# transferia/transferia

Measured on NVIDIA H100. Metric: ChangeItems/sec on ClickBench-shaped 99-col batches (filter_rows + cast + ClickHouse native block + LZ4 frames), higher is better.
Workload: dtype u8

## Files before the change

### transferia_b200/csrc/device_types.cuh

```cuda
#pragma once
#include <cstdint>
#include "../../include/tfgpu.h"

namespace tfk {

enum OutKind : int32_t {
    OK_COPY = 0,
    OK_BOOL = 1,
    OK_DATE = 2,
    OK_DATETIME = 3,
    OK_TS64 = 4,
    OK_STR = 5,
    OK_MASK = 6,
    OK_TODT = 8,
    OK_TOSTR = 7
};

struct DCol {
    int32_t type;
    int32_t out_kind;
    int32_t in_w;
    int32_t out_w;
    int32_t nullable;
    int32_t str_slot;
    int32_t mask_slot;
    int32_t pad;
    const uint8_t* values;
    const uint8_t* validity;
    const uint32_t* offsets;
    const uint8_t* heap;
    const uint8_t* aux;
    uint64_t hdr_off;
    uint64_t null_off;
    uint64_t out_off;
    uint64_t aux_off;
    uint64_t offs_off;
};

struct DTerm {
    int32_t col, op, vtype, nlist;
    int64_t i; double f;
    uint32_t s_off, s_len;
    uint32_t list_off, pad;
};

struct DFilterStep { int32_t expr_begin, nexpr, step_index, flags; };

struct DState {
    uint64_t n_kept;
    uint64_t n_errors;
    uint64_t raw_total;
    uint64_t n_frames;
    uint64_t wire_total;
    uint32_t frame_ticket;
    uint32_t pad;
};

__host__ __device__ inline int varint_len(uint64_t v) { int n = 1; while (v >= 0x80) { v >>= 7; n++; } return n; }

}
```

### transferia_b200/csrc/kernels_deflate.cuh

```cuda
#pragma once
#include "device_types.cuh"
#include "kernels_encode.cuh"
#include "deflate_sum.hpp"

namespace tfk {

#define DF_CHUNK 16384
#define DF_THREADS 512
#define DF_PPT (DF_CHUNK / DF_THREADS)
#define DF_HASH_BITS 12
#define DF_CHUNK_OVERHEAD 10
#define DF_FLAG_AGG (1ull << 62)
#define DF_FLAG_INCL (2ull << 62)
#define DF_VAL_MASK ((1ull << 62) - 1)

struct DfSmem { uint32_t data, dist, lenb, work, path, hist, lens, codes, sort, crct, total; };
__host__ __device__ inline DfSmem df_smem() {
    DfSmem s; uint32_t o = 0;
    s.data = o; o += 16 + DF_CHUNK + 32;
    s.dist = o; o += 2 * DF_CHUNK;
    s.lenb = o; o += DF_CHUNK;
    s.work = o; o += 2 * DF_CHUNK + 64;
    s.path = o; o += (DF_CHUNK / 32 + 4) * 4;
    s.hist = o; o += (288 + 32 + 20) * 4;
    s.lens = o; o += 288 + 32 + 32;
    s.codes = o; o += (288 + 32 + 32) * 2;
    s.sort = o; o += 320 * 4 * 2 + 320 * 2 + 320 * 2;
    s.crct = o; o += 256 * 4;
    s.total = o; return s;
}

struct DeflateArgs {
    const uint8_t* text; uint64_t total;
    uint8_t* out;
    unsigned long long* pfx;
    uint32_t* sums;
    uint32_t* ticket;
    uint32_t nchunks;
    int zlib;
    DState* st;
};

__device__ __forceinline__ uint32_t df_ld32(const uint32_t* w, uint32_t p) {
    const uint32_t i = p >> 2, s = (p & 3) * 8;
    return __funnelshift_r(w[i], w[i + 1], s);
}
__device__ __forceinline__ uint32_t df_match_len(const uint32_t* dw, uint32_t c, uint32_t p, uint32_t maxl) {
    uint32_t n = 0;
    while (n < maxl) {
        const uint32_t x = df_ld32(dw, c + n) ^ df_ld32(dw, p + n);
        if (x) { n += (uint32_t)(__ffs((int)x) - 1) >> 3; break; }
        n += 4;
    }
    return n < maxl ? n : maxl;
}
__device__ __forceinline__ void df_len_sym(uint32_t len, uint32_t& sym, uint32_t& eb, uint32_t& ev) {
    const uint32_t l = len - 3;
    if (l < 8) { sym = 257 + l; eb = 0; ev = 0; }
    else if (l == 255) { sym = 285; eb = 0; ev = 0; }
    else { const uint32_t nb = 31 - __clz(l); eb = nb - 2; sym = 257 + 4 * (nb - 1) + ((l >> eb) & 3); ev = l & ((1u << eb) - 1); }
}
__device__ __forceinline__ void df_dist_sym(uint32_t d, uint32_t& sym, uint32_t& eb, uint32_t& ev) {
    const uint32_t v = d - 1;
    if (v < 4) { sym = v; eb = 0; ev = 0; }
    else { const uint32_t nb = 31 - __clz(v); eb = nb - 1; sym = 2 * nb + ((v >> eb) & 1); ev = v & ((1u << eb) - 1); }
}
__device__ __forceinline__ uint32_t df_fixed_len(uint32_t s) { return s < 144 ? 8 : s < 256 ? 9 : s < 280 ? 7 : 8; }
__device__ __forceinline__ void df_put(uint32_t* img, uint32_t at, uint32_t v, uint32_t n) {
    if (!n) return;
    const uint32_t w = at >> 5, s = at & 31;
    atomicOr(&img[w], v << s);
    if (s + n > 32) atomicOr(&img[w + 1], v >> (32 - s));
}

#ifdef TF_KERNELS_DEFLATE
__device__ void df_huff_lengths(uint32_t* w, const uint16_t* sym, int n, uint32_t maxbits, uint8_t* lens) {
    w[0] += w[1];
    int root = 0, leaf = 2;
    for (int next = 1; next < n - 1; next++) {
        if (leaf >= n || w[root] < w[leaf]) { w[next] = w[root]; w[root++] = (uint32_t)next; }
        else w[next] = w[leaf++];
        if (leaf >= n || (root < next && w[root] < w[leaf])) { w[next] += w[root]; w[root++] = (uint32_t)next; }
        else w[next] += w[leaf++];
    }
    w[n - 2] = 0;
    for (int next = n - 3; next >= 0; next--) w[next] = w[w[next]] + 1;
    {
        int avail = 1, used = 0, depth = 0, r = n - 2, next = n - 1;
        while (avail > 0) {
            while (r >= 0 && (int)w[r] == depth) { used++; r--; }
            while (avail > used) { w[next--] = (uint32_t)depth; avail--; }
            avail = 2 * used; depth++; used = 0;
        }
    }
    uint32_t cnt[16];
    for (uint32_t l = 0; l <= 15; l++) cnt[l] = 0;
    for (int i = 0; i < n; i++) cnt[w[i] < maxbits ? w[i] : maxbits]++;
    uint32_t kraft = 0;
    for (uint32_t l = 1; l <= maxbits; l++) kraft += cnt[l] << (maxbits - l);
    while (kraft > (1u << maxbits)) {
        cnt[maxbits]--;
        for (uint32_t l = maxbits - 1; l > 0; l--) if (cnt[l]) { cnt[l]--; cnt[l + 1] += 2; break; }
        kraft--;
    }
    int i = n - 1;
    for (uint32_t l = 1; l <= maxbits; l++) for (uint32_t k = 0; k < cnt[l]; k++) lens[sym[i--]] = (uint8_t)l;
}
__device__ void df_codes(const uint8_t* lens, int n, uint16_t* codes) {
    uint32_t cnt[16], next[16];
    for (int l = 0; l < 16; l++) cnt[l] = 0;
    for (int s = 0; s < n; s++) cnt[lens[s]]++;
    cnt[0] = 0; uint32_t c = 0;
    for (int l = 1; l < 16; l++) { c = (c + cnt[l - 1]) << 1; next[l] = c; }
    for (int s = 0; s < n; s++) { const uint32_t l = lens[s]; codes[s] = l ? (uint16_t)(__brev(next[l]++) >> (32 - l)) : 0; }
}

__device__ __forceinline__ unsigned long long df_lookback(const DeflateArgs& a, uint32_t f, uint32_t lane) {
    unsigned long long excl = 0;
    int64_t base = (int64_t)f;
    for (uint32_t spins = 0; base > 0;) {
        const int64_t j = base - 1 - (int64_t)lane;
        const unsigned long long v = j >= 0 ? *(volatile unsigned long long*)&a.pfx[j] : DF_FLAG_INCL;
        const uint32_t fl = (uint32_t)(v >> 62);
        const uint32_t incl = __ballot_sync(0xffffffffu, fl == 2), none = __ballot_sync(0xffffffffu, fl == 0);
        const uint32_t upto = incl ? (uint32_t)__ffs((int)incl) - 1 : 31u;
        const uint32_t need = upto == 31 ? 0xffffffffu : ((2u << upto) - 1);
        if (none & need) {
            if (++spins > (1u << 20)) { if (lane == 0) a.st->pad = 1; break; }
            __nanosleep(100); continue;
        }
        unsigned long long part = lane <= upto ? (v & DF_VAL_MASK) : 0ull;
#pragma unroll
        for (int d = 16; d; d >>= 1) part += __shfl_xor_sync(0xffffffffu, part, d);
        excl += part; base -= 32;
        if (incl) break;
    }
    return excl;
}

__device__ __forceinline__ uint32_t df_block_xor(uint32_t v, uint32_t* red) {
#pragma unroll
    for (int d = 16; d; d >>= 1) v ^= __shfl_xor_sync(0xffffffffu, v, d);
    if ((threadIdx.x & 31) == 0) red[threadIdx.x >> 5] = v;
    __syncthreads();
    uint32_t r = 0;
    for (uint32_t w = 0; w < (blockDim.x + 31) / 32; w++) r ^= red[w];
    __syncthreads();
    return r;
}
__device__ __forceinline__ uint64_t df_block_sum64(uint64_t v, unsigned long long* red) {
#pragma unroll
    for (int d = 16; d; d >>= 1) v += __shfl_xor_sync(0xffffffffu, v, d);
    if ((threadIdx.x & 31) == 0) red[threadIdx.x >> 5] = v;
    __syncthreads();
    uint64_t r = 0;
    for (uint32_t w = 0; w < (blockDim.x + 31) / 32; w++) r += red[w];
    __syncthreads();
    return r;
}

__global__ void __launch_bounds__(DF_THREADS, 2) k_deflate_chunks(DeflateArgs a) {
    extern __shared__ __align__(16) uint8_t smem[];
    const DfSmem S = df_smem();
    uint8_t* db = smem + S.data + 16;
    const uint32_t* dw = (const uint32_t*)db;
    uint16_t* dist = (uint16_t*)(smem + S.dist);
    uint8_t* lenb = smem + S.lenb;
    uint16_t* J = (uint16_t*)(smem + S.work);
    uint32_t* img = (uint32_t*)(smem + S.work);
    uint32_t* path = (uint32_t*)(smem + S.path);
    uint32_t* hl = (uint32_t*)(smem + S.hist); uint32_t* hd = hl + 288; uint32_t* hc = hd + 32;
    uint8_t* ll_len = smem + S.lens; uint8_t* d_len = ll_len + 288; uint8_t* c_len = d_len + 32;
    uint16_t* ll_code = (uint16_t*)(smem + S.codes); uint16_t* d_code = ll_code + 288; uint16_t* c_code = d_code + 32;
    uint32_t* bw = (uint32_t*)(smem + S.sort);
    uint32_t* sw = bw + 320;
    uint16_t* ssym = (uint16_t*)(sw + 320);
    uint16_t* rle = ssym + 320;
    uint32_t* crct = (uint32_t*)(smem + S.crct);
    __shared__ uint32_t s_f, s_btype, s_hdr_bits, s_nbytes, s_nrle, s_hlit, s_hdist, s_hclen;
    __shared__ uint32_t red[33];
    __shared__ unsigned long long red64[32], s_off;
    const uint32_t tid = threadIdx.x, lane = tid & 31, warp = tid >> 5;

    for (uint32_t i = tid; i < 256; i += DF_THREADS) {
        uint32_t c = i;
        for (int k = 0; k < 8; k++) c = (c & 1) ? (c >> 1) ^ tfdf::CRC_POLY : c >> 1;
        crct[i] = c;
    }
    for (;;) {
        __syncthreads();
        if (tid == 0) s_f = atomicAdd(a.ticket, 1u);
        __syncthreads();
        const uint32_t f = s_f;
        if (f >= a.nchunks) break;
        const uint64_t pos0 = (uint64_t)f * DF_CHUNK;
        const uint32_t L = (uint32_t)((a.total - pos0 < DF_CHUNK) ? a.total - pos0 : DF_CHUNK);

        {
            const int4* g = (const int4*)(a.text + pos0);
            const uint32_t nv = (L + 15) >> 4;
            int4* d4 = (int4*)db;
            for (uint32_t i = tid; i < DF_CHUNK / 16 + 2; i += DF_THREADS) d4[i] = i < nv ? __ldg(g + i) : make_int4(0, 0, 0, 0);
            if (tid < 4) ((uint32_t*)(smem + S.data))[tid] = 0;
            int4* t4 = (int4*)J;
            for (uint32_t i = tid; i < (2u << DF_HASH_BITS) / 16; i += DF_THREADS) t4[i] = make_int4(0, 0, 0, 0);
            for (uint32_t i = tid; i < DF_CHUNK / 32 + 4; i += DF_THREADS) path[i] = 0;
            for (uint32_t i = tid; i < 288 + 32 + 20; i += DF_THREADS) hl[i] = 0;
        }
        __syncthreads();
        if (tid < 16 && L + tid < ((L + 15) & ~15u)) db[L + tid] = 0;
        {
            const uint32_t b0 = tid * DF_PPT, b1 = b0 + DF_PPT < L ? b0 + DF_PPT : L, nb = b1 > b0 ? b1 - b0 : 0;
            if (a.zlib) {
                uint64_t s1 = 0, s2 = 0;
                for (uint32_t i = 0; i < nb; i++) { const uint32_t v = db[b0 + i]; s1 += v; s2 += (uint64_t)(L - b0 - i) * v; }
                s1 = df_block_sum64(s1, red64) % tfdf::ADLER_MOD; s2 = df_block_sum64(s2, red64) % tfdf::ADLER_MOD;
                if (tid == 0) { a.sums[2 * f] = (uint32_t)s1; a.sums[2 * f + 1] = (uint32_t)s2; }
            } else {
                uint32_t c = 0;
                if (nb) {
                    c = 0xffffffffu;
                    for (uint32_t i = 0; i < nb; i++) c = crct[(c ^ db[b0 + i]) & 0xff] ^ (c >> 8);
                    c = tfdf::crc_mulmod(tfdf::crc_xpow8(L - b1), ~c);
                }
                c = df_block_xor(c, red);
                if (tid == 0) a.sums[2 * f] = c;
            }
        }

        const uint32_t nrounds = (L + DF_THREADS - 1) / DF_THREADS;
        for (uint32_t r = 0; r < nrounds; r++) {
            const uint32_t p = r * DF_THREADS + tid;
            const bool valid = p + 4 <= L;
            const uint32_t w = valid ? df_ld32(dw, p) : 0, h = (w * 2654435761u) >> (32 - DF_HASH_BITS);
            const uint32_t t1 = valid ? J[h] : 0;
            __syncthreads();
            if (valid) J[h] = (uint16_t)(p + 1);
            __syncthreads();
            const uint32_t t2 = valid ? J[h] : 0;
            uint32_t best = 0, bd = 0;
            if (valid) {
                const uint32_t maxl = L - p < 258 ? L - p : 258;
                uint32_t c = 0xffffffffu;
                if (p >= 1 && df_ld32(dw, p - 1) == w) c = p - 1;
                else if (p >= 2 && df_ld32(dw, p - 2) == w) c = p - 2;
                else if (p >= 4 && df_ld32(dw, p - 4) == w) c = p - 4;
                if (c != 0xffffffffu) { best = df_match_len(dw, c, p, maxl); bd = p - c; }
                const uint32_t ct = (t2 && t2 - 1 < p) ? t2 - 1 : (t1 ? t1 - 1 : 0xffffffffu);
                if (ct != 0xffffffffu && ct != c && best < maxl) {
                    const uint32_t m = df_match_len(dw, ct, p, maxl);
                    if (m > best) { best = m; bd = p - ct; }
                }
            }
            if (p < L) { lenb[p] = (uint8_t)(best >= 4 ? best - 3 : 0); dist[p] = (uint16_t)bd; }
        }
        __syncthreads();

        for (uint32_t k = 0; k < DF_PPT; k++) { const uint32_t p = tid * DF_PPT + k; if (p < L) J[p] = (uint16_t)(p + (lenb[p] ? lenb[p] + 3u : 1u)); }
        if (tid == 0) { J[L] = (uint16_t)L; path[0] = 1; }
        __syncthreads();
        for (;;) {
            uint32_t bits = path[tid];
            while (bits) {
                const uint32_t k = (uint32_t)__ffs((int)bits) - 1; bits &= bits - 1;
                const uint32_t p = tid * DF_PPT + k;
                if (p < L) { const uint32_t q = J[p]; if (q < L) atomicOr(&path[q >> 5], 1u << (q & 31)); }
            }
            __syncthreads();
            uint32_t nx[DF_PPT / 2];
#pragma unroll
            for (uint32_t k = 0; k < DF_PPT; k += 2) {
                const uint32_t p = tid * DF_PPT + k;
                const uint32_t lo = p < L ? J[J[p]] : 0, hi = p + 1 < L ? J[J[p + 1]] : 0;
                nx[k / 2] = lo | (hi << 16);
            }
            __syncthreads();
#pragma unroll
            for (uint32_t k = 0; k < DF_PPT; k += 2) {
                const uint32_t p = tid * DF_PPT + k;
                if (p < L) J[p] = (uint16_t)nx[k / 2];
                if (p + 1 < L) J[p + 1] = (uint16_t)(nx[k / 2] >> 16);
            }
            __syncthreads();
            if (J[0] == L) break;
            __syncthreads();
        }
        const uint32_t mine = path[tid] & (tid * DF_PPT + DF_PPT <= L ? 0xffffffffu : (tid * DF_PPT < L ? (1u << (L - tid * DF_PPT)) - 1 : 0u));

        uint32_t ext = 0;
        for (uint32_t bits = mine; bits;) {
            const uint32_t k = (uint32_t)__ffs((int)bits) - 1; bits &= bits - 1;
            const uint32_t p = tid * DF_PPT + k, l = lenb[p];
            if (!l) { atomicAdd(&hl[db[p]], 1u); continue; }
            uint32_t s, eb, ev, ds, deb, dev;
            df_len_sym(l + 3, s, eb, ev); df_dist_sym(dist[p], ds, deb, dev);
            atomicAdd(&hl[s], 1u); atomicAdd(&hd[ds], 1u); ext += eb + deb;
        }
        if (tid == 0) atomicAdd(&hl[256], 1u);
        uint32_t ext_total; block_excl_scan(ext, &ext_total, red);

        const int nzd = __syncthreads_count(tid < 30 && hd[tid] > 0);
        if (tid < 288) { bw[tid] = tid < 286 ? hl[tid] : 0; ll_len[tid] = 0; }
        else if (tid < 320) {
            const uint32_t i = tid - 288; uint32_t v = i < 30 ? hd[i] : 0;
            if (i < 30 && !v && ((nzd == 0 && i < 2) || (nzd == 1 && i == (hd[0] ? 1u : 0u)))) v = 1;
            bw[tid] = v; d_len[i] = 0;
        }
        __syncthreads();
        {
            const bool ll = tid < 286, dd = tid >= 288 && tid < 318;
            if (ll || dd) {
                const uint32_t base = ll ? 0 : 288, n = ll ? 286 : 30, i = tid - base, v = bw[tid];
                if (v) {
                    uint32_t rank = 0;
                    for (uint32_t j = 0; j < n; j++) { const uint32_t u = bw[base + j]; rank += (u && (u < v || (u == v && j < i))) ? 1u : 0u; }
                    sw[base + rank] = v; ssym[base + rank] = (uint16_t)i;
                }
            }
        }
        const int nzl = __syncthreads_count(tid < 286 && hl[tid] > 0);
        if (tid == 0) df_huff_lengths(sw, ssym, nzl, 15, ll_len);
        if (tid == 32) df_huff_lengths(sw + 288, ssym + 288, nzd < 2 ? 2 : nzd, 15, d_len);
        __syncthreads();
        if (tid == 0) {
            uint32_t hlit = 286; while (hlit > 257 && !ll_len[hlit - 1]) hlit--;
            uint32_t hdist = 30; while (hdist > 1 && !d_len[hdist - 1]) hdist--;
            const uint32_t N = hlit + hdist;
            auto lv = [&](uint32_t i) -> uint32_t { return i < hlit ? ll_len[i] : d_len[i - hlit]; };
            uint32_t nr = 0;
            for (uint32_t i = 0; i < N;) {
                const uint32_t v = lv(i); uint32_t run = 1;
                while (i + run < N && lv(i + run) == v) run++;
                i += run;
                if (v == 0) {
                    while (run >= 11) { const uint32_t r = run < 138 ? run : 138; rle[nr++] = (uint16_t)(18 | ((r - 11) << 8)); run -= r; }
                    if (run >= 3) { rle[nr++] = (uint16_t)(17 | ((run - 3) << 8)); run = 0; }
                } else {
                    rle[nr++] = (uint16_t)v; run--;
                    while (run >= 3) { const uint32_t r = run < 6 ? run : 6; rle[nr++] = (uint16_t)(16 | ((r - 3) << 8)); run -= r; }
                }
                while (run) { rle[nr++] = (uint16_t)v; run--; }
            }
            for (uint32_t k = 0; k < nr; k++) hc[rle[k] & 0xff]++;
            uint32_t n = 0;
            for (uint32_t s = 0; s < 19; s++) { c_len[s] = 0; if (hc[s]) { sw[n] = hc[s]; ssym[n] = (uint16_t)s; n++; } }
            for (uint32_t s = 0; n < 2; s++) if (!hc[s]) { sw[n] = 1; ssym[n] = (uint16_t)s; n++; }
            for (uint32_t i = 1; i < n; i++) {
                const uint32_t v = sw[i]; const uint16_t y = ssym[i]; int j = (int)i - 1;
                while (j >= 0 && (sw[j] > v || (sw[j] == v && ssym[j] > y))) { sw[j + 1] = sw[j]; ssym[j + 1] = ssym[j]; j--; }
                sw[j + 1] = v; ssym[j + 1] = y;
            }
            df_huff_lengths(sw, ssym, (int)n, 7, c_len);
            const uint8_t order[19] = {16, 17, 18, 0, 8, 7, 9, 6, 10, 5, 11, 4, 12, 3, 13, 2, 14, 1, 15};
            uint32_t hclen = 19; while (hclen > 4 && !c_len[order[hclen - 1]]) hclen--;
            uint64_t hdr = 14 + 3 * hclen;
            for (uint32_t s = 0; s < 19; s++) hdr += (uint64_t)hc[s] * (c_len[s] + (s == 16 ? 2 : s == 17 ? 3 : s == 18 ? 7 : 0));
            uint64_t dyn = 3 + hdr + ext_total, fix = 3 + ext_total;
            for (uint32_t s = 0; s < 286; s++) { dyn += (uint64_t)hl[s] * ll_len[s]; fix += (uint64_t)hl[s] * df_fixed_len(s); }
            for (uint32_t s = 0; s < 30; s++) { dyn += (uint64_t)hd[s] * d_len[s]; fix += (uint64_t)hd[s] * 5; }
            const uint64_t by_dyn = (dyn + 3 + 7) / 8 + 4, by_fix = (fix + 3 + 7) / 8 + 4, by_sto = (uint64_t)L + DF_CHUNK_OVERHEAD;
            uint32_t bt = 2; uint64_t by = by_dyn;
            if (by_fix <= by) { bt = 1; by = by_fix; }
            if (by_sto <= by) { bt = 0; by = by_sto; }
            s_btype = bt; s_nbytes = (uint32_t)by; s_hdr_bits = bt == 2 ? (uint32_t)hdr : 0;
            s_nrle = nr; s_hlit = hlit; s_hdist = hdist; s_hclen = hclen;
            if (bt == 1) { for (uint32_t s = 0; s < 288; s++) ll_len[s] = (uint8_t)df_fixed_len(s); for (uint32_t s = 0; s < 30; s++) d_len[s] = 5; }
            if (bt != 0) { df_codes(ll_len, 288, ll_code); df_codes(d_len, 30, d_code); df_codes(c_len, 19, c_code); }
        }
        __syncthreads();
        const uint32_t btype = s_btype, nbytes = s_nbytes;
        for (uint32_t i = tid; i < (nbytes + 11) / 4; i += DF_THREADS) img[i] = 0;
        __syncthreads();

        if (btype == 0) {
            uint8_t* ib = (uint8_t*)img;
            if (tid == 0) { ib[1] = (uint8_t)L; ib[2] = (uint8_t)(L >> 8); ib[3] = (uint8_t)~L; ib[4] = (uint8_t)(~L >> 8); ib[L + 8] = 0xff; ib[L + 9] = 0xff; }
            for (uint32_t i = tid; i < L; i += DF_THREADS) ib[5 + i] = db[i];
        } else {
            if (tid == 0) {
                df_put(img, 0, (uint32_t)btype << 1, 3);
                if (btype == 2) {
                    uint32_t at = 3;
                    df_put(img, at, s_hlit - 257, 5); df_put(img, at + 5, s_hdist - 1, 5); df_put(img, at + 10, s_hclen - 4, 4); at += 14;
                    const uint8_t order[19] = {16, 17, 18, 0, 8, 7, 9, 6, 10, 5, 11, 4, 12, 3, 13, 2, 14, 1, 15};
                    for (uint32_t k = 0; k < s_hclen; k++) { df_put(img, at, c_len[order[k]], 3); at += 3; }
                    for (uint32_t k = 0; k < s_nrle; k++) {
                        const uint32_t s = rle[k] & 0xff, x = rle[k] >> 8;
                        df_put(img, at, c_code[s], c_len[s]); at += c_len[s];
                        const uint32_t xb = s == 16 ? 2 : s == 17 ? 3 : s == 18 ? 7 : 0;
                        df_put(img, at, x, xb); at += xb;
                    }
                }
            }
            uint32_t my = 0;
            for (uint32_t bits = mine; bits;) {
                const uint32_t k = (uint32_t)__ffs((int)bits) - 1; bits &= bits - 1;
                const uint32_t p = tid * DF_PPT + k, l = lenb[p];
                if (!l) { my += ll_len[db[p]]; continue; }
                uint32_t s, eb, ev, ds, deb, dev;
                df_len_sym(l + 3, s, eb, ev); df_dist_sym(dist[p], ds, deb, dev);
                my += ll_len[s] + eb + d_len[ds] + deb;
            }
            uint32_t tok_total; uint32_t at = 3 + s_hdr_bits + block_excl_scan(my, &tok_total, red);
            for (uint32_t bits = mine; bits;) {
                const uint32_t k = (uint32_t)__ffs((int)bits) - 1; bits &= bits - 1;
                const uint32_t p = tid * DF_PPT + k, l = lenb[p];
                if (!l) { const uint32_t c = db[p]; df_put(img, at, ll_code[c], ll_len[c]); at += ll_len[c]; continue; }
                uint32_t s, eb, ev, ds, deb, dev;
                df_len_sym(l + 3, s, eb, ev); df_dist_sym(dist[p], ds, deb, dev);
                df_put(img, at, ll_code[s] | (ev << ll_len[s]), ll_len[s] + eb); at += ll_len[s] + eb;
                df_put(img, at, d_code[ds] | (dev << d_len[ds]), d_len[ds] + deb); at += d_len[ds] + deb;
            }
            if (tid == 0) {
                const uint32_t e = 3 + s_hdr_bits + tok_total;
                df_put(img, e, ll_code[256], ll_len[256]);
                uint8_t* ib = (uint8_t*)img; ib[nbytes - 2] = 0xff; ib[nbytes - 1] = 0xff;
            }
        }
        if (tid == 0) *(volatile unsigned long long*)&a.pfx[f] = DF_FLAG_AGG | nbytes;
        __syncthreads();

        if (warp == 0) {
            const unsigned long long excl = df_lookback(a, f, lane);
            if (lane == 0) { *(volatile unsigned long long*)&a.pfx[f] = DF_FLAG_INCL | (excl + nbytes); s_off = excl; }
        }
        __syncthreads();
        uint8_t* G = a.out + (a.zlib ? sizeof(tfdf::ZLIB_HDR) : sizeof(tfdf::GZIP_HDR)) + s_off;
        const uint8_t* ib = (const uint8_t*)img;
        for (uint32_t i = tid; i < nbytes; i += DF_THREADS) G[i] = ib[i];
    }
}

__global__ void __launch_bounds__(1024) k_deflate_finish(DeflateArgs a) {
    __shared__ uint32_t red[33];
    __shared__ unsigned long long red64[32];
    const uint32_t tid = threadIdx.x, n = a.nchunks;
    const uint64_t T = a.total;
    const uint32_t per = (n + blockDim.x - 1) / blockDim.x, f0 = tid * per < n ? tid * per : n, f1 = f0 + per < n ? f0 + per : n;
    uint32_t sum;
    if (a.zlib) {
        uint64_t s1 = 0, s2 = 0;
        for (uint32_t f = f0; f < f1; f++) {
            const uint64_t end = (uint64_t)f * DF_CHUNK + DF_CHUNK < T ? (uint64_t)f * DF_CHUNK + DF_CHUNK : T;
            s1 += a.sums[2 * f]; s2 = (s2 + a.sums[2 * f + 1] + ((T - end) % tfdf::ADLER_MOD) * a.sums[2 * f]) % tfdf::ADLER_MOD;
        }
        s1 = df_block_sum64(s1 % tfdf::ADLER_MOD, red64) % tfdf::ADLER_MOD;
        s2 = df_block_sum64(s2, red64) % tfdf::ADLER_MOD;
        sum = (uint32_t)((((T % tfdf::ADLER_MOD) + s2) % tfdf::ADLER_MOD) << 16 | ((1 + s1) % tfdf::ADLER_MOD));
    } else {
        uint32_t acc = 0; uint64_t end = (uint64_t)f0 * DF_CHUNK;
        const uint32_t xc = tfdf::crc_xpow8(DF_CHUNK);
        for (uint32_t f = f0; f < f1; f++) {
            const uint64_t len = T - end < DF_CHUNK ? T - end : DF_CHUNK;
            acc = tfdf::crc_mulmod(len == DF_CHUNK ? xc : tfdf::crc_xpow8(len), acc) ^ a.sums[2 * f];
            end += len;
        }
        if (f1 > f0) acc = tfdf::crc_mulmod(tfdf::crc_xpow8(T - end), acc);
        sum = df_block_xor(acc, red);
    }
    if (tid == 0) {
        const uint32_t hdr = a.zlib ? sizeof(tfdf::ZLIB_HDR) : sizeof(tfdf::GZIP_HDR);
        const uint64_t body = n ? (a.pfx[n - 1] & DF_VAL_MASK) : 0;
        uint8_t* o = a.out;
        if (a.zlib) { o[0] = 0x78; o[1] = 0x9c; }
        else { o[0] = 0x1f; o[1] = 0x8b; o[2] = 0x08; for (int i = 3; i < 9; i++) o[i] = 0; o[9] = 0xff; }
        o += hdr + body;
        *o++ = 0x03; *o++ = 0x00;
        if (a.zlib) { for (int i = 0; i < 4; i++) *o++ = (uint8_t)(sum >> (24 - 8 * i)); }
        else { for (int i = 0; i < 4; i++) *o++ = (uint8_t)(sum >> (8 * i)); for (int i = 0; i < 4; i++) *o++ = (uint8_t)(T >> (8 * i)); }
        a.st->wire_total = hdr + body + 2 + (a.zlib ? tfdf::ZLIB_TRAILER : tfdf::GZIP_TRAILER);
    }
}
#endif

}
```

### transferia_b200/csrc/kernels_encode.cuh

```cuda
#pragma once
#include "device_types.cuh"

namespace tfk {

__device__ __forceinline__ uint32_t warp_incl_scan(uint32_t v) {
    const unsigned lane = threadIdx.x & 31;
#pragma unroll
    for (int d = 1; d < 32; d <<= 1) { uint32_t t = __shfl_up_sync(0xffffffffu, v, d); if (lane >= (unsigned)d) v += t; }
    return v;
}
__device__ __forceinline__ uint32_t block_excl_scan(uint32_t v, uint32_t* total, uint32_t* smem33) {
    const unsigned lane = threadIdx.x & 31, warp = threadIdx.x >> 5, nw = (blockDim.x + 31) >> 5;
    uint32_t inc = warp_incl_scan(v);
    if (lane == 31) smem33[warp] = inc;
    __syncthreads();
    if (warp == 0) {
        uint32_t w = lane < nw ? smem33[lane] : 0;
        uint32_t wi = warp_incl_scan(w);
        smem33[lane] = wi - w;
        if (lane == 31) smem33[32] = wi;
    }
    __syncthreads();
    uint32_t res = inc - v + smem33[warp];
    *total = smem33[32];
// ... 119 lines not shown
    const bool is_float1 = v.cls == 2 || v.cls == 3 || v.cls == 0;
    const double float1 = v.cls == 2 ? v.f : (v.cls == 3 ? v.f : 0.0);
    const int64_t* il = (const int64_t*)(blob + t.list_off);
    const double* fl = (const double*)(blob + t.list_off);
    switch (base) {
    case 1:
        if (is_int1) {
            if (is_set) { bool c = false; for (int k = 0; k < t.nlist; k++) c |= (il[k] == v.i); matched = (op == 6) ? c : !c; return 0; }
            matched = ordered<int64_t>(v.i, t.i, op); return 0;
        }
        if (is_float1) {
            if (is_set) {
                if (trunc(float1) == float1) { int64_t x = go_f2i64(float1); bool c = false; for (int k = 0; k < t.nlist; k++) c |= (il[k] == x); matched = (op == 6) ? c : !c; }
                else matched = false;
                return 0;
            }
            matched = ordered<double>(float1, (double)t.i, op); return 0;
        }
        break;
    case 2:
        if (is_int1 || is_float1) {
            const double x = is_int1 ? (double)v.i : float1;
            if (is_set) { bool c = false; for (int k = 0; k < t.nlist; k++) c |= (fl[k] == x); matched = (op == 6) ? c : !c; return 0; }
            matched = ordered<double>(x, t.f, op); return 0;
        }
        break;
    case 3:
        if (!is_list && v.cls == 3) { matched = ordered<int>(v.i ? 1 : 0, t.i ? 1 : 0, op); return 0; }
        break;
    case 4:
        if (v.cls == 4 || v.cls == 5) {
            const uint8_t* lit = blob + t.s_off;
            if (!is_list) {
                if (op == 8) { matched = contains_bytes(v.s, v.slen, lit, t.s_len); return 0; }
                if (op == 9) { matched = !contains_bytes(v.s, v.slen, lit, t.s_len); return 0; }
                if (is_set) return TF_ROWERR_FILTER_TYPEPAIR;
                const int c = cmp_bytes(v.s, v.slen, lit, t.s_len);
                matched = ordered<int>(c, 0, op); return 0;
            }
            if (!is_set) return TF_ROWERR_FILTER_TYPEPAIR;
            const uint32_t* so = (const uint32_t*)(blob + t.list_off);
            const uint8_t* sh = (const uint8_t*)(so + t.nlist + 1);
            bool c = false;
            for (int k = 0; k < t.nlist && !c; k++) { uint32_t a = so[k], b = so[k + 1]; c = (b - a == v.slen) && cmp_bytes(sh + a, b - a, v.s, v.slen) == 0; }
            matched = (op == 6) ? c : !c; return 0;
        }
        break;
    case 5:
        if (v.cls == 6) {
            const int64_t um = v.i * 1000000LL + (int64_t)(v.nsec / 1000u);
            if (is_set) { bool c = false; for (int k = 0; k < t.nlist; k++) c |= (il[k] == um); matched = (op == 6) ? c : !c; return 0; }
            matched = ordered<int64_t>(um, t.i, op); return 0;
        }
        break;
    case 6:
        if (op == 0) { matched = v.cls == 0; return 0; }
        if (op == 1) { matched = v.cls != 0; return 0; }
        break;
    }
    return TF_ROWERR_FILTER_TYPEPAIR;
}

struct FilterArgs {
    const DCol* cols; const uint8_t* kinds; uint64_t nrows;
    const DFilterStep* steps; int nsteps;
    const uint32_t* expr_off;
    const DTerm* terms; const uint8_t* blob;
    uint8_t* keep; uint8_t* errcode; uint16_t* errstep; uint32_t* blockcnt; DState* st;
    const uint8_t* pre_err;
    const uint16_t* pre_term;
    int sink_guard;
};

#ifdef TF_KERNELS_ENCODE
__global__ void __launch_bounds__(256) k_filter(FilterArgs a) {
    __shared__ uint32_t s_cnt, s_err;
    if (threadIdx.x == 0) { s_cnt = 0; s_err = 0; }
    __syncthreads();
    const uint64_t r = (uint64_t)blockIdx.x * blockDim.x + threadIdx.x;
    bool keep = false, is_err = false;
    if (r < a.nrows) {
        keep = true; int err = 0, estep = 0;
        const int kind = a.kinds ? a.kinds[r] : TF_KIND_INSERT;
        if (a.pre_err && a.pre_err[r]) { err = a.pre_err[r]; estep = a.pre_term ? a.pre_term[r] : 0xff; keep = false; }
        for (int s = 0; s < a.nsteps && keep; s++) {
            const DFilterStep st = a.steps[s];
            if (st.flags & 1) { if ((st.expr_begin >> kind) & 1) keep = false; continue; }
            if (kind == TF_KIND_UPDATE || kind == TF_KIND_DELETE) { err = TF_ROWERR_FILTER_KIND; estep = st.step_index; keep = false; break; }
            if (st.flags & 2) continue;
            bool any = false;
            for (int e = 0; e < st.nexpr && !any && !err; e++) {
                bool all = true;
                const uint32_t kb = a.expr_off[st.expr_begin + e], ke = a.expr_off[st.expr_begin + e + 1];
                for (uint32_t k = kb; k < ke; k++) {
                    const DTerm t = a.terms[k];
                    const RowVal v = load_val(a.cols[t.col], r);
                    bool m = false; const int rc = eval_term(v, t, a.blob, m);
                    if (rc) { err = rc; break; }
                    if (!m) { all = false; break; }
                }
                if (!err && all) any = true;
            }
            if (err) { estep = st.step_index; keep = false; break; }
            if (!any) keep = false;
        }
        if (keep && a.sink_guard && (kind == TF_KIND_UPDATE || kind == TF_KIND_DELETE)) { err = TF_ROWERR_SINK_KIND_HOST; estep = 0xff; keep = false; }
        a.keep[r] = keep ? 1 : 0;
        a.errcode[r] = (uint8_t)err; a.errstep[r] = (uint16_t)estep; is_err = err != 0;
    }
    const unsigned b = __ballot_sync(0xffffffffu, keep);
    const unsigned be = __ballot_sync(0xffffffffu, is_err);
    if ((threadIdx.x & 31) == 0) { if (b) atomicAdd(&s_cnt, __popc(b)); if (be) atomicAdd(&s_err, __popc(be)); }
    __syncthreads();
    if (threadIdx.x == 0) { a.blockcnt[blockIdx.x] = s_cnt; if (s_err) atomicAdd((unsigned long long*)&a.st->n_errors, (unsigned long long)s_err); }
}
#endif

struct DevRowErr { uint32_t row; uint16_t code, term; };
#ifdef TF_KERNELS_ENCODE
__global__ void __launch_bounds__(256) k_collect_errors(const uint8_t* errcode, const uint16_t* errstep, uint64_t nrows, DevRowErr* out, unsigned long long* counter, unsigned long long cap) {
    const uint64_t r = (uint64_t)blockIdx.x * blockDim.x + threadIdx.x;
    const uint8_t c = r < nrows ? errcode[r] : 0;
    if (!c) return;
    const unsigned long long at = atomicAdd(counter, 1ull);
    if (at < cap) out[at] = DevRowErr{(uint32_t)r, c, errstep[r]};
}
#endif

#ifdef TF_KERNELS_ENCODE
__global__ void __launch_bounds__(1024) k_scan_blockcnt(const uint32_t* blockcnt, uint32_t* blockoff, uint32_t nblocks, DState* st) {
    __shared__ uint32_t sm[33];
    uint32_t carry = 0;
    for (uint32_t base = 0; base < nblocks; base += blockDim.x) {
        const uint32_t i = base + threadIdx.x;
        const uint32_t v = i < nblocks ? blockcnt[i] : 0;
        uint32_t tot; const uint32_t ex = block_excl_scan(v, &tot, sm);
        if (i < nblocks) blockoff[i] = carry + ex;
        carry += tot;
    }
    if (threadIdx.x == 0) st->n_kept = carry;
}
#endif

#ifdef TF_KERNELS_ENCODE
__global__ void __launch_bounds__(256) k_compact_sel(const uint8_t* keep, const uint32_t* blockoff, uint64_t nrows, uint32_t* sel) {
    __shared__ uint32_t sm[33];
    const uint64_t r = (uint64_t)blockIdx.x * blockDim.x + threadIdx.x;
    const uint32_t k = (r < nrows && keep[r]) ? 1u : 0u;
    uint32_t tot; const uint32_t ex = block_excl_scan(k, &tot, sm);
    if (k) sel[blockoff[blockIdx.x] + ex] = (uint32_t)r;
}
#endif

struct LayoutArgs {
    DCol* cols; int ncols;
    const int32_t* out_cols;
    const int32_t* str_cols; int nstr;
    const uint32_t* tile_sum;
    uint64_t* tile_base;
    uint32_t ntiles_cap;
    const uint8_t* col_headers; const uint32_t* col_header_off;
    uint8_t* raw; DState* st;
    uint64_t nrows_in; int has_sel; uint32_t frame_bytes;
    uint64_t* col_bytes;
};

#define TF_STR_TILE 256
#define TF_STR_THREADS 256
#define TF_STR_STAGE 16384

#ifdef TF_KERNELS_ENCODE
__global__ void __launch_bounds__(1024) k_layout_scan(LayoutArgs a) {
    __shared__ uint32_t sm[33];
    const int s = blockIdx.x;
    const uint64_t n = a.st->n_kept;
    const uint32_t ntiles = (uint32_t)((n + TF_STR_TILE - 1) / TF_STR_TILE);
    uint64_t carry = 0;
    for (uint32_t base = 0; base < ntiles; base += blockDim.x) {
        const uint32_t i = base + threadIdx.x;
        const uint32_t v = i < ntiles ? a.tile_sum[(size_t)s * a.ntiles_cap + i] : 0;
        uint32_t tot; const uint32_t ex = block_excl_scan(v, &tot, sm);
        if (i < ntiles) a.tile_base[(size_t)s * a.ntiles_cap + i] = carry + ex;
        carry += tot;
    }
    if (threadIdx.x == 0) a.col_bytes[s] = carry;
}
#endif

#ifdef TF_KERNELS_ENCODE
__global__ void __launch_bounds__(256) k_layout_finish(LayoutArgs a) {
    __shared__ uint64_t s_size[3][256];
    __shared__ uint64_t s_pos[256];
    __shared__ uint64_t s_run;
    const uint64_t n = a.st->n_kept;
    if (threadIdx.x == 0) {
        uint8_t* o = a.raw; uint64_t p = 0;
        o[p++] = 1; o[p++] = 0; o[p++] = 2; o[p++] = 0xff; o[p++] = 0xff; o[p++] = 0xff; o[p++] = 0xff; o[p++] = 0;
        uint64_t v = (uint64_t)a.ncols; while (v >= 0x80) { o[p++] = (uint8_t)(v | 0x80); v >>= 7; } o[p++] = (uint8_t)v;
        v = n; while (v >= 0x80) { o[p++] = (uint8_t)(v | 0x80); v >>= 7; } o[p++] = (uint8_t)v;
        s_run = p;
    }
    for (int base = 0; base < a.ncols; base += 256) {
        const int c = base + threadIdx.x;
        __syncthreads();
        if (c < a.ncols) {
            const DCol& d = a.cols[a.out_cols[c]];
            s_size[0][threadIdx.x] = a.col_header_off[c + 1] - a.col_header_off[c];
            s_size[1][threadIdx.x] = (d.nullable && n) ? n : 0;
            s_size[2][threadIdx.x] = n ? ((d.out_kind == OK_STR || d.out_kind == OK_TOSTR) ? a.col_bytes[d.str_slot] : (uint64_t)d.out_w * n) : 0;
        }
        __syncthreads();
        if (threadIdx.x == 0) {
            uint64_t p = s_run; const int m = a.ncols - base < 256 ? a.ncols - base : 256;
            for (int k = 0; k < m; k++) { s_pos[k] = p; p += s_size[0][k] + s_size[1][k] + s_size[2][k]; }
            s_run = p;
        }
        __syncthreads();
        if (c < a.ncols) {
            DCol& d = a.cols[a.out_cols[c]];
            const uint64_t p = s_pos[threadIdx.x];
            d.hdr_off = p; d.null_off = p + s_size[0][threadIdx.x]; d.out_off = d.null_off + s_size[1][threadIdx.x];
            const uint32_t hb = a.col_header_off[c], hn = (uint32_t)s_size[0][threadIdx.x];
            for (uint32_t k = 0; k < hn; k++) a.raw[p + k] = a.col_headers[hb + k];
        }
    }
    __syncthreads();
    if (threadIdx.x == 0) {
        const uint64_t p = s_run;
        a.st->raw_total = p;
        a.st->n_frames = p ? (p + a.frame_bytes - 1) / a.frame_bytes : 1;
        a.st->frame_ticket = 0;
    }
}
#endif

struct ColRegions { uint64_t values, validity, aux, offsets, heap, heap_len; };

#ifdef TF_KERNELS_ENCODE
__global__ void __launch_bounds__(256) k_layout_columnar(LayoutArgs a, ColRegions* regions) {
    __shared__ uint64_t s_sz[5][256];
    __shared__ uint64_t s_pos[256];
    __shared__ uint64_t s_run;
    const uint64_t n = a.st->n_kept;
    if (threadIdx.x == 0) s_run = 0;
    for (int base = 0; base < a.ncols; base += 256) {
        const int k = base + threadIdx.x;
        __syncthreads();
        if (k < a.ncols) {
            const DCol& d = a.cols[a.out_cols[k]];
            const bool var = d.out_kind == OK_STR || d.out_kind == OK_MASK || d.out_kind == OK_TOSTR;
            const bool fresh = d.out_kind == OK_MASK || d.out_kind == OK_TOSTR || d.out_kind == OK_TODT;
            const uint64_t heap = (d.out_kind == OK_STR || d.out_kind == OK_TOSTR) ? a.col_bytes[d.str_slot] : (d.out_kind == OK_MASK ? 64 * n : 0);
            s_sz[0][threadIdx.x] = var ? 0 : (uint64_t)d.out_w * n;
            s_sz[1][threadIdx.x] = (d.validity && !fresh) ? (n + 7) / 8 : 0;
            s_sz[2][threadIdx.x] = (d.aux && !fresh) ? (d.type == TF_ANY ? n : 4 * n) : 0;
            s_sz[3][threadIdx.x] = var ? 4 * (n + 1) : 0;
            s_sz[4][threadIdx.x] = heap;
        }
        __syncthreads();
        if (threadIdx.x == 0) {
            uint64_t p = s_run; const int m = a.ncols - base < 256 ? a.ncols - base : 256;
            for (int q = 0; q < m; q++) { s_pos[q] = p; for (int z = 0; z < 5; z++) p += (s_sz[z][q] + 15) & ~15ull; }
            s_run = p;
        }
        __syncthreads();
        if (k < a.ncols) {
            DCol& d = a.cols[a.out_cols[k]];
            uint64_t p = s_pos[threadIdx.x]; ColRegions r;
            auto take = [&](int z) { const uint64_t at = p; p += (s_sz[z][threadIdx.x] + 15) & ~15ull; return at; };
            const uint64_t v = take(0), val = take(1), ax = take(2), of = take(3), hp = take(4);
            const bool var = d.out_kind == OK_STR || d.out_kind == OK_MASK || d.out_kind == OK_TOSTR;
            d.out_off = var ? hp : v; d.null_off = val; d.aux_off = ax; d.offs_off = of;
            r.values = var ? ~0ull : v; r.validity = s_sz[1][threadIdx.x] ? val : ~0ull; r.aux = s_sz[2][threadIdx.x] ? ax : ~0ull;
            r.offsets = var ? of : ~0ull; r.heap = var ? hp : ~0ull; r.heap_len = s_sz[4][threadIdx.x];
            regions[k] = r;
            if (var) ((uint32_t*)(a.raw + of))[n] = (uint32_t)s_sz[4][threadIdx.x];
        }
    }
    __syncthreads();
    if (threadIdx.x == 0) { a.st->raw_total = s_run; a.st->n_frames = 0; a.st->frame_ticket = 0; }
}
#endif

struct EncodeArgs {
    const DCol* cols;
    const int32_t* slots;
    const uint32_t* sel; const DState* st; uint8_t* raw;
    uint32_t* tile_sum; const uint64_t* tile_base; uint32_t ntiles_cap;
    int columnar;
};

#define TF_SLOT_NULLMAP (1 << 30)
#define TF_SLOT_AUX (1 << 29)
#define TF_SLOT_ZEROMAP (1 << 28)
#define TF_FIX_TILE_WORDS 2048
#define CH_MAX_DATE_SEC 4291747200LL

enum StreamKind { SK_COPY = 0, SK_BOOL, SK_DATE, SK_DATETIME, SK_TS64, SK_NULLMAP, SK_AUX32, SK_AUX8, SK_ZERO, SK_TODT_CH, SK_TODT_SEC };

template <int K, int INW> __device__ __forceinline__ uint64_t elem_t(const DCol& c, const uint32_t* sel, uint64_t j, uint64_t n) {
    if (j >= n) return 0;
    const uint64_t r = sel ? sel[j] : j;
    if (K == SK_ZERO) return 0;
    if (K == SK_TODT_CH || K == SK_TODT_SEC) {
        int64_t s = 0;
        if (row_valid(c, r)) s = c.type == TF_INT32 ? (int64_t)((const int32_t*)c.values)[r] : (int64_t)((const uint32_t*)c.values)[r];
        if (K == SK_TODT_SEC) return (uint64_t)s;
        if (s > CH_MAX_DATE_SEC) s = CH_MAX_DATE_SEC;
        if (s < 0) s = 0;
        return (uint64_t)s;
    }
    if (K == SK_AUX8) return (uint64_t)c.aux[r];
    if (K == SK_AUX32) return (uint64_t)((const uint32_t*)c.aux)[r];
    const bool valid = row_valid(c, r);
    if (K == SK_NULLMAP) return valid ? 0 : 1;
    if (!valid) return 0;
    if (K == SK_COPY) {
        if (INW == 1) return c.values[r];
        if (INW == 2) return ((const uint16_t*)c.values)[r];
        if (INW == 4) return ((const uint32_t*)c.values)[r];
        return ((const uint64_t*)c.values)[r];
    }
    if (K == SK_BOOL) return c.values[r] != 0;
    if (K == SK_DATE || K == SK_DATETIME) {
        int64_t s = ((const int64_t*)c.values)[r];
        const uint32_t ns = c.aux ? ((const uint32_t*)c.aux)[r] : 0;
        if (s > CH_MAX_DATE_SEC || (s == CH_MAX_DATE_SEC && ns > 0)) s = CH_MAX_DATE_SEC;
        if (s < 0) s = 0;
        return K == SK_DATE ? (uint64_t)(s / 86400) : (uint64_t)s;
    }
    const int64_t s = ((const int64_t*)c.values)[r];
    const uint32_t ns = c.aux ? ((const uint32_t*)c.aux)[r] : 0;
    return (uint64_t)(s * 1000000LL + (int64_t)(ns / 1000u));
}

template <int K, int INW, int W> __device__ __forceinline__ uint32_t stream_word_t(const DCol& c, const uint32_t* sel, uint64_t q, uint64_t n) {
    if (W == 1) return (uint32_t)elem_t<K, INW>(c, sel, 4 * q, n) | ((uint32_t)elem_t<K, INW>(c, sel, 4 * q + 1, n) << 8) |
                       ((uint32_t)elem_t<K, INW>(c, sel, 4 * q + 2, n) << 16) | ((uint32_t)elem_t<K, INW>(c, sel, 4 * q + 3, n) << 24);
    if (W == 2) return (uint32_t)(elem_t<K, INW>(c, sel, 2 * q, n) & 0xffff) | ((uint32_t)(elem_t<K, INW>(c, sel, 2 * q + 1, n) & 0xffff) << 16);
    if (W == 4) return (uint32_t)elem_t<K, INW>(c, sel, q, n);
    const uint64_t v = elem_t<K, INW>(c, sel, q >> 1, n); return (uint32_t)(v >> ((q & 1) * 32));
}

template <int K, int INW, int W> __device__ __forceinline__ void encode_stream(const DCol& c, const EncodeArgs& a, uint64_t base, uint64_t n) {
    const uint32_t m = (uint32_t)(base & 3);
    const uint64_t total = n * (uint64_t)W;
    const uint64_t T = (m + total + 3) >> 2;
    uint8_t* dst0 = a.raw + (base - m);
    const unsigned lane = threadIdx.x & 31;
    for (uint64_t t0 = (uint64_t)blockIdx.x * TF_FIX_TILE_WORDS; t0 < T; t0 += (uint64_t)gridDim.x * TF_FIX_TILE_WORDS)
#pragma unroll 2
    for (uint32_t it = 0; it < TF_FIX_TILE_WORDS / 256; it++) {
        const uint64_t t = t0 + it * 256 + threadIdx.x;
        const uint32_t wcur = (t < T) ? stream_word_t<K, INW, W>(c, a.sel, t, n) : 0;
        uint32_t wprev = __shfl_up_sync(0xffffffffu, wcur, 1);
        if (lane == 0) wprev = (m && t > 0 && t <= T) ? stream_word_t<K, INW, W>(c, a.sel, t - 1, n) : 0;
        if (t >= T) continue;
        const uint32_t val = m ? __funnelshift_r(wprev, wcur, 8 * (4 - m)) : wcur;
        const int64_t sb = (int64_t)(4 * t) - (int64_t)m;
        uint8_t* dst = dst0 + 4 * t;
        if (sb >= 0 && (uint64_t)sb + 4 <= total) *(uint32_t*)dst = val;
        else {
#pragma unroll
            for (int b = 0; b < 4; b++) { const int64_t x = sb + b; if (x >= 0 && (uint64_t)x < total) dst[b] = (uint8_t)(val >> (8 * b)); }
        }
    }
}

#ifdef TF_KERNELS_ENCODE
__global__ void __launch_bounds__(256) k_encode_fixed(EncodeArgs a) {
    const int32_t slot = a.slots[blockIdx.y];
    const DCol c = a.cols[slot & ~(TF_SLOT_NULLMAP | TF_SLOT_AUX | TF_SLOT_ZEROMAP)];
    const uint64_t n = a.st->n_kept;
    if (n == 0) return;
// ... 70 lines not shown
```

### transferia_b200/csrc/kernels_lz4.cuh

```cuda
#pragma once
#include "device_types.cuh"
#include "kernels_encode.cuh"

namespace tfk {

#ifndef LZ_THREADS
#define LZ_THREADS 256
#endif
#define LZ_CTAS_PER_SM (LZ_THREADS <= 256 ? 4 : 2)
#define LZ_ROUND (4 * LZ_THREADS)
#define LZ_SEG 60
#ifndef LZ_HASH_BITS
#define LZ_HASH_BITS 11
#endif
#define LZ_MAX_FRAME (LZ_THREADS * LZ_SEG)
#define LZ_HDR 25
#define LZ_NONE 0xffffffffu
#define LZ_FLAG_AGG (1ull << 62)
#define LZ_FLAG_INCL (2ull << 62)
#define LZ_VAL_MASK ((1ull << 62) - 1)

__host__ __device__ inline uint32_t lz4_bound(uint32_t n) { return n + n / 255 + 16; }

struct LzSmem { uint32_t data, cand, bitmap, table, stg, total; };
__host__ __device__ inline LzSmem lz_smem(uint32_t F) {
    LzSmem s; uint32_t o = 0;
    const uint32_t F16 = (F + 15) & ~15u;
    s.data = o + 16; o += 16 + F16 + 16;
    s.cand = o; o += F16;
    s.bitmap = o; o += ((F + LZ_ROUND - 1) / LZ_ROUND) * (LZ_THREADS / 4) + 16;
    s.table = o; o += 4u << LZ_HASH_BITS;
    s.stg = o + 16; o += 16 + ((9 + lz4_bound(F) + 15) & ~15u) + 32;
    s.total = o; return s;
}

struct Lz4Args {
    const uint8_t* raw; DState* st; uint8_t* wire; uint32_t* comp_size; uint64_t* wire_off;
    unsigned long long* pfx;
    uint64_t* tail;
    uint32_t frame_bytes;
    unsigned long long* phases;
};
#define LZ_PHASE(k) do { if (a.phases && tid == 0) { const long long t_ = clock64(); atomicAdd(&a.phases[k], (unsigned long long)(t_ - t_ph)); t_ph = t_; } } while (0)

__device__ __forceinline__ uint32_t ld32u(const uint32_t* w, uint32_t p) {
    const uint32_t i = p >> 2, s = (p & 3) * 8;
    return __funnelshift_r(w[i], w[i + 1], s);
}
__device__ __forceinline__ uint32_t ext_bytes(uint32_t x) { return x < 15 ? 0u : 1u + (x - 15u) / 255u; }
__device__ __forceinline__ uint8_t* put_ext(uint8_t* o, uint32_t x) {
    x -= 15; while (x >= 255) { *o++ = 255; x -= 255; } *o++ = (uint8_t)x; return o;
}
__device__ __forceinline__ void put_bytes3(uint8_t* dst, uint32_t x, uint32_t n) {
#pragma unroll
    for (uint32_t k = 0; k < 3; k++) if (k < n) dst[k] = (uint8_t)(x >> (8 * k));
}
__device__ __forceinline__ void copy_lit(uint8_t* dst, const uint32_t* dw, uint32_t src, uint32_t n) {
    const uint32_t h = min(n, (0u - (uint32_t)(uintptr_t)dst) & 3u);
    if (h) { put_bytes3(dst, ld32u(dw, src), h); dst += h; src += h; n -= h; }
    for (; n >= 8; n -= 8, dst += 8, src += 8) {
        const uint32_t x = ld32u(dw, src), y = ld32u(dw, src + 4);
        *(uint32_t*)dst = x; *(uint32_t*)(dst + 4) = y;
    }
    if (n >= 4) { *(uint32_t*)dst = ld32u(dw, src); n -= 4; dst += 4; src += 4; }
    if (n) put_bytes3(dst, ld32u(dw, src), n);
}
__device__ __forceinline__ uint32_t lz_match_len(const uint32_t* dw, uint32_t c, uint32_t p, uint32_t maxl) {
    uint32_t ic = c >> 2, ip = p >> 2; const uint32_t sc = (c & 3) * 8, sp = (p & 3) * 8;
    uint32_t wc0 = dw[ic], wp0 = dw[ip], ml = 0;
    for (;;) {
        const uint32_t wc1 = dw[ic + 1], wp1 = dw[ip + 1], wc2 = dw[ic + 2], wp2 = dw[ip + 2];
        const uint32_t x0 = __funnelshift_r(wc0, wc1, sc) ^ __funnelshift_r(wp0, wp1, sp);
        const uint32_t x1 = __funnelshift_r(wc1, wc2, sc) ^ __funnelshift_r(wp1, wp2, sp);
        if (x0 | x1) { ml += x0 ? (uint32_t)(__ffs((int)x0) - 1) >> 3 : 4u + ((uint32_t)(__ffs((int)x1) - 1) >> 3); break; }
        ml += 8; if (ml >= maxl) break;
        ic += 2; ip += 2; wc0 = wc2; wp0 = wp2;
    }
    return ml < maxl ? ml : maxl;
}
__device__ __forceinline__ uint32_t lz_back_len(const uint32_t* dw, uint32_t c, uint32_t p, uint32_t maxb) {
    uint32_t n = 0;
    while (n < maxb) {
        const int32_t qc = (int32_t)(c - n) - 4, qp = (int32_t)(p - n) - 4;
        const uint32_t x = __funnelshift_r(dw[qc >> 2], dw[(qc >> 2) + 1], (qc & 3) * 8) ^ __funnelshift_r(dw[qp >> 2], dw[(qp >> 2) + 1], (qp & 3) * 8);
        if (x) { n += (uint32_t)__clz((int)x) >> 3; break; }
        n += 4;
    }
    return n < maxb ? n : maxb;
}

__device__ __forceinline__ unsigned long long lz_lookback(const Lz4Args& a, uint32_t f, uint32_t lane) {
    unsigned long long excl = 0;
    if (!f) return 0;
    int64_t base = (int64_t)f;
    for (uint32_t spins = 0;;) {
        unsigned long long v[4];
#pragma unroll
        for (int k = 0; k < 4; k++) { const int64_t j = base - 1 - 32 * k - (int64_t)lane; v[k] = j >= 0 ? *(volatile unsigned long long*)&a.pfx[j] : LZ_FLAG_INCL; }
        bool done = false, stale = false;
#pragma unroll
        for (int k = 0; k < 4; k++) {
            if (done || stale) continue;
            const uint32_t fl = (uint32_t)(v[k] >> 62);
            const uint32_t incl = __ballot_sync(0xffffffffu, fl == 2), none = __ballot_sync(0xffffffffu, fl == 0);
            const uint32_t upto = incl ? (uint32_t)__ffs((int)incl) - 1 : 31u;
            const uint32_t need = upto == 31 ? 0xffffffffu : ((2u << upto) - 1);
            if (none & need) { stale = true; continue; }
            unsigned long long part = lane <= upto ? (v[k] & LZ_VAL_MASK) : 0ull;
#pragma unroll
            for (int d = 16; d; d >>= 1) part += __shfl_xor_sync(0xffffffffu, part, d);
            excl += part; base -= 32;
            if (incl) done = true;
        }
        if (done) break;
        if (stale) { if (++spins > (1u << 20)) { if (lane == 0) a.st->pad = 1; break; } __nanosleep(100); }
    }
    return excl;
}

#ifdef TF_KERNELS_LZ4
template <bool FULL>
__device__ __forceinline__ void lz_match_round(const uint32_t* dw, uint32_t* table, uint32_t* cand_w, uint32_t* bm, uint32_t wi, uint32_t lane, uint32_t len) {
    const uint32_t p0 = wi * 4;
    const bool active = FULL || p0 < len;
    uint32_t i0 = 0, i1 = 0, i2 = 0, i3 = 0, e0 = 0, e1 = 0, e2 = 0, e3 = 0, c0 = LZ_NONE, c2 = LZ_NONE, t0 = 0, t2 = 0;
    if (active) {
        const uint32_t wm2 = dw[(int)wi - 2], wm1 = dw[(int)wi - 1], w0 = dw[wi], w1 = dw[wi + 1];
        const uint32_t s1 = __funnelshift_r(w0, w1, 8), s2 = __funnelshift_r(w0, w1, 16), s3 = __funnelshift_r(w0, w1, 24);
        const uint32_t h0 = w0 * 2654435761u, h1 = s1 * 2654435761u, h2 = s2 * 2654435761u, h3 = s3 * 2654435761u;
        i0 = h0 >> (32 - LZ_HASH_BITS); i1 = h1 >> (32 - LZ_HASH_BITS); i2 = h2 >> (32 - LZ_HASH_BITS); i3 = h3 >> (32 - LZ_HASH_BITS);
        e0 = ((h0 << LZ_HASH_BITS) & 0xffff0000u) | p0; e1 = ((h1 << LZ_HASH_BITS) & 0xffff0000u) | (p0 + 1);
        e2 = ((h2 << LZ_HASH_BITS) & 0xffff0000u) | (p0 + 2); e3 = ((h3 << LZ_HASH_BITS) & 0xffff0000u) | (p0 + 3);
        const uint32_t a2 = __funnelshift_r(wm1, w0, 16), b2 = __funnelshift_r(wm2, wm1, 16);
        c0 = w0 == wm1 ? p0 - 4 : (w0 == wm2 ? p0 - 8 : LZ_NONE);
        c2 = s2 == a2 ? p0 - 2 : (s2 == b2 ? p0 - 6 : LZ_NONE);
        if (p0 < 8) c0 = c2 = LZ_NONE;
        t0 = table[i0]; t2 = table[i2];
    }
    __syncthreads();
    if (active) {
        table[i3] = e3; table[i2] = e2; table[i1] = e1; table[i0] = e0;
        if (c0 == LZ_NONE && ((t0 ^ e0) >> 16) == 0) c0 = t0 & 0xffffu;
        if (c2 == LZ_NONE && ((t2 ^ e2) >> 16) == 0) c2 = t2 & 0xffffu;
    }
    __syncthreads();
    if (active) {
        if (c0 == LZ_NONE) { const uint32_t t = table[i0]; if (((t ^ e0) >> 16) == 0 && (t & 0xffffu) < p0) c0 = t & 0xffffu; }
        if (c2 == LZ_NONE) { const uint32_t t = table[i2]; if (((t ^ e2) >> 16) == 0 && (t & 0xffffu) < p0 + 2) c2 = t & 0xffffu; }
        cand_w[wi] = (c0 & 0xffffu) | (c2 << 16);
    }
    const uint32_t b0 = __ballot_sync(0xffffffffu, c0 != LZ_NONE), b2 = __ballot_sync(0xffffffffu, c2 != LZ_NONE);
    if (lane == 0) { bm[2 * (wi >> 5)] = b0; bm[2 * (wi >> 5) + 1] = b2; }
}
__device__ __forceinline__ uint32_t lz_spread(uint32_t x) {
    x = (x | (x << 8)) & 0x00ff00ffu; x = (x | (x << 4)) & 0x0f0f0f0fu; x = (x | (x << 2)) & 0x33333333u; return (x | (x << 1)) & 0x55555555u;
}

__global__ void __launch_bounds__(LZ_THREADS, LZ_CTAS_PER_SM) k_lz4_frames(Lz4Args a) {
    extern __shared__ __align__(16) uint8_t smem[];
    const uint32_t F = a.frame_bytes;
    const LzSmem L = lz_smem(F);
    uint32_t* dw = (uint32_t*)(smem + L.data);
    uint16_t* cand = (uint16_t*)(smem + L.cand);
    uint32_t* cand_w = (uint32_t*)(smem + L.cand);
    uint32_t* bm = (uint32_t*)(smem + L.bitmap);
    uint32_t* table = (uint32_t*)(smem + L.table);
    uint8_t* stg = smem + L.stg;
    __shared__ uint32_t s_frame;
    __shared__ uint32_t scratch[80];
    __shared__ unsigned long long s_woff;
    int32_t* delta0 = (int32_t*)table;
    uint32_t* scanv = (uint32_t*)(delta0 + LZ_THREADS);
    uint16_t* carry_incl = (uint16_t*)(scanv + LZ_THREADS);
    uint16_t* ext16 = carry_incl + LZ_THREADS;
    uint8_t* clt8 = (uint8_t*)(ext16 + LZ_THREADS + 4);
    uint8_t* flg8 = clt8 + LZ_THREADS;
    const uint32_t tid = threadIdx.x, lane = tid & 31, warp = tid >> 5;
    const uint64_t raw_total = a.st->raw_total, n_frames = a.st->n_frames;

    uint32_t pend_f = 0xffffffffu, pend_cs = 0;
    auto resolve_flush = [&](uint32_t pf, uint32_t pcs) {
        if (warp == 0) {
            const unsigned long long excl = lz_lookback(a, pf, lane);
            if (lane == 0) {
                *(volatile unsigned long long*)&a.pfx[pf] = LZ_FLAG_INCL | (excl + pcs + LZ_HDR);
                s_woff = excl;
                a.comp_size[pf] = pcs; a.wire_off[pf] = excl;
                if (pf + 1 == n_frames) { a.st->wire_total = excl + pcs + LZ_HDR; a.tail[0] = n_frames; }
            }
        }
        __syncthreads();
        uint8_t* G = a.wire + s_woff + 16;
        const uint32_t m = (uint32_t)((uintptr_t)G & 15), total = 9 + pcs;
        const uint32_t nchunks = (m + total + 15) >> 4;
        int4* g4 = (int4*)(G - m);
        const uint32_t* sw = (const uint32_t*)(stg - 16);
        const uint32_t o0 = 16 - m, sh = (o0 & 3) * 8;
        for (uint32_t j = tid; j < nchunks; j += LZ_THREADS) {
            const uint32_t wi0 = (o0 + 16 * j) >> 2;
            const uint32_t q0 = sw[wi0], q1 = sw[wi0 + 1], q2 = sw[wi0 + 2], q3 = sw[wi0 + 3], q4 = sw[wi0 + 4];
            int4 v;
            v.x = (int)__funnelshift_r(q0, q1, sh); v.y = (int)__funnelshift_r(q1, q2, sh);
            v.z = (int)__funnelshift_r(q2, q3, sh); v.w = (int)__funnelshift_r(q3, q4, sh);
            g4[j] = v;
        }
        __syncthreads();
    };
    for (;;) {
        __syncthreads();
        if (tid == 0) s_frame = atomicAdd(&a.st->frame_ticket, 1u);
        __syncthreads();
        const uint32_t f = s_frame;
        if (f >= n_frames) break;
        long long t_ph = a.phases ? clock64() : 0;
        const uint64_t pos0 = (uint64_t)f * F;
        const uint32_t len = (uint32_t)((raw_total - pos0 < F) ? raw_total - pos0 : F);

        {
            const int4* g = (const int4*)(a.raw + pos0);
            const uint32_t nv = (len + 15) >> 4;
            int4* d4 = (int4*)(smem + L.data);
            constexpr uint32_t NLD = (LZ_MAX_FRAME / 16 + LZ_THREADS) / LZ_THREADS;
            int4 v[NLD];
#pragma unroll
            for (uint32_t k = 0; k < NLD; k++) { const uint32_t i = tid + k * LZ_THREADS; v[k] = i < nv ? __ldg(g + i) : make_int4(0, 0, 0, 0); }
#pragma unroll
            for (uint32_t k = 0; k < NLD; k++) { const uint32_t i = tid + k * LZ_THREADS; if (i < nv + 1) d4[i] = v[k]; }
            int4* t4 = (int4*)table;
            for (uint32_t i = tid; i < (1u << LZ_HASH_BITS) / 4; i += LZ_THREADS) t4[i] = make_int4(0, 0, 0, 0);
            if (tid < 4) ((uint32_t*)smem)[tid] = 0;
        }
        __syncthreads();

        LZ_PHASE(0);
        const uint32_t nrounds = (len + LZ_ROUND - 1) / LZ_ROUND;
        const uint32_t nfull = len / LZ_ROUND;
        for (uint32_t rd = 0; rd < nfull; rd++) lz_match_round<true>(dw, table, cand_w, bm, rd * LZ_THREADS + tid, lane, len);
        if (nfull < nrounds) lz_match_round<false>(dw, table, cand_w, bm, nfull * LZ_THREADS + tid, lane, len);
        if (tid == 0) { bm[((nrounds * LZ_THREADS) >> 4)] = 0; bm[((nrounds * LZ_THREADS) >> 4) + 1] = 0; }
        __syncthreads();
        if (tid == 0) bm[0] &= ~1u;

        LZ_PHASE(1);
        const uint32_t nseg = (len + LZ_SEG - 1) / LZ_SEG;
        const uint32_t lim5 = len >= 5 ? len - 5 : 0;
        const int32_t pmax = (int32_t)len - 12;
        const uint32_t sa = tid * LZ_SEG;
        uint32_t sb = 0, slimit = 0, nseq = 0, d_last = 0;
        bool reach = false, pure = false;
        uint32_t* desc = cand_w + tid * (LZ_SEG / 4);
        if (tid < nseg) {
            sb = sa + LZ_SEG < len ? sa + LZ_SEG : len;
            slimit = sb < lim5 ? sb : lim5;
            const uint32_t k = tid * (LZ_SEG / 4), bw = 2 * (k >> 5);
            const uint32_t m0 = __funnelshift_r(bm[bw], bm[bw + 2], k & 31) & 0x7fffu, m2 = __funnelshift_r(bm[bw + 1], bm[bw + 3], k & 31) & 0x7fffu;
            const uint32_t m = lz_spread(m0) | (lz_spread(m2) << 1);
            uint32_t cur = 0, anchor = sa;
            for (;;) {
                const uint32_t cb = (cur + 1) >> 1;
                if (cb >= LZ_SEG / 2) break;
                const uint32_t mm = m >> cb;
                if (!mm) break;
                const uint32_t r = cb + (uint32_t)__ffs((int)mm) - 1;
                uint32_t p = sa + 2 * r;
                if (p + 4 > slimit || (int32_t)p > pmax) break;
                uint32_t c = cand[p >> 1];
                uint32_t ml = lz_match_len(dw, c, p, slimit - p);
                if (ml < 4) { cur = 2 * r + 1; continue; }
                const uint32_t nb = lz_back_len(dw, c, p, min(p - anchor, c));
                p -= nb; c -= nb; ml += nb;
                desc[nseq++] = ((p - c) << 16) | (ml << 8) | (p - sa);
                d_last = p - c;
                anchor = p + ml; cur = anchor - sa;
            }
            reach = nseq && anchor == sa + LZ_SEG;
            pure = nseq == 1 && reach && (desc[0] & 0xffu) == 0;
        }
        __syncthreads();

        uint32_t k0 = 0, cl = 0, D = 0; bool merged = false, head = false;
        {
            uint32_t sv = tid < nseg ? (pure ? 0u : (reach ? (d_last << 2) | 2u : 1u)) : 1u;
#pragma unroll
            for (int d = 1; d < 32; d <<= 1) { const uint32_t o = __shfl_up_sync(0xffffffffu, sv, d); if (lane >= (uint32_t)d && sv == 0) sv = o; }
            if (lane == 31) scratch[warp] = sv;
            __syncthreads();
            if (sv == 0) { for (int w = (int)warp - 1; w >= 0; w--) { const uint32_t o = scratch[w]; if (o) { sv = o; break; } } if (sv == 0) sv = 1; }
            scanv[tid] = sv;
            __syncthreads();
            const uint32_t prev = tid ? scanv[tid - 1] : 1u;
            const bool dvalid = tid < nseg && prev >= 2;
            D = prev >> 2;
            uint32_t n = 0;
            if (dvalid && slimit > sa) {
                const uint32_t maxn = slimit - sa;
                const uint32_t q = sa - D; uint32_t iq = q >> 2; const uint32_t sq = (q & 3) * 8;
                uint32_t wq0 = dw[iq]; const uint32_t* pw = dw + tid * (LZ_SEG / 4);
                for (;;) {
                    const uint32_t wq1 = dw[iq + 1], wq2 = dw[iq + 2];
                    const uint32_t x0 = __funnelshift_r(wq0, wq1, sq) ^ pw[n >> 2], x1 = __funnelshift_r(wq1, wq2, sq) ^ pw[(n >> 2) + 1];
                    if (x0 | x1) { n += x0 ? (uint32_t)(__ffs((int)x0) - 1) >> 3 : 4u + ((uint32_t)(__ffs((int)x1) - 1) >> 3); break; }
                    n += 8; if (n >= maxn) break;
                    iq += 2; wq0 = wq2;
                }
                if (n > maxn) n = maxn;
            }
            clt8[tid] = (uint8_t)n; flg8[tid] = (uint8_t)((pure ? 1 : 0) | (reach ? 2 : 0) | (dvalid ? 4 : 0));
            __syncthreads();
            if (dvalid) {
                const uint32_t pf = flg8[tid - 1];
                const bool alive = (pf & 1) ? (clt8[tid - 1] == LZ_SEG && (pf & 4)) : (pf & 2) != 0;
                if (pure) {
                    if (!(alive && n > 0) && n != LZ_SEG) n = 0;
                    if (n && n < LZ_SEG && LZ_SEG - n < 4) n = LZ_SEG - 4;
                } else {
                    if (!alive) n = 0;
                    if (reach && n > LZ_SEG - 4) n = LZ_SEG - 4;
                }
                if (n && !alive && (int32_t)sa > pmax) n = 0;
                cl = n;
                if (n) {
                    merged = alive; head = !alive;
                    while (k0 < nseq) {
                        const uint32_t dsc = desc[k0], pr = dsc & 0xffu, ml = (dsc >> 8) & 0xffu;
                        if (pr + ml <= n) { k0++; continue; }
                        if (pr >= n) break;
                        const uint32_t nml = pr + ml - n;
                        if (nml >= 4 && (int32_t)(sa + n) <= pmax) desc[k0] = (dsc & 0xffff0000u) | (nml << 8) | n; else k0++;
                        break;
                    }
                }
            }
            uint32_t es = merged ? cl : 0u, ec = (merged && cl == LZ_SEG) ? 1u : 0u;
#pragma unroll
            for (int d = 1; d < 32; d <<= 1) {
                const uint32_t os = __shfl_down_sync(0xffffffffu, es, d), oc = __shfl_down_sync(0xffffffffu, ec, d);
                if (lane + d < 32 && ec) { es += os; ec = oc; }
            }
            if (lane == 0) { scratch[32 + warp] = es; scratch[48 + warp] = ec; }
            __syncthreads();
            if (ec) for (uint32_t w = warp + 1; w < LZ_THREADS / 32; w++) { es += scratch[32 + w]; if (!scratch[48 + w]) break; }
            ext16[tid] = (uint16_t)es;
            if (tid == 0) ext16[LZ_THREADS] = 0;
        }
        __syncthreads();
        const uint32_t ext_next = ext16[tid + 1];

        LZ_PHASE(2);
        const bool emits = tid < nseg && (head || k0 < nseq);
        uint32_t my_trail = 0;
        if (tid < nseg) {
            uint32_t last_end = sa + cl;
            if (k0 < nseq) { const uint32_t dsc = desc[nseq - 1]; last_end = sa + (dsc & 0xffu) + ((dsc >> 8) & 0xffu); }
            my_trail = sb - last_end;
        }
        {
            uint32_t has = emits ? 1u : 0u, tr = my_trail;
#pragma unroll
            for (int d = 1; d < 32; d <<= 1) {
                const uint32_t h2 = __shfl_up_sync(0xffffffffu, has, d), t2 = __shfl_up_sync(0xffffffffu, tr, d);
                if (lane >= (uint32_t)d && !has) { tr += t2; has = h2; }
            }
            if (lane == 31) { scratch[warp] = has; scratch[16 + warp] = tr; }
            __syncthreads();
            if (warp == 0) {
                uint32_t wh = lane < LZ_THREADS / 32 ? scratch[lane] : 0, wt = lane < LZ_THREADS / 32 ? scratch[16 + lane] : 0;
#pragma unroll
                for (int d = 1; d < 16; d <<= 1) {
                    const uint32_t h2 = __shfl_up_sync(0xffffffffu, wh, d), t2 = __shfl_up_sync(0xffffffffu, wt, d);
                    if (lane >= (uint32_t)d && !wh) { wt += t2; wh = h2; }
                }
                const uint32_t eh = __shfl_up_sync(0xffffffffu, wh, 1), et = __shfl_up_sync(0xffffffffu, wt, 1);
                if (lane < LZ_THREADS / 32) { scratch[lane] = lane ? eh : 0; scratch[16 + lane] = lane ? et : 0; }
            }
            __syncthreads();
            if (!has) { tr += scratch[16 + warp]; }
            carry_incl[tid] = (uint16_t)tr;
        }
        __syncthreads();
        const uint32_t carry_in = (tid > 0 && tid < nseg) ? carry_incl[tid - 1] : 0;

        uint32_t my_bytes = 0, p_first = 0, ll_first = 0;
        if (emits) {
            uint32_t prev_end = sa + (merged ? cl : 0u); bool first = true;
            if (head) {
                const uint32_t ml = LZ_SEG + ext_next;
                my_bytes += 1 + ext_bytes(carry_in) + carry_in + 2 + ext_bytes(ml - 4);
                p_first = sa; ll_first = carry_in; prev_end = sa + LZ_SEG; first = false;
            }
            for (uint32_t k = k0; k < nseq; k++) {
                const uint32_t dsc = desc[k], pr = dsc & 0xffu; uint32_t ml = (dsc >> 8) & 0xffu;
                const uint32_t p = sa + pr, ll = (first ? carry_in : 0u) + (p - prev_end);
                prev_end = p + ml;
                if (k + 1 == nseq && pr + ml == LZ_SEG) ml += ext_next;
                my_bytes += 1 + ext_bytes(ll) + ll + 2 + ext_bytes(ml - 4);
                if (first) { p_first = p; ll_first = ll; first = false; }
            }
        }
        uint32_t total_seq_bytes;
        const uint32_t my_off = block_excl_scan(my_bytes, &total_seq_bytes, scratch);
        if (emits) delta0[tid] = (int32_t)(my_off + 1 + ext_bytes(ll_first)) - (int32_t)(p_first - ll_first);
        uint32_t my_next_has = 0xffff;
        {
            const uint32_t hm = __ballot_sync(0xffffffffu, emits);
            if (lane == 0) scratch[40 + warp] = hm;
            __syncthreads();
            const uint32_t above = lane == 31 ? 0u : (hm >> (lane + 1));
            if (above) my_next_has = tid + (uint32_t)__ffs((int)above);
            else for (uint32_t w = warp + 1; w < LZ_THREADS / 32; w++) { const uint32_t m = scratch[40 + w]; if (m) { my_next_has = w * 32 + (uint32_t)__ffs((int)m) - 1; break; } }
        }
        const uint32_t ll_final = nseg ? carry_incl[nseg - 1] : 0;
        const int32_t delta_final = (int32_t)(total_seq_bytes + 1 + ext_bytes(ll_final)) - (int32_t)(len - ll_final);
        const uint32_t cs = total_seq_bytes + 1 + ext_bytes(ll_final) + ll_final;
        if (tid == 0) { *(volatile unsigned long long*)&a.pfx[f] = LZ_FLAG_AGG | (unsigned long long)(cs + LZ_HDR); }
        LZ_PHASE(3);
        if (pend_f != 0xffffffffu) resolve_flush(pend_f, pend_cs);
        LZ_PHASE(5);
        uint8_t* out = stg + 9;
        if (tid < nseg) {
            uint32_t prev_end = sa + (merged ? cl : 0u);
            if (emits) {
                uint8_t* o = out + my_off; bool first = true;
                if (head) {
                    const uint32_t mt = LZ_SEG + ext_next - 4, ll = carry_in;
                    *o++ = (uint8_t)(((ll < 15 ? ll : 15) << 4) | 15);
                    if (ll >= 15) o = put_ext(o, ll);
                    o += ll;
                    *o++ = (uint8_t)D; *o++ = (uint8_t)(D >> 8);
                    o = put_ext(o, mt);
                    prev_end = sa + LZ_SEG; first = false;
                }
                for (uint32_t k = k0; k < nseq; k++) {
                    const uint32_t dsc = desc[k], pr = dsc & 0xffu, off = dsc >> 16; uint32_t ml = (dsc >> 8) & 0xffu;
                    const uint32_t p = sa + pr, cin = first ? carry_in : 0u, ll = cin + (p - prev_end);
                    const uint32_t lit0 = prev_end, nlit = p - prev_end;
                    prev_end = p + ml;
                    if (k + 1 == nseq && pr + ml == LZ_SEG) ml += ext_next;
                    const uint32_t mt = ml - 4;
                    *o++ = (uint8_t)(((ll < 15 ? ll : 15) << 4) | (mt < 15 ? mt : 15));
                    if (ll >= 15) o = put_ext(o, ll);
                    copy_lit(o + cin, dw, lit0, nlit);
                    o += ll;
                    *o++ = (uint8_t)off; *o++ = (uint8_t)(off >> 8);
                    if (mt >= 15) o = put_ext(o, mt);
                    first = false;
                }
            }
            if (sb > prev_end) {
                const uint32_t nh = my_next_has;
                const int32_t dl = (nh != 0xffff && nh < nseg) ? delta0[nh] : delta_final;
                copy_lit(out + ((int32_t)prev_end + dl), dw, prev_end, sb - prev_end);
            }
        }
        if (tid == 0) {
            uint8_t* o = out + total_seq_bytes;
            *o++ = (uint8_t)((ll_final < 15 ? ll_final : 15) << 4);
            if (ll_final >= 15) o = put_ext(o, ll_final);
            const uint32_t c9 = cs + 9;
            stg[0] = 0x82; stg[1] = (uint8_t)c9; stg[2] = (uint8_t)(c9 >> 8); stg[3] = (uint8_t)(c9 >> 16); stg[4] = (uint8_t)(c9 >> 24);
            stg[5] = (uint8_t)len; stg[6] = (uint8_t)(len >> 8); stg[7] = (uint8_t)(len >> 16); stg[8] = (uint8_t)(len >> 24);
        }
        LZ_PHASE(4);
        pend_f = f; pend_cs = cs;
    }
    if (pend_f != 0xffffffffu) { __syncthreads(); resolve_flush(pend_f, pend_cs); }
}
#endif

namespace cityd {
#define CK0 0xc3a5c85c97cb3127ULL
#define CK1 0xb492b66fbe98f273ULL
#define CK2 0x9ae16a3b2f90404fULL
#define CK3 0xc949d7c7509e6557ULL
__device__ __forceinline__ uint64_t f64(const uint8_t* p) {
    const uintptr_t a = (uintptr_t)p; const uint64_t* q = (const uint64_t*)(a & ~(uintptr_t)7); const uint32_t s = (uint32_t)(a & 7) * 8;
    if (s == 0) return q[0];
    return (q[0] >> s) | (q[1] << (64 - s));
}
__device__ __forceinline__ uint32_t f32(const uint8_t* p) { return (uint32_t)p[0] | ((uint32_t)p[1] << 8) | ((uint32_t)p[2] << 16) | ((uint32_t)p[3] << 24); }
__device__ __forceinline__ uint64_t rot(uint64_t v, int s) { return s == 0 ? v : ((v >> s) | (v << (64 - s))); }
__device__ __forceinline__ uint64_t smix(uint64_t v) { return v ^ (v >> 47); }
__device__ __forceinline__ uint64_t hl16(uint64_t u, uint64_t v) {
    const uint64_t kMul = 0x9ddfea08eb382d69ULL;
    uint64_t a = (u ^ v) * kMul; a ^= (a >> 47);
    uint64_t b = (v ^ a) * kMul; b ^= (b >> 47); b *= kMul; return b;
}
static __device__ uint64_t hl0to16(const uint8_t* s, size_t len) {
    if (len > 8) { uint64_t a = f64(s), b = f64(s + len - 8); return hl16(a, rot(b + len, (int)len)) ^ b; }
    if (len >= 4) { uint64_t a = f32(s); return hl16(len + (a << 3), f32(s + len - 4)); }
    if (len > 0) { uint8_t a = s[0], b = s[len >> 1], c = s[len - 1]; uint32_t y = (uint32_t)a + ((uint32_t)b << 8); uint32_t z = (uint32_t)len + ((uint32_t)c << 2); return smix(y * CK2 ^ z * CK3) * CK2; }
    return CK2;
}
struct P { uint64_t first, second; };
__device__ __forceinline__ P weak32(uint64_t w, uint64_t x, uint64_t y, uint64_t z, uint64_t a, uint64_t b) {
    a += w; b = rot(b + a + z, 21); const uint64_t c = a; a += x; a += y; b += rot(a, 44); P r; r.first = a + z; r.second = b + c; return r;
}
__device__ __forceinline__ P weak32p(const uint8_t* s, uint64_t a, uint64_t b) { return weak32(f64(s), f64(s + 8), f64(s + 16), f64(s + 24), a, b); }
static __device__ P murmur(const uint8_t* s, size_t len, P seed) {
    uint64_t a = seed.first, b = seed.second, c = 0, d = 0; long l = (long)len - 16;
    if (l <= 0) { a = smix(a * CK1) * CK1; c = b * CK1 + hl0to16(s, len); d = smix(a + (len >= 8 ? f64(s) : c)); }
    else {
        c = hl16(f64(s + len - 8) + CK1, a); d = hl16(b + len, c + f64(s + len - 16)); a += d;
        do { a ^= smix(f64(s) * CK1) * CK1; a *= CK1; b ^= a; c ^= smix(f64(s + 8) * CK1) * CK1; c *= CK1; d ^= c; s += 16; l -= 16; } while (l > 0);
    }
    a = hl16(a, c); b = hl16(d, b);
    P r; r.first = a ^ b; r.second = hl16(b, a); return r;
}
static __device__ P hash128_seed(const uint8_t* s, size_t len, P seed) {
    if (len < 128) return murmur(s, len, seed);
    P v, w; uint64_t x = seed.first, y = seed.second, z = len * CK1;
    v.first = rot(y ^ CK1, 49) * CK1 + f64(s);
    v.second = rot(v.first, 42) * CK1 + f64(s + 8);
    w.first = rot(y + z, 35) * CK1 + x;
    w.second = rot(x + f64(s + 88), 53) * CK1;
    do {
#pragma unroll
        for (int rep = 0; rep < 2; rep++) {
            x = rot(x + y + v.first + f64(s + 16), 37) * CK1;
            y = rot(y + v.second + f64(s + 48), 42) * CK1;
            x ^= w.second; y ^= v.first; z = rot(z ^ w.first, 33);
            v = weak32p(s, v.second * CK1, x + w.first);
            w = weak32p(s + 32, z + w.second, y);
            const uint64_t t = z; z = x; x = t; s += 64;
        }
        len -= 128;
    } while (len >= 128);
    y += rot(w.first, 37) * CK0 + z;
    x += rot(v.first + z, 49) * CK0;
    for (size_t tail = 0; tail < len;) {
        tail += 32;
        y = rot(y - x, 42) * CK0 + v.second;
        w.first += f64(s + len - tail + 16);
        x = rot(x, 49) * CK0 + w.first;
        w.first += v.first;
        v = weak32p(s + len - tail, v.first, v.second);
    }
    x = hl16(x, v.first); y = hl16(y, w.first);
    P r; r.first = hl16(x + v.second, w.second) + y; r.second = hl16(x + w.second, y + v.second); return r;
}
static __device__ P hash128(const uint8_t* s, size_t len) {
    P seed;
    if (len >= 16) { seed.first = f64(s) ^ CK3; seed.second = f64(s + 8); return hash128_seed(s + 16, len - 16, seed); }
    if (len >= 8) { seed.first = f64(s) ^ (len * CK0); seed.second = f64(s + len - 8) ^ CK1; return hash128_seed(nullptr, 0, seed); }
    seed.first = CK0; seed.second = CK1; return hash128_seed(s, len, seed);
}
}

struct FrameArgs { const uint32_t* comp_size; const uint64_t* wire_off; uint8_t* wire; const uint64_t* tail; };

#define SEAL_STEP 512
#define SEAL_STRIDE 544
#define SEAL_TAIL 320
#define SEAL_STAGES 2
#define SEAL_SMEM ((size_t)SEAL_STAGES * 32 * SEAL_STRIDE + 32 * SEAL_TAIL)
__device__ __forceinline__ uint64_t sm64u(const uint8_t* base, uint32_t off) {
    const uint32_t al = off & ~7u, s = (off & 7u) * 8;
    const uint64_t lo = *(const uint64_t*)(base + al), hi = *(const uint64_t*)(base + al + 8);
    return (lo >> s) | ((hi << 1) << (63 - s));
}
__device__ __forceinline__ void cp_async16(void* smem_dst, const void* gsrc) {
    const uint32_t d = (uint32_t)__cvta_generic_to_shared(smem_dst);
    asm volatile("cp.async.cg.shared.global [%0], [%1], 16;\n" ::"r"(d), "l"(gsrc) : "memory");
}
__device__ __forceinline__ void cp_async_commit() { asm volatile("cp.async.commit_group;\n" ::: "memory"); }
template <int N> __device__ __forceinline__ void cp_async_wait() { asm volatile("cp.async.wait_group %0;\n" ::"n"(N) : "memory"); }

#ifdef TF_KERNELS_LZ4
// ... 97 lines not shown
```

### transferia_b200/csrc/kernels_str.cuh

```cuda
#pragma once
#include "device_types.cuh"
#include "kernels_encode.cuh"
#include "kernels_fmt.cuh"

namespace tfk {

__device__ __forceinline__ uint32_t str_len(const DCol& c, const uint32_t* sel, uint64_t j, uint64_t n, uint64_t& r) {
    if (j >= n) { r = 0; return 0xffffffffu; }
    r = sel ? sel[j] : j;
    if (c.out_kind == OK_TOSTR) { CountSink cs; cs.n = 0; fmt_value(cs, c, r); return cs.n; }
    if (!row_valid(c, r)) return 0;
    return c.offsets[r + 1] - c.offsets[r];
}

#define TF_STR_GROUP 4
#ifdef TF_KERNELS_STR
__global__ void __launch_bounds__(TF_STR_THREADS) k_str_sizes(EncodeArgs a) {
    __shared__ uint32_t sm[33];
    const DCol c = a.cols[a.slots[blockIdx.y]];
    const uint64_t n = a.st->n_kept;
    const uint64_t jg = (uint64_t)blockIdx.x * TF_STR_TILE * TF_STR_GROUP;
    if (jg >= n) return;
    uint32_t Ls[TF_STR_GROUP];
#pragma unroll
    for (int g = 0; g < TF_STR_GROUP; g++) { uint64_t r; Ls[g] = str_len(c, a.sel, jg + (uint64_t)g * TF_STR_TILE + threadIdx.x, n, r); }
#pragma unroll
    for (int g = 0; g < TF_STR_GROUP; g++) {
        uint32_t tot; block_excl_scan(Ls[g] != 0xffffffffu ? Ls[g] + (a.columnar ? 0 : varint_len(Ls[g])) : 0u, &tot, sm);
        if (threadIdx.x == 0 && jg + (uint64_t)g * TF_STR_TILE < n) a.tile_sum[(size_t)c.str_slot * a.ntiles_cap + blockIdx.x * TF_STR_GROUP + g] = tot;
        __syncthreads();
    }
}
#endif

__device__ __forceinline__ uint32_t str_find_row(const uint32_t* ex, uint32_t x) {
    uint32_t lo = 0, hi = TF_STR_TILE;
#pragma unroll
    for (int it = 0; it < 8; it++) { const uint32_t mid = (lo + hi) >> 1; if (ex[mid] <= x) lo = mid; else hi = mid; }
    return lo;
}
#ifdef TF_KERNELS_STR
__global__ void __launch_bounds__(TF_STR_THREADS) k_encode_str_plain(EncodeArgs a) {
    __shared__ uint32_t sm[33];
    __shared__ uint32_t s_ex[TF_STR_GROUP][TF_STR_TILE + 1];
    __shared__ uint32_t s_src[TF_STR_GROUP][TF_STR_TILE];
    __shared__ uint64_t s_tb[TF_STR_GROUP];
    const DCol c = a.cols[a.slots[blockIdx.y]];
    if (c.out_kind == OK_TOSTR) return;
    const uint64_t n = a.st->n_kept;
    const uint64_t jg = (uint64_t)blockIdx.x * TF_STR_TILE * TF_STR_GROUP;
    if (jg >= n) return;
    const uint32_t vlb = a.columnar ? 0u : 1u;
    uint32_t Ls[TF_STR_GROUP]; uint64_t Rs[TF_STR_GROUP]; uint32_t src[TF_STR_GROUP];
#pragma unroll
    for (int g = 0; g < TF_STR_GROUP; g++) Ls[g] = str_len(c, a.sel, jg + (uint64_t)g * TF_STR_TILE + threadIdx.x, n, Rs[g]);
#pragma unroll
    for (int g = 0; g < TF_STR_GROUP; g++) src[g] = (Ls[g] != 0xffffffffu && Ls[g]) ? c.offsets[Rs[g]] : 0u;
#pragma unroll
    for (int g = 0; g < TF_STR_GROUP; g++) {
        const bool have = Ls[g] != 0xffffffffu;
        uint32_t tot; const uint32_t ex = block_excl_scan(have ? Ls[g] + (vlb ? varint_len(Ls[g]) : 0) : 0u, &tot, sm);
        const uint64_t j0 = jg + (uint64_t)g * TF_STR_TILE;
        const uint64_t tb = j0 < n ? a.tile_base[(size_t)c.str_slot * a.ntiles_cap + blockIdx.x * TF_STR_GROUP + g] : 0;
        if (a.columnar && have) ((uint32_t*)(a.raw + c.offs_off))[j0 + threadIdx.x] = (uint32_t)(tb + ex);
        s_ex[g][threadIdx.x] = ex; s_src[g][threadIdx.x] = src[g];
        if (threadIdx.x == 0) { s_ex[g][TF_STR_TILE] = tot; s_tb[g] = tb; }
        __syncthreads();
    }
    const uint32_t hsh = ((uint32_t)(uintptr_t)c.heap & 3);
    const uint32_t* hw = (const uint32_t*)(c.heap - hsh);
#pragma unroll 1
    for (int g = 0; g < TF_STR_GROUP; g++) {
        const uint32_t* ex_ = s_ex[g]; const uint32_t* src_ = s_src[g];
        const uint32_t tot = ex_[TF_STR_TILE];
        if (!tot) continue;
        uint8_t* gdst = a.raw + c.out_off + s_tb[g];
        const uint32_t m = (uint32_t)((uintptr_t)gdst & 3);
        const uint32_t T = (m + tot + 3) >> 2;
        uint8_t* dst0 = gdst - m;
        for (uint32_t t = threadIdx.x; t < T; t += TF_STR_THREADS) {
            const int32_t sb = (int32_t)(4 * t) - (int32_t)m;
            const uint32_t x0 = sb < 0 ? 0u : (uint32_t)sb;
            uint32_t r = str_find_row(ex_, x0);
            uint32_t pe = ex_[r + 1], pl = pe - ex_[r];
            uint32_t plen = pl, vl = 0;
            if (vlb) { vl = pl < 129 ? 1 : (pl < 16386 ? 2 : (pl < 2097155 ? 3 : (pl < 268435460 ? 4 : 5))); plen = pl - vl; }
            const uint32_t k0 = x0 - ex_[r];
            if (sb >= 0 && (uint32_t)sb + 4 <= pe && k0 >= vl) {
                const uint32_t so = src_[r] + (k0 - vl) + hsh; const uint32_t sh = (so & 3) * 8;
                const uint32_t w0 = __ldg(hw + (so >> 2)); uint32_t val = w0;
                if (sh) val = __funnelshift_r(w0, __ldg(hw + (so >> 2) + 1), sh);
                *(uint32_t*)(dst0 + 4 * (size_t)t) = val;
                continue;
            }
            uint32_t val = 0, mask = 0;
#pragma unroll
            for (int b = 0; b < 4; b++) {
                const int32_t xs = sb + b;
                if (xs < 0 || (uint32_t)xs >= tot) continue;
                const uint32_t x = (uint32_t)xs;
                while (x >= pe) { r++; pe = ex_[r + 1]; pl = pe - ex_[r]; if (vlb) { vl = pl < 129 ? 1 : (pl < 16386 ? 2 : (pl < 2097155 ? 3 : (pl < 268435460 ? 4 : 5))); plen = pl - vl; } else plen = pl; }
                const uint32_t k = x - ex_[r];
                uint32_t byte;
                if (k < vl) { const uint32_t v = plen >> (7 * k); byte = (v & 0x7f) | ((v >> 7) ? 0x80u : 0u); }
                else byte = c.heap[src_[r] + (k - vl)];
                val |= byte << (8 * b); mask |= 1u << b;
            }
            uint8_t* dst = dst0 + 4 * (size_t)t;
            if (mask == 15) *(uint32_t*)dst = val;
            else { for (int b = 0; b < 4; b++) if ((mask >> b) & 1) dst[b] = (uint8_t)(val >> (8 * b)); }
        }
    }
}
#endif

#ifdef TF_KERNELS_STR
__global__ void __launch_bounds__(TF_STR_THREADS) k_encode_str(EncodeArgs a) {
    __shared__ uint32_t sm[33];
    __shared__ __align__(16) uint8_t stage[TF_STR_STAGE + 8];
    const DCol c = a.cols[a.slots[blockIdx.y]];
    if (c.out_kind != OK_TOSTR) return;
    const uint64_t n = a.st->n_kept;
    const uint64_t j0 = (uint64_t)blockIdx.x * TF_STR_TILE;
    if (j0 >= n) return;
    uint64_t R; const uint32_t L = str_len(c, a.sel, j0 + threadIdx.x, n, R);
    const bool tostr = c.out_kind == OK_TOSTR;
    const uint8_t* s = (L != 0xffffffffu && L && !tostr) ? c.heap + c.offsets[R] : nullptr;
    if (tostr && c.nullable && !a.columnar && L != 0xffffffffu) a.raw[c.null_off + j0 + threadIdx.x] = 0;
    uint32_t tot; const uint32_t ex = block_excl_scan(L != 0xffffffffu ? L + (a.columnar ? 0 : varint_len(L)) : 0u, &tot, sm);
    const uint64_t tb = a.tile_base[(size_t)c.str_slot * a.ntiles_cap + blockIdx.x];
    uint8_t* gdst = a.raw + c.out_off + tb;
    if (a.columnar && L != 0xffffffffu) ((uint32_t*)(a.raw + c.offs_off))[j0 + threadIdx.x] = (uint32_t)(tb + ex);
    const bool staged = tot <= TF_STR_STAGE;
    uint8_t* o = staged ? stage + ex : gdst + ex;
    if (L != 0xffffffffu) {
        if (!a.columnar) {
            uint32_t v = L;
            while (v >= 0x80) { *o++ = (uint8_t)(v | 0x80); v >>= 7; }
            *o++ = (uint8_t)v;
        }
        if (tostr) { MemSink ms; ms.p = o; fmt_value(ms, c, R); o = ms.p; }
        uint32_t nb = tostr ? 0 : L;
        const uint32_t sh = ((uint32_t)(uintptr_t)s & 3) * 8;
        const uint32_t* sw = (const uint32_t*)((uintptr_t)s & ~(uintptr_t)3);
        while (nb) {
            const uint32_t take = nb < 16 ? nb : 16;
            const uint32_t need = (take + (sh >> 3) + 3) >> 2;
            uint32_t w0 = __ldg(sw), w1 = need > 1 ? __ldg(sw + 1) : 0, w2 = need > 2 ? __ldg(sw + 2) : 0, w3 = need > 3 ? __ldg(sw + 3) : 0, w4 = need > 4 ? __ldg(sw + 4) : 0;
            if (sh) { w0 = __funnelshift_r(w0, w1, sh); w1 = __funnelshift_r(w1, w2, sh); w2 = __funnelshift_r(w2, w3, sh); w3 = __funnelshift_r(w3, w4, sh); }
            const uint32_t ww[4] = {w0, w1, w2, w3};
#pragma unroll
            for (int q = 0; q < 4; q++) {
#pragma unroll
                for (int b = 0; b < 4; b++) if ((uint32_t)(4 * q + b) < take) o[4 * q + b] = (uint8_t)(ww[q] >> (8 * b));
            }
            o += take; sw += 4; nb -= take;
        }
    }
    if (!staged) return;
    __syncthreads();
    const uint32_t m = (uint32_t)((uintptr_t)gdst & 3);
    const uint32_t T = (m + tot + 3) >> 2;
    uint8_t* dst0 = gdst - m;
    const uint32_t* sw = (const uint32_t*)stage;
    for (uint32_t t = threadIdx.x; t < T; t += TF_STR_THREADS) {
        const uint32_t wcur = sw[t], wprev = t ? sw[t - 1] : 0;
        const uint32_t val = m ? __funnelshift_r(wprev, wcur, 8 * (4 - m)) : wcur;
        const int32_t sb = (int32_t)(4 * t) - (int32_t)m;
        uint8_t* dst = dst0 + 4 * (size_t)t;
        if (sb >= 0 && (uint32_t)sb + 4 <= tot) *(uint32_t*)dst = val;
        else {
#pragma unroll
            for (int b = 0; b < 4; b++) { const int32_t x = sb + b; if (x >= 0 && (uint32_t)x < tot) dst[b] = (uint8_t)(val >> (8 * b)); }
        }
    }
}
#endif


}
```

### transferia_b200/csrc/launch.hpp

```cpp
#pragma once
#include <cuda_runtime.h>
#include "kernels_encode.cuh"
#include "kernels_str.cuh"
#include "kernels_mask.cuh"
#include "kernels_lz4.cuh"
#include "kernels_csv.cuh"
#include "kernels_json_in.cuh"
#include "kernels_n2f.cuh"
#include "kernels_dbz.cuh"
#include "kernels_json_out.cuh"
#include "kernels_deflate.cuh"
namespace tfk {
void launch_k_strictify(dim3 grid, dim3 block, size_t smem, cudaStream_t s, StrictArgs a);
void launch_k_filter(dim3 grid, dim3 block, size_t smem, cudaStream_t s, FilterArgs a);
void launch_k_scan_blockcnt(dim3 grid, dim3 block, size_t smem, cudaStream_t s, const uint32_t* blockcnt, uint32_t* blockoff, uint32_t nblocks, DState* st);
void launch_k_collect_errors(dim3 grid, dim3 block, size_t smem, cudaStream_t s, const uint8_t* errcode, const uint16_t* errstep, uint64_t nrows, DevRowErr* out, unsigned long long* counter, unsigned long long cap);
void launch_k_compact_sel(dim3 grid, dim3 block, size_t smem, cudaStream_t s, const uint8_t* keep, const uint32_t* blockoff, uint64_t nrows, uint32_t* sel);
void launch_k_layout_scan(dim3 grid, dim3 block, size_t smem, cudaStream_t s, LayoutArgs a);
void launch_k_layout_finish(dim3 grid, dim3 block, size_t smem, cudaStream_t s, LayoutArgs a);
void launch_k_layout_columnar(dim3 grid, dim3 block, size_t smem, cudaStream_t s, LayoutArgs a, ColRegions* regions);
void launch_k_encode_fixed(dim3 grid, dim3 block, size_t smem, cudaStream_t s, EncodeArgs a);
void launch_k_pack_validity(dim3 grid, dim3 block, size_t smem, cudaStream_t s, EncodeArgs a);
void launch_k_measure(dim3 grid, dim3 block, size_t smem, cudaStream_t s, MeasureArgs a);
void launch_k_str_sizes(dim3 grid, dim3 block, size_t smem, cudaStream_t s, EncodeArgs a);
void launch_k_encode_str_plain(dim3 grid, dim3 block, size_t smem, cudaStream_t s, EncodeArgs a);
void launch_k_encode_str(dim3 grid, dim3 block, size_t smem, cudaStream_t s, EncodeArgs a);
void launch_k_mask_encode(dim3 grid, dim3 block, size_t smem, cudaStream_t s, MaskArgs a);
void launch_k_shard_ids(dim3 grid, dim3 block, size_t smem, cudaStream_t s, ShardArgs a);
void launch_k_lz4_frames(dim3 grid, dim3 block, size_t smem, cudaStream_t s, Lz4Args a);
void launch_k_frame_seal(dim3 grid, dim3 block, size_t smem, cudaStream_t s, FrameArgs a);
void launch_k_csv_count_nl(dim3 grid, dim3 block, size_t smem, cudaStream_t s, const uint8_t* text, uint64_t len, uint32_t* blk_cnt, const uint32_t* endbits);
void launch_k_csv_line_index(dim3 grid, dim3 block, size_t smem, cudaStream_t s, const uint8_t* text, uint64_t len, const uint32_t* blk_off, uint32_t* line_end, const uint32_t* endbits);
void launch_k_widen_lens(dim3 grid, dim3 block, size_t smem, cudaStream_t s, const LensSrc* src, uint64_t nrows, uint32_t* out);
void launch_k_csv_pass1(dim3 grid, dim3 block, size_t smem, cudaStream_t s, CsvArgs a);
void launch_k_csv_offsets(dim3 grid, dim3 block, size_t smem, cudaStream_t s, const uint32_t* span_len, uint64_t nrows, uint32_t* offsets , uint64_t* col_total);
void launch_k_offsets_sum(dim3 grid, dim3 block, size_t smem, cudaStream_t s, const uint32_t* span_len, uint64_t nrows, uint32_t nchunks, uint64_t* chunk_sum);
void launch_k_offsets_chunks(dim3 grid, dim3 block, size_t smem, cudaStream_t s, uint64_t* chunk_sum, uint32_t nchunks, uint64_t* col_total);
void launch_k_offsets_write(dim3 grid, dim3 block, size_t smem, cudaStream_t s, const uint32_t* span_len, uint64_t nrows, uint32_t nchunks, const uint64_t* chunk_base, const uint64_t* col_total, uint32_t* offsets);
void launch_k_csv_pass2(dim3 grid, dim3 block, size_t smem, cudaStream_t s, CsvCopyArgs a);
void launch_k_json_mark_msgs(dim3 grid, dim3 block, size_t smem, cudaStream_t s, const uint64_t* msg_end, uint32_t nmsgs, uint32_t* bits);
void launch_k_json_count_nonempty(dim3 grid, dim3 block, size_t smem, cudaStream_t s, const uint8_t* text, const uint32_t* line_end, uint64_t nlines, uint32_t* blk_cnt);
void launch_k_json_rank(dim3 grid, dim3 block, size_t smem, cudaStream_t s, const uint8_t* text, const uint32_t* line_end, uint64_t nlines, const uint32_t* blk_off, uint32_t* rank);
void launch_k_json_msg_first(dim3 grid, dim3 block, size_t smem, cudaStream_t s, const uint64_t* msg_end, uint32_t nmsgs, const uint32_t* line_end, uint64_t nlines, const uint32_t* rank, uint32_t* msg_rank0);
void launch_k_json_pass1(dim3 grid, dim3 block, size_t smem, cudaStream_t s, JsnArgs a);
void launch_k_json_pass2(dim3 grid, dim3 block, size_t smem, cudaStream_t s, JsnWriteArgs w);
void launch_k_n2f_sizes(dim3 grid, dim3 block, size_t smem, cudaStream_t s, N2fArgs a);
void launch_k_n2f_write(dim3 grid, dim3 block, size_t smem, cudaStream_t s, N2fArgs a);
void launch_k_dbz_pass1(dim3 grid, dim3 block, size_t smem, cudaStream_t s, DbzArgs a);
void launch_k_dbz_pass2(dim3 grid, dim3 block, size_t smem, cudaStream_t s, DbzWriteArgs w);
void launch_k_json_sizes(dim3 grid, dim3 block, size_t smem, cudaStream_t s, JsonArgs a);
void launch_k_json_write(dim3 grid, dim3 block, size_t smem, cudaStream_t s, JsonArgs a);
cudaError_t dbz_kernels_init();
void launch_k_deflate_chunks(dim3 grid, dim3 block, size_t smem, cudaStream_t s, DeflateArgs a);
void launch_k_deflate_finish(dim3 grid, dim3 block, size_t smem, cudaStream_t s, DeflateArgs a);
cudaError_t deflate_kernels_init();
cudaError_t lz4_kernels_init();
}
```

### transferia_b200/csrc/tfgpu.cu

```cuda
#include <cuda_runtime.h>
#include <algorithm>
#include <chrono>
#include <cstdio>
#include <cstdlib>
#include <cstring>
#include <memory>
#include <string>
#include <vector>

#include "../../include/tfgpu.h"
#include "../../include/tfgpu_sink.h"
#include "plan.hpp"
#include "device_types.cuh"
#include "launch.hpp"
#include "host_internal.hpp"

using namespace tfk;

namespace {

struct CudaError { cudaError_t e; const char* what; };
#define CK(x) do { cudaError_t _e = (x); if (_e != cudaSuccess) throw CudaError{_e, #x}; } while (0)

inline size_t align_up(size_t v, size_t a) { return (v + a - 1) / a * a; }

struct DevBuf {
    uint8_t* p = nullptr; size_t cap = 0;
    DevBuf() = default;
    DevBuf(const DevBuf&) = delete;
    DevBuf& operator=(const DevBuf&) = delete;
    ~DevBuf() { if (p) cudaFree(p); }
    void ensure(size_t n) {
        if (n <= cap) return;
        if (p) { CK(cudaDeviceSynchronize()); CK(cudaFree(p)); p = nullptr; cap = 0; }
        size_t want = align_up(n + n / 8 + 4096, 1 << 20);
        CK(cudaMalloc(&p, want)); cap = want;
    }
};

struct Layout {
    size_t slack, end = 0;
    explicit Layout(size_t slack_ = 0) : slack(slack_) {}
    size_t take(size_t bytes) { const size_t at = end; end += align_up(std::max<size_t>(bytes + slack, 1), 256); return at; }
    size_t total() const { return end; }
};

struct PlanDev {
    tfplan::Plan plan;
    DevBuf consts;
    DTerm* d_terms = nullptr; uint32_t* d_expr_off = nullptr; DFilterStep* d_fsteps = nullptr; uint8_t* d_blob = nullptr;
    uint8_t* d_col_headers = nullptr; uint32_t* d_col_header_off = nullptr;
    JsonCol* d_jcols = nullptr; uint8_t* d_jnames = nullptr; size_t jnames_len = 0;
    JsonCol* d_sjcols = nullptr; JsonCol* d_scsvcols = nullptr; uint8_t* d_snames = nullptr;
    int32_t* d_fixed_slots = nullptr; int32_t* d_str_slots = nullptr; int32_t* d_mask_slots = nullptr; int32_t* d_out_cols = nullptr;
    MaskKey* d_mask_keys = nullptr;
    int n_fsteps = 0, n_fixed_slots = 0, n_str = 0, n_mask_cols = 0, n_tostr = 0;
    std::vector<int32_t> fixed_slots, str_slots, mask_slot_cols, mask_slot_key;
    std::vector<int> col_out_kind, col_out_w, col_str_slot, col_mask_slot, col_nullable;
    ShardCol* d_shard_cols = nullptr;
    std::vector<JsonCol> h_sjcols;
    DevBuf dbz_consts; std::string dbz_opts_key; DbzEmitArgs dbz{};
};

}

struct tfgpu_engine {
    int device = 0;
    cudaStream_t own_stream = nullptr, stream = nullptr;
    cudaStream_t side_stream = nullptr; cudaEvent_t ev_fork = nullptr, ev_tail = nullptr;
    bool tail_pending = false; uint64_t tail_nrows = 0, tail_nframes_max = 0; const void* tail_plan = nullptr;
    uint64_t* d_tail = nullptr;
    std::string last_error;
    uint64_t launches = 0;
    uint32_t frame_bytes = LZ_MAX_FRAME;
    int sm_count = 132;
    std::vector<std::unique_ptr<PlanDev>> plans;
    DevBuf in_arena, work, raw, wire, strict_stage, lens_arena, lens_arena2, csv_text, csv_stage, json_msgs, n2f_stage, n2f_heap, off_scratch;
    DState* d_state = nullptr; DCol* d_cols = nullptr; size_t d_cols_cap = 0;
    int32_t* d_call_slots = nullptr; ColRegions* d_regions = nullptr; size_t d_call_cap = 0;
    uint8_t *keep = nullptr, *errcode = nullptr; uint16_t* errstep = nullptr; uint32_t *blockcnt = nullptr, *blockoff = nullptr, *sel = nullptr;
    uint32_t* tile_sum = nullptr; uint64_t* tile_base = nullptr; uint64_t* col_bytes = nullptr; uint32_t* comp_size = nullptr; uint64_t* wire_off = nullptr; unsigned long long* frame_pfx = nullptr;
    uint64_t last_nrows = 0; bool last_has_filter = false, last_has_sharder = false; int last_wire_fmt = 0;
    uint8_t* pinned = nullptr; size_t pinned_cap = 0;
    DevBuf err_list;
    DevBuf sel_stage; uint8_t* sel_host = nullptr; size_t sel_host_cap = 0; tfgpu_columnar* gather_pool = nullptr;
    uint64_t h2d_bytes = 0;
    DevBuf json_sizes, dbz_keysz, dbz_meta, dbz_old, dbz_msgsz, old_arena, part_ids;
    DevBuf defl_meta;
    DbzEmitArgs dbz{};
    unsigned long long* lz_phases = nullptr;
    void* work_json_sizes(uint64_t n) { json_sizes.ensure(n * 4 + 256); return json_sizes.p; }
    bool prof_on = false; std::vector<cudaEvent_t> prof_ev; std::vector<const char*> prof_names; int prof_n = 0;
    std::string prof_json;
    void prof_begin(const char* name, cudaStream_t s) {
        launches++;
        if (!prof_on) return;
        while ((int)prof_ev.size() < 2 * (prof_n + 1)) { cudaEvent_t ev; cudaEventCreate(&ev); prof_ev.push_back(ev); }
        if ((int)prof_names.size() <= prof_n) prof_names.resize(prof_n + 1);
        prof_names[prof_n] = name; cudaEventRecord(prof_ev[2 * prof_n], s);
    }
    void prof_end(cudaStream_t s) { if (!prof_on) return; cudaEventRecord(prof_ev[2 * prof_n + 1], s); prof_n++; }
};

struct tfgpu_result {
    uint64_t rows_in = 0, rows_out = 0, raw_len = 0, n_frames = 0, consumed = 0;
    std::vector<tf_rowerr> errs;
    uint8_t* bytes = nullptr; uint64_t bytes_len = 0; bool bytes_pinned = false;
    std::vector<uint32_t> selection;
    std::vector<uint8_t> meta_kinds; std::vector<uint32_t> meta_tx; std::vector<uint64_t> meta_lsn, meta_ct;
    std::vector<uint32_t> row_sizes;
    std::vector<uint32_t> key_sizes;
    std::vector<uint32_t> msg_sizes;
    std::vector<uint32_t> part_ids;
    tf_batch batch{}; std::vector<tf_col> cols; std::vector<uint8_t*> owned;
};

namespace {

void join_tail(tfgpu_engine* e) {
    if (!e->tail_pending) return;
    CK(cudaStreamWaitEvent(e->stream, e->ev_tail, 0));
    e->tail_pending = false;
}
int fail(tfgpu_engine* e, int code, const std::string& msg) { if (e) e->last_error = msg; return code; }
int cuda_fail(tfgpu_engine* e, const CudaError& c) {
    std::string m = std::string("CUDA error: ") + cudaGetErrorString(c.e) + " in " + c.what;
    cudaGetLastError();
    return fail(e, c.e == cudaErrorMemoryAllocation ? TF_E_RETRY_OOM : TF_E_RETRY_LAUNCH, m);
}

template <typename F> int on_device(tfgpu_engine* e, F&& body) {
    try {
        CK(cudaSetDevice(e->device));
        return body();
    } catch (const tfplan::FatalError& f) { return fail(e, f.code, f.what()); }
    catch (const CudaError& c) { return cuda_fail(e, c); }
    catch (const std::bad_alloc&) { return fail(e, TF_E_RETRY_OOM, "host allocation failed"); }
    catch (const std::exception& x) { return fail(e, TF_E_FATAL_CONFIG, x.what()); }
}

tfj::ValuePtr parse_opts_json(const char* js) {
    try { return tfj::parse(js); }
    catch (const std::runtime_error& x) { throw tfplan::FatalError(TF_E_FATAL_CONFIG, std::string("opts_json: ") + x.what()); }
}

int in_width(int tf) {
    switch (tf) {
    case TF_INT8: case TF_UINT8: case TF_BOOLEAN: return 1;
    case TF_INT16: case TF_UINT16: return 2;
    case TF_INT32: case TF_UINT32: case TF_FLOAT: return 4;
    case TF_INT64: case TF_UINT64: case TF_DOUBLE: case TF_INTERVAL: case TF_DATE: case TF_DATETIME: case TF_TIMESTAMP: return 8;
    }
    return 0;
}

struct ConstImage {
    Layout L; std::vector<uint8_t> bytes;
    size_t add(const void* src, size_t n) { const size_t at = L.take(n); bytes.resize(L.total()); if (n) std::memcpy(bytes.data() + at, src, n); return at; }
    uint8_t* upload(DevBuf& dst) { dst.ensure(bytes.size()); CK(cudaMemcpy(dst.p, bytes.data(), bytes.size(), cudaMemcpyHostToDevice)); return dst.p; }
};

void upload_plan(PlanDev& pd) {
    const tfplan::Plan& pl = pd.plan;
    const size_t nc = pl.in_schema.size();
    pd.col_mask_slot.assign(nc, -1);
    std::vector<MaskKey> keys;
    for (size_t m = 0; m < pl.masks.size(); m++) {
        keys.push_back(make_mask_key((const uint8_t*)pl.masks[m].salt.data(), pl.masks[m].salt.size()));
        for (int c : pl.masks[m].cols) {
            if (pd.col_mask_slot[c] >= 0) throw tfplan::FatalError(TF_E_FATAL_UNSUPPORTED, "column masked twice in one chain");
            pd.col_mask_slot[c] = (int)m;
        }
    }
    pd.col_out_kind.assign(nc, 0); pd.col_out_w.assign(nc, 0); pd.col_str_slot.assign(nc, -1);
    pd.col_nullable.assign(nc, 0);
    for (size_t k = 0; k < pl.out_cols.size(); k++) {
        const size_t c = (size_t)pl.out_cols[k];
        const int tf = pl.in_schema[c].tf;
        int kind, w;
        if (pd.col_mask_slot[c] >= 0) {
            kind = OK_MASK; w = 65;
        } else if (pl.tostr_col.size() > c && pl.tostr_col[c]) { kind = OK_TOSTR; w = 0; }
        else if (pl.todt_col.size() > c && pl.todt_col[c]) { kind = OK_TODT; w = 4; }
        else switch (tf) {
            case TF_BOOLEAN: kind = OK_BOOL; w = 1; break;
            case TF_DATE: kind = OK_DATE; w = 2; break;
            case TF_DATETIME: kind = OK_DATETIME; w = 4; break;
            case TF_TIMESTAMP: kind = OK_TS64; w = 8; break;
            case TF_BYTES: case TF_UTF8: case TF_ANY: kind = OK_STR; w = 0; break;
            default: kind = OK_COPY; w = in_width(tf);
        }
        pd.col_out_kind[c] = kind; pd.col_out_w[c] = w;
        const bool nullable = !pl.out_schema[k].required; pd.col_nullable[c] = nullable ? 1 : 0;
        if (kind == OK_STR || kind == OK_TOSTR) { pd.col_str_slot[c] = (int)pd.str_slots.size(); pd.str_slots.push_back((int32_t)c); }
        else if (kind == OK_MASK) { pd.mask_slot_cols.push_back((int32_t)c); }
        else pd.fixed_slots.push_back((int32_t)c);
        if (nullable && kind == OK_TODT) pd.fixed_slots.push_back((int32_t)c | TF_SLOT_ZEROMAP);
        else if (nullable && kind != OK_MASK && kind != OK_TOSTR) pd.fixed_slots.push_back((int32_t)c | TF_SLOT_NULLMAP);
    }
    if (pd.str_slots.size() > 65535) throw tfplan::FatalError(TF_E_FATAL_UNSUPPORTED, "more than 65535 String columns (one grid row per column)");
    std::vector<JsonCol> jcols; std::vector<uint8_t> jnames;
    for (size_t k = 0; k < pl.out_cols.size(); k++) {
        JsonCol jc; std::memset(&jc, 0, sizeof jc); jc.col = pl.out_cols[k]; jc.name_off = (int32_t)jnames.size(); jc.name_len = (int32_t)pl.out_schema[k].name.size();
        jnames.insert(jnames.end(), pl.out_schema[k].name.begin(), pl.out_schema[k].name.end());
        const int rt = pl.out_schema[k].tf; jc.result_tf = rt;
        jc.ch_class = (rt == TF_ANY || rt == TF_BYTES || rt == TF_UTF8) ? JC_STRING : rt == TF_DATE ? JC_DATE : rt == TF_DATETIME ? JC_DATETIME : rt == TF_TIMESTAMP ? JC_DT64 : JC_OTHER;
        jc.prec = 6;
        jcols.push_back(jc);
    }
    pd.jnames_len = jnames.size();
    std::vector<JsonCol> sjcols, scsvcols; std::vector<uint8_t> snames;
    {
        std::vector<size_t> order(pl.out_cols.size()); for (size_t k = 0; k < order.size(); k++) order[k] = k;
        std::stable_sort(order.begin(), order.end(), [&](size_t a, size_t b) { return pl.out_schema[a].name < pl.out_schema[b].name; });
        for (size_t j = 0; j < order.size(); j++) {
            const size_t k = order[j]; JsonCol jc = jcols[k]; jc.pad0 = (int32_t)k;
            const std::string q = host_json_quote_nohtml(pl.out_schema[k].name) + ":";
            jc.name_off = (int32_t)snames.size(); jc.name_len = (int32_t)q.size(); snames.insert(snames.end(), q.begin(), q.end());
            sjcols.push_back(jc);
        }
        for (size_t k = 0; k < jcols.size(); k++) { JsonCol jc = jcols[k]; jc.pad0 = (int32_t)k; scsvcols.push_back(jc); }
        pd.h_sjcols = sjcols;
    }
    std::vector<DTerm> terms; std::vector<uint32_t> expr_off(1, 0); std::vector<DFilterStep> fsteps;
    for (size_t f = 0; f < pl.filters.size(); f++) {
        DFilterStep st; st.expr_begin = (int32_t)expr_off.size() - 1; st.nexpr = (int32_t)pl.filters[f].exprs.size(); st.step_index = pl.filter_step_index[f];
        st.flags = (pl.filters[f].is_skip ? 1 : 0) | (pl.filters[f].pass_all ? 2 : 0);
        if (pl.filters[f].is_skip) { st.expr_begin = pl.filters[f].kind_mask; st.nexpr = 0; }
        for (auto& ex : pl.filters[f].exprs) {
            for (auto& t : ex) { DTerm d; static_assert(sizeof(DTerm) == sizeof(tfplan::DTerm), "DTerm mismatch"); std::memcpy(&d, &t, sizeof d); terms.push_back(d); }
            expr_off.push_back((uint32_t)terms.size());
        }
        fsteps.push_back(st);
    }
    pd.n_fsteps = (int)fsteps.size(); pd.n_fixed_slots = (int)pd.fixed_slots.size(); pd.n_str = (int)pd.str_slots.size(); pd.n_mask_cols = (int)pd.mask_slot_cols.size();
    pd.n_tostr = 0; for (size_t c = 0; c < pd.col_out_kind.size(); c++) if (pd.col_out_kind[c] == OK_TOSTR) pd.n_tostr++;
    std::vector<ShardCol> shcols;
    for (size_t k = 0; k < pl.shard_cols.size(); k++) shcols.push_back(ShardCol{pl.shard_cols[k], pl.shard_form[k], 0, 0});
    const std::vector<int32_t> oc(pl.out_cols.begin(), pl.out_cols.end());
    ConstImage ci;
    const size_t o_terms = ci.add(terms.data(), terms.size() * sizeof(DTerm)), o_expr_off = ci.add(expr_off.data(), expr_off.size() * 4),
                 o_fsteps = ci.add(fsteps.data(), fsteps.size() * sizeof(DFilterStep)), o_blob = ci.add(pl.blob.data(), pl.blob.size()),
                 o_hdr = ci.add(pl.col_headers.data(), pl.col_headers.size()), o_hdr_off = ci.add(pl.col_header_off.data(), pl.col_header_off.size() * 4),
                 o_fixed = ci.add(pd.fixed_slots.data(), pd.fixed_slots.size() * 4), o_str = ci.add(pd.str_slots.data(), pd.str_slots.size() * 4),
                 o_mask = ci.add(pd.mask_slot_cols.data(), pd.mask_slot_cols.size() * 4), o_keys = ci.add(keys.data(), keys.size() * sizeof(MaskKey)),
                 o_out = ci.add(oc.data(), oc.size() * 4), o_jcols = ci.add(jcols.data(), jcols.size() * sizeof(JsonCol)), o_jnames = ci.add(jnames.data(), jnames.size()),
                 o_sjcols = ci.add(sjcols.data(), sjcols.size() * sizeof(JsonCol)), o_scsv = ci.add(scsvcols.data(), scsvcols.size() * sizeof(JsonCol)),
                 o_snames = ci.add(snames.data(), snames.size()), o_shard = ci.add(shcols.data(), shcols.size() * sizeof(ShardCol));
    uint8_t* P = ci.upload(pd.consts);
    pd.d_terms = (DTerm*)(P + o_terms); pd.d_expr_off = (uint32_t*)(P + o_expr_off); pd.d_fsteps = (DFilterStep*)(P + o_fsteps); pd.d_blob = P + o_blob;
    pd.d_col_headers = P + o_hdr; pd.d_col_header_off = (uint32_t*)(P + o_hdr_off);
    pd.d_fixed_slots = (int32_t*)(P + o_fixed); pd.d_str_slots = (int32_t*)(P + o_str); pd.d_mask_slots = (int32_t*)(P + o_mask); pd.d_mask_keys = (MaskKey*)(P + o_keys);
    pd.d_out_cols = (int32_t*)(P + o_out); pd.d_jcols = (JsonCol*)(P + o_jcols); pd.d_jnames = P + o_jnames;
    pd.d_sjcols = (JsonCol*)(P + o_sjcols); pd.d_scsvcols = (JsonCol*)(P + o_scsv); pd.d_snames = P + o_snames; pd.d_shard_cols = (ShardCol*)(P + o_shard);
}

struct Sizes { uint64_t raw_bound, n_frames_max, wire_bound; uint32_t ntiles_cap, nblocks; };

Sizes compute_sizes(const tfgpu_engine* e, const PlanDev& pd, const tf_batch* in, bool columnar = false, bool json = false) {
    const tfplan::Plan& pl = pd.plan; const uint64_t n = in->nrows;
    uint64_t raw = 64 + pl.col_headers.size();
    for (int oc : pl.out_cols) {
        const size_t c = (size_t)oc;
        if (pd.col_nullable[c]) raw += n;
        bool n2f = false; for (int q : pl.n2f_cols) if ((size_t)q == c) n2f = true;
        if (pd.col_out_kind[c] == OK_STR) raw += (n2f ? 6 : 1) * in->cols[c].heap_len + 5 * n;
        else if (pd.col_out_kind[c] == OK_TOSTR) raw += (in_width(in->cols[c].type) ? 40 * n : (n2f ? 36 : 6) * in->cols[c].heap_len + 8 * n) + 5 * n;
        else raw += (uint64_t)pd.col_out_w[c] * n;
        if (columnar) raw += 8 * n + 4 * (n + 1) + n / 8 + 6 * 16 + (pd.col_out_kind[c] == OK_MASK ? 64 * n : 0);
        if (json) raw += (uint64_t)(pl.in_schema[c].name.size() + 4 + 48) * n + (in_width(in->cols[c].type) ? 0 : (n2f ? 36 : 6) * in->cols[c].heap_len);
    }
    Sizes s;
    s.raw_bound = raw + 256;
    s.n_frames_max = (raw + e->frame_bytes - 1) / e->frame_bytes + 1;
    s.wire_bound = s.n_frames_max * (uint64_t)(LZ_HDR + lz4_bound(e->frame_bytes)) + 1024;
    s.ntiles_cap = (uint32_t)((n + TF_STR_TILE - 1) / TF_STR_TILE + 1);
    s.nblocks = (uint32_t)((n + 255) / 256 + 1);
    return s;
}


static void launch_offsets(tfgpu_engine* e, const uint32_t* d_len, uint64_t nrows, uint32_t nslots, uint32_t* d_off, uint64_t* d_tot, cudaStream_t s) {
    const uint32_t nchunks = (uint32_t)((nrows + CSV_OFF_CHUNK - 1) / CSV_OFF_CHUNK);
    if (!nchunks || !nslots) { launch_k_csv_offsets(nslots ? nslots : 1, 1024, 0, s, d_len, nrows, d_off, d_tot); return; }
    e->off_scratch.ensure((size_t)nslots * nchunks * 8 + 256);
    uint64_t* cs = (uint64_t*)e->off_scratch.p;
    e->prof_begin("k_offsets_sum", s); launch_k_offsets_sum(dim3(nchunks, nslots), 1024, 0, s, d_len, nrows, nchunks, cs); e->prof_end(s);
    e->prof_begin("k_offsets_chunks", s); launch_k_offsets_chunks(nslots, 32, 0, s, cs, nchunks, d_tot); e->prof_end(s);
    e->prof_begin("k_offsets_write", s); launch_k_offsets_write(dim3(nchunks, nslots), 1024, 0, s, d_len, nrows, nchunks, cs, d_tot, d_off); e->prof_end(s);
}

struct Heaps { std::vector<uint64_t> total, base; };
Heaps size_heaps(tfgpu_engine* e, const uint32_t* d_len, uint64_t nrows, uint32_t k, uint32_t* d_off, uint64_t* d_tot, uint64_t* d_base,
                 DevBuf& heap, const char* too_big) {
    cudaStream_t s = e->stream;
    launch_offsets(e, d_len, nrows, k, d_off, d_tot, s);
    Heaps h{std::vector<uint64_t>(k), std::vector<uint64_t>(k)};
    CK(cudaMemcpyAsync(h.total.data(), d_tot, (size_t)k * 8, cudaMemcpyDeviceToHost, s)); CK(cudaStreamSynchronize(s));
    uint64_t run = 0; for (uint32_t i = 0; i < k; i++) { h.base[i] = run; run += align_up(h.total[i], 16); }
    if (run >= (1ull << 32)) throw tfplan::FatalError(TF_E_FATAL_ARG, too_big);
    heap.ensure(run + 256);
    CK(cudaMemcpyAsync(d_base, h.base.data(), (size_t)k * 8, cudaMemcpyHostToDevice, s));
    return h;
}

DCol make_dcol(const tf_col& ic, int type) {
    DCol d; std::memset(&d, 0, sizeof d);
    d.type = type; d.in_w = in_width(type); d.str_slot = -1; d.mask_slot = -1;
    d.values = (const uint8_t*)ic.values; d.validity = ic.validity; d.offsets = ic.offsets; d.heap = ic.heap; d.aux = (const uint8_t*)ic.aux;
    return d;
}

void ensure_d_cols(tfgpu_engine* e, size_t nc) {
    if (e->d_cols_cap >= nc) return;
    if (e->d_cols) CK(cudaFree(e->d_cols));
    CK(cudaMalloc(&e->d_cols, sizeof(DCol) * nc)); e->d_cols_cap = nc;
}

#define TF_WIRE_COLUMNAR_INTERNAL 100
uint32_t grid_cap(const tfgpu_engine* e, uint32_t tiles_upper, uint32_t nslots, uint32_t waves) {
    const uint32_t want = ((uint32_t)e->sm_count * 6u * waves + nslots - 1) / (nslots ? nslots : 1);
    return std::max(1u, std::min(tiles_upper, std::max(want, 8u)));
}

void run_deflate(tfgpu_engine* e, const uint8_t* text, uint64_t total, bool zlib) {
    cudaStream_t s = e->stream;
    const uint64_t nch = (total + DF_CHUNK - 1) / DF_CHUNK;
    if (nch >= (1ull << 32)) throw tfplan::FatalError(TF_E_FATAL_ARG, "row text too large to compress in one call");
    e->wire.ensure(total + nch * DF_CHUNK_OVERHEAD + 64);
    Layout L;
    const size_t o_pfx = L.take(nch * 8), o_sums = L.take(nch * 8), o_ticket = L.take(4);
    e->defl_meta.ensure(L.total());
    uint8_t* M = e->defl_meta.p;
    CK(cudaMemsetAsync(M + o_pfx, 0, nch * 8, s)); CK(cudaMemsetAsync(M + o_ticket, 0, 4, s));
    DeflateArgs da{text, total, e->wire.p, (unsigned long long*)(M + o_pfx), (uint32_t*)(M + o_sums), (uint32_t*)(M + o_ticket), (uint32_t)nch, zlib ? 1 : 0, e->d_state};
    if (nch) {
        const uint32_t grid = (uint32_t)std::min<uint64_t>(nch, (uint64_t)e->sm_count * 2);
        e->prof_begin("k_deflate_chunks", s); launch_k_deflate_chunks(grid, DF_THREADS, df_smem().total, s, da); e->prof_end(s);
    }
    e->prof_begin("k_deflate_finish", s); launch_k_deflate_finish(1, 1024, 0, s, da); e->prof_end(s);
}

void run_chain(tfgpu_engine* e, PlanDev& pd, const tf_batch* in, const tf_col* dev_cols, const uint8_t* dev_kinds, int wire_fmt, const uint8_t* pre_err = nullptr) {
    const bool columnar = wire_fmt == TF_WIRE_COLUMNAR_INTERNAL;
    const tfplan::Plan& pl = pd.plan;
    const size_t nc = pl.in_schema.size(); const uint64_t n = in->nrows;
    const int wire_base = wire_fmt == TF_WIRE_COLUMNAR_INTERNAL ? wire_fmt : (wire_fmt & 0xff);
    const bool dbz = wire_base == TF_WIRE_DEBEZIUM;
    const bool ser = wire_base == TF_WIRE_SER_JSON || wire_base == TF_WIRE_SER_CSV || dbz;
    const bool json_rows = wire_base == TF_WIRE_CH_JSONEACHROW || ser;
    if (ser) for (size_t c = 0; c < nc; c++) if (pd.col_out_kind[c] == OK_TOSTR && pl.in_schema[c].tf == TF_ANY)
        throw tfplan::FatalError(TF_E_FATAL_UNSUPPORTED, "serializer sinks after convert_to_string on an `any` column are not handled on the device");
    const Sizes sz = compute_sizes(e, pd, in, columnar, json_rows);
    cudaStream_t s = e->stream;
    if (e->tail_pending && !(wire_fmt == TF_WIRE_CH_NATIVE_LZ4 && n == e->tail_nrows && (const void*)&pd == e->tail_plan && sz.n_frames_max == e->tail_nframes_max)) join_tail(e);
    const size_t nslot_alloc = (size_t)(pd.n_str > 0 ? pd.n_str : 1);
    Layout W;
    const size_t o_keep = W.take(n), o_errcode = W.take(n), o_errstep = W.take(2 * n), o_blockcnt = W.take(sz.nblocks * 4), o_blockoff = W.take(sz.nblocks * 4),
                 o_sel = W.take(n * 4), o_tile_sum = W.take(nslot_alloc * sz.ntiles_cap * 4), o_tile_base = W.take(nslot_alloc * sz.ntiles_cap * 8),
                 o_comp = W.take(sz.n_frames_max * 4), o_wire_off = W.take(sz.n_frames_max * 8), o_pfx = W.take(sz.n_frames_max * 8), o_col_bytes = W.take(nslot_alloc * 8);
    e->work.ensure(W.total());
    uint8_t* w = e->work.p;
    e->keep = w + o_keep; e->errcode = w + o_errcode; e->errstep = (uint16_t*)(w + o_errstep);
    e->blockcnt = (uint32_t*)(w + o_blockcnt); e->blockoff = (uint32_t*)(w + o_blockoff); e->sel = (uint32_t*)(w + o_sel);
    e->tile_sum = (uint32_t*)(w + o_tile_sum); e->tile_base = (uint64_t*)(w + o_tile_base);
    e->comp_size = (uint32_t*)(w + o_comp); e->wire_off = (uint64_t*)(w + o_wire_off); e->frame_pfx = (unsigned long long*)(w + o_pfx); e->col_bytes = (uint64_t*)(w + o_col_bytes);
    e->raw.ensure(sz.raw_bound);
    const bool lz = wire_fmt == TF_WIRE_CH_NATIVE_LZ4;
    if (lz) e->wire.ensure(sz.wire_bound);
    ensure_d_cols(e, nc);
    std::vector<DCol> hc(nc); std::vector<StrictCol> strict;
    for (size_t c = 0; c < nc; c++) {
        const tf_col& ic = dev_cols[c];
        int ctype = ic.type;
        if (ic.type != pl.in_schema[c].tf) {
            const int st = ic.type, dt = pl.in_schema[c].tf;
            const bool s_num = in_width(st) && st != TF_INTERVAL && st != TF_DATE && st != TF_DATETIME && st != TF_TIMESTAMP;
            if ((st == TF_UTF8 && dt == TF_BYTES) || (st == TF_BYTES && dt == TF_UTF8)) ctype = dt;
            else if (s_num && in_width(dt) && !(st == TF_FLOAT && dt == TF_DOUBLE) && !(st == TF_BOOLEAN && dt == TF_DOUBLE)) { strict.push_back(StrictCol{(const uint8_t*)ic.values, nullptr, ic.validity, st, dt, (int32_t)c, 0}); ctype = dt; }
            else throw tfplan::FatalError(TF_E_FATAL_ARG, "column " + std::to_string(c) + ": a " + std::to_string(st) + " value cannot be strictified to the plan's column type on the device");
        }
        DCol& d = hc[c]; d = make_dcol(ic, ctype);
        d.out_kind = pd.col_out_kind[c]; d.out_w = pd.col_out_w[c];
        if (columnar && d.out_kind == OK_TODT) d.out_w = 8;
        else if (columnar && d.out_kind != OK_STR && d.out_kind != OK_MASK && d.out_kind != OK_TOSTR) { d.out_kind = OK_COPY; d.out_w = d.in_w; }
        d.nullable = pd.col_nullable[c]; d.str_slot = pd.col_str_slot[c]; d.mask_slot = pd.col_mask_slot[c];
        if (n) {
            if (d.in_w && !d.values) throw tfplan::FatalError(TF_E_FATAL_ARG, "column " + std::to_string(c) + ": values pointer is NULL");
            if (!d.in_w && !d.offsets) throw tfplan::FatalError(TF_E_FATAL_ARG, "column " + std::to_string(c) + ": offsets pointer is NULL");
        }
    }
    if (!pre_err) e->prof_n = 0;
    const uint16_t* pre_term = nullptr;
    if (!strict.empty() && n) {
        Layout S;
        const size_t o_desc = S.take(strict.size() * sizeof(StrictCol)), o_err = S.take(n), o_term = S.take(2 * n);
        std::vector<size_t> o_val(strict.size());
        for (size_t k = 0; k < strict.size(); k++) o_val[k] = S.take((size_t)in_width(strict[k].dst_tf) * n + 16);
        e->strict_stage.ensure(S.total() + 256);
        uint8_t* B = e->strict_stage.p;
        for (size_t k = 0; k < strict.size(); k++) { strict[k].dst = B + o_val[k]; hc[strict[k].col].values = B + o_val[k]; }
        CK(cudaMemcpyAsync(B + o_desc, strict.data(), strict.size() * sizeof(StrictCol), cudaMemcpyHostToDevice, s));
        if (pre_err) CK(cudaMemcpyAsync(B + o_err, pre_err, n, cudaMemcpyDeviceToDevice, s)); else CK(cudaMemsetAsync(B + o_err, 0, n, s));
        StrictArgs sa{(const StrictCol*)(B + o_desc), (int)strict.size(), n, B + o_err, (uint16_t*)(B + o_term)};
        e->prof_begin("k_strictify", s); launch_k_strictify((uint32_t)((n + 255) / 256), 256, 0, s, sa); e->prof_end(s);
        pre_err = B + o_err; pre_term = (const uint16_t*)(B + o_term);
    }
    CK(cudaMemcpyAsync(e->d_cols, hc.data(), sizeof(DCol) * nc, cudaMemcpyHostToDevice, s));
    CK(cudaMemsetAsync(e->d_state, 0, sizeof(DState), s));
    if (!pl.n2f_cols.empty() && n) {
        const size_t k2 = pl.n2f_cols.size();
        Layout S;
        const size_t o_which = S.take(k2 * 4), o_len = S.take(k2 * n * 4), o_off = S.take(k2 * (n + 1) * 4), o_tot = S.take(k2 * 8 + 8), o_base = S.take(k2 * 8 + 8), o_err = S.take(n);
        e->n2f_stage.ensure(S.total() + 256);
        uint8_t* B = e->n2f_stage.p;
        std::vector<int32_t> which(pl.n2f_cols.begin(), pl.n2f_cols.end());
        CK(cudaMemcpyAsync(B + o_which, which.data(), k2 * 4, cudaMemcpyHostToDevice, s));
        if (pre_err) CK(cudaMemcpyAsync(B + o_err, pre_err, n, cudaMemcpyDeviceToDevice, s)); else CK(cudaMemsetAsync(B + o_err, 0, n, s));
        N2fArgs na{e->d_cols, (const int32_t*)(B + o_which), dev_kinds, n, (uint32_t*)(B + o_len), (const uint32_t*)(B + o_off), nullptr, (const uint64_t*)(B + o_base), B + o_err};
        e->prof_begin("k_n2f_sizes", s); launch_k_n2f_sizes(dim3((uint32_t)((n + 127) / 128), (uint32_t)k2), 128, 0, s, na); e->prof_end(s);
        const Heaps h = size_heaps(e, (const uint32_t*)(B + o_len), n, (uint32_t)k2, (uint32_t*)(B + o_off), (uint64_t*)(B + o_tot), (uint64_t*)(B + o_base),
                                   e->n2f_heap, "number_to_float: a rewritten column exceeds 4 GiB");
        na.heap = e->n2f_heap.p;
        e->prof_begin("k_n2f_write", s); launch_k_n2f_write(dim3((uint32_t)((n + 127) / 128), (uint32_t)k2), 128, 0, s, na); e->prof_end(s);
        for (size_t k = 0; k < k2; k++) { DCol& d = hc[pl.n2f_cols[k]]; d.offsets = (const uint32_t*)(B + o_off) + k * (n + 1); d.heap = e->n2f_heap.p + h.base[k]; }
        CK(cudaMemcpyAsync(e->d_cols, hc.data(), sizeof(DCol) * nc, cudaMemcpyHostToDevice, s));
        pre_err = B + o_err;
    }
    const bool sink_guard = dev_kinds && wire_fmt != TF_WIRE_COLUMNAR_INTERNAL && wire_base != TF_WIRE_DEBEZIUM;
    const bool has_filter = pd.n_fsteps > 0 || pre_err || sink_guard;
    e->last_nrows = n; e->last_has_filter = has_filter; e->last_wire_fmt = wire_fmt;
    const uint32_t nb = (uint32_t)((n + 255) / 256);
    if (has_filter && n) {
        FilterArgs fa{e->d_cols, dev_kinds, n, pd.d_fsteps, pd.n_fsteps, pd.d_expr_off, pd.d_terms, pd.d_blob, e->keep, e->errcode, e->errstep, e->blockcnt, e->d_state, pre_err, pre_term, sink_guard ? 1 : 0};
        e->prof_begin("k_filter", s); launch_k_filter(nb, 256, 0, s, fa); e->prof_end(s);
        e->prof_begin("k_scan_blockcnt", s); launch_k_scan_blockcnt(1, 1024, 0, s, e->blockcnt, e->blockoff, nb, e->d_state); e->prof_end(s);
        e->prof_begin("k_compact_sel", s); launch_k_compact_sel(nb, 256, 0, s, e->keep, e->blockoff, n, e->sel); e->prof_end(s);
    }
    const uint32_t* sel = (has_filter && n) ? e->sel : nullptr;
    const uint32_t ntiles = (uint32_t)((n + TF_STR_TILE - 1) / TF_STR_TILE);
    const uint32_t str_gx = std::max(1u, (ntiles + TF_STR_GROUP - 1) / TF_STR_GROUP);
    EncodeArgs ea{e->d_cols, pd.d_str_slots, sel, e->d_state, e->raw.p, e->tile_sum, e->tile_base, sz.ntiles_cap, columnar ? 1 : 0};
    if (!has_filter || !n) {
        DState init; std::memset(&init, 0, sizeof init); init.n_kept = n;
        CK(cudaMemcpyAsync(e->d_state, &init, sizeof init, cudaMemcpyHostToDevice, s));
    }
    if (pl.has_sharder && n) {
        e->part_ids.ensure(n * 4 + 256);
        ShardArgs sa{e->d_cols, pd.d_shard_cols, (int)pl.shard_cols.size(), pd.d_mask_keys, sel, e->d_state, pl.shards, (uint32_t*)e->part_ids.p};
        e->prof_begin("k_shard_ids", s); launch_k_shard_ids(nb, 256, 0, s, sa); e->prof_end(s);
    }
    e->last_has_sharder = pl.has_sharder;
    if (json_rows) {
        const uint32_t jt = (uint32_t)((n + TF_JSON_TILE - 1) / TF_JSON_TILE);
        JsonArgs ja{e->d_cols, ser ? (wire_base == TF_WIRE_SER_CSV ? pd.d_scsvcols : pd.d_sjcols) : pd.d_jcols, (int)pl.out_cols.size(), ser ? pd.d_snames : pd.d_jnames, pd.d_mask_keys, sel, e->d_state, e->raw.p,
                    (uint32_t*)e->work_json_sizes(n), e->tile_sum, e->tile_base, e->col_bytes,
                    dbz ? 3 : ser ? (wire_base == TF_WIRE_SER_JSON ? 1 : 2) : 0, (uint32_t)(((wire_fmt & TF_WIRE_F_CLOSING_NEWLINE) ? TF_SER_NL : 0) | ((wire_fmt & TF_WIRE_F_ANY_AS_STRING) ? TF_SER_AAS : 0)), e->errcode, e->errstep, DbzEmitArgs{}};
        if (dbz) { ja.jcols = pd.d_sjcols; e->dbz_keysz.ensure(n * 4 + 256); e->dbz_msgsz.ensure(n * 28 + 256); ja.dz = e->dbz; ja.dz.key_size = (uint32_t*)e->dbz_keysz.p; ja.dz.msg_size = (uint32_t*)e->dbz_msgsz.p; }
        if (ser && !has_filter && n) { CK(cudaMemsetAsync(e->errcode, 0, n, s)); CK(cudaMemsetAsync(e->errstep, 0, 2 * n, s)); }
        if (jt) { e->prof_begin("k_json_sizes", s); launch_k_json_sizes(jt, TF_JSON_TILE, 0, s, ja); e->prof_end(s); }
        LayoutArgs lj{e->d_cols, 0, pd.d_out_cols, pd.d_str_slots, 1, e->tile_sum, e->tile_base, sz.ntiles_cap, pd.d_col_headers, pd.d_col_header_off,
                      e->raw.p, e->d_state, n, 1, e->frame_bytes, e->col_bytes};
        e->prof_begin("k_layout_scan", s); launch_k_layout_scan(1, 1024, 0, s, lj); e->prof_end(s);
        uint64_t json_total = 0;
        {
            CK(cudaMemcpyAsync(&json_total, e->col_bytes, 8, cudaMemcpyDeviceToHost, s)); CK(cudaStreamSynchronize(s));
            e->raw.ensure(json_total + 256); ja.raw = e->raw.p;
        }
        e->prof_begin("k_json_write", s); launch_k_json_write(jt ? jt : 1, TF_JSON_TILE, 0, s, ja); e->prof_end(s);
        if (ser && (wire_fmt & (TF_WIRE_F_GZIP | TF_WIRE_F_ZLIB))) run_deflate(e, e->raw.p, n ? json_total : 0, (wire_fmt & TF_WIRE_F_ZLIB) != 0);
        CK(cudaGetLastError());
        return;
    }
    if (pd.n_str && ntiles) { e->prof_begin("k_str_sizes", s); launch_k_str_sizes(dim3(str_gx, pd.n_str), TF_STR_THREADS, 0, s, ea); e->prof_end(s); }
    LayoutArgs la{e->d_cols, (int)pl.out_cols.size(), pd.d_out_cols, pd.d_str_slots, pd.n_str, e->tile_sum, e->tile_base, sz.ntiles_cap, pd.d_col_headers, pd.d_col_header_off,
                  e->raw.p, e->d_state, n, 1, e->frame_bytes, e->col_bytes};
    if (pd.n_str) { e->prof_begin("k_layout_scan", s); launch_k_layout_scan(pd.n_str, 1024, 0, s, la); e->prof_end(s); }
    if (!columnar) {
        e->prof_begin("k_layout_finish", s); launch_k_layout_finish(1, 256, 0, s, la); e->prof_end(s);
        if (n) {
            if (pd.n_fixed_slots) {
                const uint32_t gx = grid_cap(e, (uint32_t)((2 * n + 2 + TF_FIX_TILE_WORDS - 1) / TF_FIX_TILE_WORDS), (uint32_t)pd.n_fixed_slots, 6);
                EncodeArgs fa = ea; fa.slots = pd.d_fixed_slots;
                e->prof_begin("k_encode_fixed", s); launch_k_encode_fixed(dim3(gx, pd.n_fixed_slots), 256, 0, s, fa); e->prof_end(s);
            }
            if (pd.n_str) { e->prof_begin("k_encode_str_plain", s); launch_k_encode_str_plain(dim3(str_gx, pd.n_str), TF_STR_THREADS, 0, s, ea); e->prof_end(s); }
            if (pd.n_str && pd.n_tostr) { e->prof_begin("k_encode_str", s); launch_k_encode_str(dim3(ntiles, pd.n_str), TF_STR_THREADS, 0, s, ea); e->prof_end(s); }
            if (pd.n_mask_cols) {
                MaskArgs ma{e->d_cols, pd.d_mask_slots, pd.d_mask_keys, sel, e->d_state, e->raw.p, 0};
                e->prof_begin("k_mask_encode", s); launch_k_mask_encode(dim3((uint32_t)((n + 127) / 128), pd.n_mask_cols), 128, 0, s, ma); e->prof_end(s);
            }
        }
    } else {
        const size_t no = pl.out_cols.size();
        if (e->d_call_cap < no) {
            if (e->d_call_slots) { CK(cudaFree(e->d_call_slots)); CK(cudaFree(e->d_regions)); }
            CK(cudaMalloc(&e->d_call_slots, sizeof(int32_t) * 3 * no)); CK(cudaMalloc(&e->d_regions, sizeof(ColRegions) * no)); e->d_call_cap = no;
        }
        std::vector<int32_t> fixed, valid;
        for (int oc : pl.out_cols) {
            const DCol& d = hc[oc];
            if (d.out_kind == OK_COPY || d.out_kind == OK_TODT) fixed.push_back(oc);
            const bool fresh = d.out_kind == OK_MASK || d.out_kind == OK_TOSTR || d.out_kind == OK_TODT;
            if (!fresh && d.aux) fixed.push_back(oc | TF_SLOT_AUX);
            if (!fresh && d.validity) valid.push_back(oc);
        }
        std::vector<int32_t> both(fixed); both.insert(both.end(), valid.begin(), valid.end());
        if (!both.empty()) CK(cudaMemcpyAsync(e->d_call_slots, both.data(), both.size() * 4, cudaMemcpyHostToDevice, s));
        e->prof_begin("k_layout_columnar", s); launch_k_layout_columnar(1, 256, 0, s, la, e->d_regions); e->prof_end(s);
        if (n) {
            if (!fixed.empty()) {
                const uint32_t gx = grid_cap(e, (uint32_t)((2 * n + 2 + TF_FIX_TILE_WORDS - 1) / TF_FIX_TILE_WORDS), (uint32_t)fixed.size(), 6);
                EncodeArgs fa = ea; fa.slots = e->d_call_slots;
                e->prof_begin("k_encode_fixed", s); launch_k_encode_fixed(dim3(gx, (uint32_t)fixed.size()), 256, 0, s, fa); e->prof_end(s);
            }
            if (!valid.empty()) {
                EncodeArgs va = ea; va.slots = e->d_call_slots + fixed.size();
                e->prof_begin("k_pack_validity", s); launch_k_pack_validity(dim3((uint32_t)((n / 8 + 256) / 256), (uint32_t)valid.size()), 256, 0, s, va); e->prof_end(s);
            }
            if (pd.n_str) { e->prof_begin("k_encode_str_plain", s); launch_k_encode_str_plain(dim3(str_gx, pd.n_str), TF_STR_THREADS, 0, s, ea); e->prof_end(s); }
            if (pd.n_str && pd.n_tostr) { e->prof_begin("k_encode_str", s); launch_k_encode_str(dim3(ntiles, pd.n_str), TF_STR_THREADS, 0, s, ea); e->prof_end(s); }
            if (pd.n_mask_cols) {
                MaskArgs ma{e->d_cols, pd.d_mask_slots, pd.d_mask_keys, sel, e->d_state, e->raw.p, 1};
                e->prof_begin("k_mask_encode", s); launch_k_mask_encode(dim3((uint32_t)((n + 127) / 128), pd.n_mask_cols), 128, 0, s, ma); e->prof_end(s);
            }
        }
    }
    if (lz) {
        Lz4Args za{e->raw.p, e->d_state, e->wire.p, e->comp_size, e->wire_off, e->frame_pfx, e->d_tail, e->frame_bytes, e->lz_phases};
        const size_t smem = lz_smem(e->frame_bytes).total;
        const uint32_t per_sm = (uint32_t)std::max<size_t>(1, std::min<size_t>(LZ_CTAS_PER_SM, (227 * 1024) / (smem + 1024)));
        const uint32_t grid = (uint32_t)std::min<uint64_t>(sz.n_frames_max, (uint64_t)e->sm_count * per_sm);
        join_tail(e);
        CK(cudaMemsetAsync(e->frame_pfx, 0, sz.n_frames_max * 8, s));
        e->prof_begin("k_lz4_frames", s); launch_k_lz4_frames(grid, LZ_THREADS, smem, s, za); e->prof_end(s);
        FrameArgs fa{e->comp_size, e->wire_off, e->wire.p, e->d_tail};
        cudaStream_t s3 = e->side_stream;
        CK(cudaEventRecord(e->ev_fork, s)); CK(cudaStreamWaitEvent(s3, e->ev_fork, 0));
        e->prof_begin("k_frame_seal", s3); launch_k_frame_seal((uint32_t)((sz.n_frames_max + 31) / 32), 32, SEAL_SMEM, s3, fa); e->prof_end(s3);
        CK(cudaEventRecord(e->ev_tail, s3));
        e->tail_pending = true; e->tail_nrows = n; e->tail_plan = (const void*)&pd; e->tail_nframes_max = sz.n_frames_max;
    }
    CK(cudaGetLastError());
}

}


static bool wire_is_ser(int wire_fmt) {
    const int b = wire_fmt & 0xff;
    return (b == TF_WIRE_SER_JSON || b == TF_WIRE_SER_CSV) && (wire_fmt & ~(0xff | TF_WIRE_F_CLOSING_NEWLINE | TF_WIRE_F_ANY_AS_STRING | TF_WIRE_F_GZIP | TF_WIRE_F_ZLIB)) == 0 &&
           (wire_fmt & (TF_WIRE_F_GZIP | TF_WIRE_F_ZLIB)) != (TF_WIRE_F_GZIP | TF_WIRE_F_ZLIB);
}
static bool wire_known(int wire_fmt) { return wire_fmt == TF_WIRE_CH_NATIVE || wire_fmt == TF_WIRE_CH_NATIVE_LZ4 || wire_fmt == TF_WIRE_CH_JSONEACHROW || wire_is_ser(wire_fmt); }

extern "C" {

const char* tfgpu_version(void) { return "tfgpu 0.1.0 sm_90a"; }

int tfgpu_engine_create(const char* cfg_json, const int* device_ids, int n_devices, tfgpu_engine** out) {
    if (!out) return TF_E_FATAL_ARG;
    *out = nullptr;
    int ndev = 0;
    if (cudaGetDeviceCount(&ndev) != cudaSuccess || ndev == 0) { cudaGetLastError(); return TF_E_FATAL_NODEVICE; }
    if (n_devices > 1) return TF_E_FATAL_ARG;
    auto e = std::make_unique<tfgpu_engine>();
    e->device = (n_devices == 1 && device_ids) ? device_ids[0] : 0;
    if (e->device < 0 || e->device >= ndev) return TF_E_FATAL_ARG;
    try {
        if (cfg_json && *cfg_json) {
            auto cfg = tfj::parse(cfg_json);
            double fb = cfg->get_num("frame_bytes", LZ_MAX_FRAME);
            if (fb < 1024 || fb > LZ_MAX_FRAME || ((uint32_t)fb & 15)) return TF_E_FATAL_CONFIG;
            e->frame_bytes = (uint32_t)fb;
        }
        CK(cudaSetDevice(e->device));
        cudaDeviceProp prop; CK(cudaGetDeviceProperties(&prop, e->device));
        e->sm_count = prop.multiProcessorCount;
        CK(cudaStreamCreateWithFlags(&e->own_stream, cudaStreamNonBlocking));
        e->stream = e->own_stream;
        CK(cudaStreamCreateWithFlags(&e->side_stream, cudaStreamNonBlocking));
        CK(cudaEventCreateWithFlags(&e->ev_tail, cudaEventDisableTiming));
        CK(cudaMalloc(&e->d_tail, 64)); CK(cudaMemset(e->d_tail, 0, 64));
        CK(cudaEventCreateWithFlags(&e->ev_fork, cudaEventDisableTiming));
        CK(cudaMalloc(&e->d_state, sizeof(DState)));
        CK(lz4_kernels_init()); CK(dbz_kernels_init()); CK(deflate_kernels_init());
    } catch (const CudaError& c) { return c.e == cudaErrorMemoryAllocation ? TF_E_RETRY_OOM : TF_E_RETRY_LAUNCH; }
    catch (const std::exception&) { return TF_E_FATAL_CONFIG; }
    *out = e.release();
    return TF_OK;
}

int tfgpu_engine_destroy(tfgpu_engine* e) {
    if (!e) return TF_E_FATAL_ARG;
    cudaSetDevice(e->device);
    cudaDeviceSynchronize();
    if (e->d_state) cudaFree(e->d_state);
    if (e->d_cols) cudaFree(e->d_cols);
    if (e->d_call_slots) { cudaFree(e->d_call_slots); cudaFree(e->d_regions); }
    if (e->d_tail) cudaFree(e->d_tail);
    if (e->lz_phases) cudaFree(e->lz_phases);
    if (e->pinned) cudaFreeHost(e->pinned);
    if (e->sel_host) cudaFreeHost(e->sel_host);
    if (e->gather_pool) tfgpu_columnar_destroy(e->gather_pool);
    for (auto ev : e->prof_ev) cudaEventDestroy(ev);
    if (e->ev_fork) cudaEventDestroy(e->ev_fork);
    if (e->ev_tail) cudaEventDestroy(e->ev_tail);
    if (e->side_stream) cudaStreamDestroy(e->side_stream);
    if (e->own_stream) cudaStreamDestroy(e->own_stream);
    delete e;
    return TF_OK;
}

const char* tfgpu_last_error(const tfgpu_engine* e) { return e ? e->last_error.c_str() : "null engine"; }
uint64_t tfgpu_engine_launch_count(const tfgpu_engine* e) { return e ? e->launches : 0; }

int tfgpu_profile_enable(tfgpu_engine* e, int on) { if (!e) return TF_E_FATAL_ARG; e->prof_on = on != 0; e->prof_n = 0; return TF_OK; }

const char* tfgpu_profile_read(tfgpu_engine* e) {
    if (!e) return nullptr;
    on_device(e, [&] { join_tail(e); return TF_OK; });
    cudaStreamSynchronize(e->stream);
    std::string j = "[";
    for (int i = 0; i < e->prof_n; i++) {
        float ms = 0; cudaEventElapsedTime(&ms, e->prof_ev[2 * i], e->prof_ev[2 * i + 1]);
        char b[160]; snprintf(b, sizeof b, "%s{\"name\":\"%s\",\"ms\":%.6f}", i ? "," : "", e->prof_names[i], ms); j += b;
    }
    e->prof_json = j + "]";
    return e->prof_json.c_str();
}

int tfgpu_engine_set_stream(tfgpu_engine* e, void* cuda_stream) {
    if (!e) return TF_E_FATAL_ARG;
    if (e->tail_pending) { cudaSetDevice(e->device); cudaStreamSynchronize(e->side_stream); e->tail_pending = false; }
    e->stream = cuda_stream ? (cudaStream_t)cuda_stream : e->own_stream;
    return TF_OK;
}

int tfgpu_plan(tfgpu_engine* e, const char* ns, const char* name, const char* schema_json, const char* transformers_json,
               const char* sink_json, int* plan_id) {
    if (!e || !schema_json || !plan_id || !name) return TF_E_FATAL_ARG;
    return on_device(e, [&] {
        auto pd = std::make_unique<PlanDev>();
        pd->plan = tfplan::build_plan(ns ? ns : "", name, schema_json, transformers_json ? transformers_json : "", sink_json ? sink_json : "");
        upload_plan(*pd);
        e->plans.push_back(std::move(pd));
        *plan_id = (int)e->plans.size() - 1;
        return TF_OK;
    });
}

const char* tfgpu_plan_describe(tfgpu_engine* e, int plan_id) {
    if (!e || plan_id < 0 || plan_id >= (int)e->plans.size()) return nullptr;
    return e->plans[plan_id]->plan.describe.c_str();
}

static const uint8_t* stage_input(tfgpu_engine* e, const tf_batch* in, std::vector<tf_col>& dev, DevBuf* arena_opt = nullptr);
int tfgpu_push_encode_resident(tfgpu_engine* e, int plan_id, int wire_fmt, const tf_batch* in) {
    if (!e || !in || plan_id < 0 || plan_id >= (int)e->plans.size()) return TF_E_FATAL_ARG;
    PlanDev& pd = *e->plans[plan_id];
    if (!pd.plan.has_sink) return fail(e, TF_E_FATAL_CONFIG, "plan was built without a sink");
    if (in->mem != TF_MEM_DEVICE) return fail(e, TF_E_FATAL_ARG, "tfgpu_push_encode_resident needs a TF_MEM_DEVICE batch");
    if (in->ncols != pd.plan.in_schema.size()) return fail(e, TF_E_FATAL_ARG, "batch column count does not match the plan schema");
    if (wire_fmt != TF_WIRE_CH_NATIVE && wire_fmt != TF_WIRE_CH_NATIVE_LZ4) return fail(e, TF_E_FATAL_UNSUPPORTED, "wire format not implemented");
    if (in->nrows >= (1ull << 31)) return fail(e, TF_E_FATAL_ARG, "batch too large (>= 2^31 rows)");
    return on_device(e, [&] {
        std::vector<tf_col> dev; const uint8_t* dev_kinds = stage_input(e, in, dev);
        run_chain(e, pd, in, dev.data(), dev_kinds, wire_fmt);
        return TF_OK;
    });
}

int tfgpu_resident_stats(tfgpu_engine* e, uint64_t* rows_out, uint64_t* raw_bytes, uint64_t* wire_bytes, uint64_t* n_errors) {
    if (!e) return TF_E_FATAL_ARG;
    return on_device(e, [&] {
        join_tail(e);
        DState st; CK(cudaMemcpyAsync(&st, e->d_state, sizeof st, cudaMemcpyDeviceToHost, e->stream)); CK(cudaStreamSynchronize(e->stream));
        if (rows_out) *rows_out = st.n_kept; if (raw_bytes) *raw_bytes = st.raw_total;
        if (wire_bytes) *wire_bytes = e->last_wire_fmt == TF_WIRE_CH_NATIVE_LZ4 ? st.wire_total : st.raw_total;
        if (n_errors) *n_errors = st.n_errors;
        return TF_OK;
    });
}

int tfgpu_resident_fetch(tfgpu_engine* e, int what, uint8_t* dst, uint64_t cap) {
    if (!e || !dst) return TF_E_FATAL_ARG;
    return on_device(e, [&] {
        join_tail(e);
        DState st; CK(cudaMemcpyAsync(&st, e->d_state, sizeof st, cudaMemcpyDeviceToHost, e->stream)); CK(cudaStreamSynchronize(e->stream));
        const bool wire = what == 1 && e->last_wire_fmt == TF_WIRE_CH_NATIVE_LZ4;
        const uint64_t n = wire ? st.wire_total : st.raw_total;
        if (n > cap) return fail(e, TF_E_FATAL_ARG, "destination too small");
        CK(cudaMemcpyAsync(dst, wire ? e->wire.p : e->raw.p, n, cudaMemcpyDeviceToHost, e->stream)); CK(cudaStreamSynchronize(e->stream));
        return TF_OK;
    });
}

static void fetch_errors(tfgpu_engine* e, uint64_t n, tfgpu_result* r);
static void finish_wire(tfgpu_engine* e, uint64_t n, int wire_fmt, tfgpu_result* r);

int tfgpu_push_encode(tfgpu_engine* e, int plan_id, int wire_fmt, const tf_batch* in, tfgpu_result** out) {
    if (!e || !in || !out || plan_id < 0 || plan_id >= (int)e->plans.size()) return TF_E_FATAL_ARG;
    *out = nullptr;
    PlanDev& pd = *e->plans[plan_id];
    if (!wire_known(wire_fmt)) return fail(e, TF_E_FATAL_UNSUPPORTED, "wire format not implemented");
    if (!wire_is_ser(wire_fmt) && !pd.plan.has_sink) return fail(e, TF_E_FATAL_CONFIG, "plan was built without a sink");
    if (in->ncols != pd.plan.in_schema.size()) return fail(e, TF_E_FATAL_ARG, "batch column count does not match the plan schema");
    if (in->nrows >= (1ull << 31)) return fail(e, TF_E_FATAL_ARG, "batch too large (>= 2^31 rows)");
    return on_device(e, [&] {
        std::vector<tf_col> dev; const uint8_t* dev_kinds = stage_input(e, in, dev);
        run_chain(e, pd, in, dev.data(), dev_kinds, wire_fmt);
        auto r = std::make_unique<tfgpu_result>();
        finish_wire(e, in->nrows, wire_fmt, r.get());
        *out = r.release();
        return TF_OK;
    });
}

int tfgpu_push_encode_selective(tfgpu_engine* e, int plan_id, int wire_fmt, const tf_batch* in, int threads, tfgpu_result** out) {
    if (!e || !in || !out || plan_id < 0 || plan_id >= (int)e->plans.size()) return TF_E_FATAL_ARG;
    PlanDev& pd = *e->plans[plan_id];
    const tfplan::Plan& pl = pd.plan;
    const uint64_t n = in->nrows; const size_t nc = pl.in_schema.size();
    if (in->mem != TF_MEM_HOST || in->ncols != nc || pd.n_fsteps == 0 || n < 8192 || !wire_known(wire_fmt)) return tfgpu_push_encode(e, plan_id, wire_fmt, in, out);
    std::vector<uint8_t> pred(nc, 0);
    for (const auto& fs : pl.filters) for (const auto& ex : fs.exprs) for (const auto& t : ex) if (t.col >= 0 && (size_t)t.col < nc) pred[t.col] = 1;
    for (size_t c = 0; c < nc; c++) if (pred[c] && in->cols[c].type != pl.in_schema[c].tf) return tfgpu_push_encode(e, plan_id, wire_fmt, in, out);
    *out = nullptr;
    return on_device(e, [&] {
        join_tail(e);
        cudaStream_t s = e->stream;
        static const bool trace = std::getenv("TFGPU_SELECTIVE_TRACE") != nullptr;
        const auto t_0 = std::chrono::steady_clock::now();
        std::vector<tf_col> pc(in->cols, in->cols + nc);
        for (size_t c = 0; c < nc; c++) if (!pred[c]) { pc[c].values = nullptr; pc[c].validity = nullptr; pc[c].offsets = nullptr; pc[c].heap = nullptr; pc[c].aux = nullptr; pc[c].heap_len = 0; pc[c].flags = 0; }
        const tf_batch b1{n, (uint32_t)nc, TF_MEM_HOST, pc.data(), in->kinds};
        std::vector<tf_col> dev; const uint8_t* dev_kinds = stage_input(e, &b1, dev);
        std::vector<DCol> hc(nc);
        for (size_t c = 0; c < nc; c++) hc[c] = make_dcol(dev[c], pl.in_schema[c].tf);
// ... 898 lines not shown
```

### transferia_b200/csrc/tu_str.cu

```cuda
#define TF_KERNELS_STR
#include <cuda_runtime.h>
#include "kernels_str.cuh"
namespace tfk {
void launch_k_str_sizes(dim3 grid, dim3 block, size_t smem, cudaStream_t s, EncodeArgs a) { k_str_sizes<<<grid, block, smem, s>>>(a); }
void launch_k_encode_str_plain(dim3 grid, dim3 block, size_t smem, cudaStream_t s, EncodeArgs a) { k_encode_str_plain<<<grid, block, smem, s>>>(a); }
void launch_k_encode_str(dim3 grid, dim3 block, size_t smem, cudaStream_t s, EncodeArgs a) { k_encode_str<<<grid, block, smem, s>>>(a); }
}
```

Before: 1.079 billion.

## Fuse string sizing, layout scan and encoding into one persistent lookback kernel

For the native (non-columnar) path, the separate string-size, layout-scan, plain-encode and to-string encode kernels are replaced by a single persistent k_encode_str_native kernel. It hands out row groups by ticket and computes their output offsets with a decoupled lookback prefix sum. String data placement is precomputed per slot, so k_layout_finish can place string columns before their sizes are known. The lookback helper is shared across the LZ4, deflate and string kernels. This removes several launches and passes over string lengths, at the cost of serialized lookback chains and spin-waiting on a grid sized to occupancy.

```diff
diff --git a/transferia_b200/csrc/device_types.cuh b/transferia_b200/csrc/device_types.cuh
--- a/transferia_b200/csrc/device_types.cuh
+++ b/transferia_b200/csrc/device_types.cuh
@@ -53,6 +53,7 @@
     uint64_t n_frames;
     uint64_t wire_total;
     uint32_t frame_ticket;
+    uint32_t str_ticket;
     uint32_t pad;
 };
 
diff --git a/transferia_b200/csrc/kernels_deflate.cuh b/transferia_b200/csrc/kernels_deflate.cuh
--- a/transferia_b200/csrc/kernels_deflate.cuh
+++ b/transferia_b200/csrc/kernels_deflate.cuh
@@ -1,6 +1,7 @@
 #pragma once
 #include "device_types.cuh"
 #include "kernels_encode.cuh"
+#include "lookback.cuh"
 #include "deflate_sum.hpp"
 
 namespace tfk {
@@ -10,9 +11,6 @@
 #define DF_PPT (DF_CHUNK / DF_THREADS)
 #define DF_HASH_BITS 12
 #define DF_CHUNK_OVERHEAD 10
-#define DF_FLAG_AGG (1ull << 62)
-#define DF_FLAG_INCL (2ull << 62)
-#define DF_VAL_MASK ((1ull << 62) - 1)
 
 struct DfSmem { uint32_t data, dist, lenb, work, path, hist, lens, codes, sort, crct, total; };
 __host__ __device__ inline DfSmem df_smem() {
@@ -113,29 +111,6 @@
     cnt[0] = 0; uint32_t c = 0;
     for (int l = 1; l < 16; l++) { c = (c + cnt[l - 1]) << 1; next[l] = c; }
     for (int s = 0; s < n; s++) { const uint32_t l = lens[s]; codes[s] = l ? (uint16_t)(__brev(next[l]++) >> (32 - l)) : 0; }
-}
-
-__device__ __forceinline__ unsigned long long df_lookback(const DeflateArgs& a, uint32_t f, uint32_t lane) {
-    unsigned long long excl = 0;
-    int64_t base = (int64_t)f;
-    for (uint32_t spins = 0; base > 0;) {
-        const int64_t j = base - 1 - (int64_t)lane;
-        const unsigned long long v = j >= 0 ? *(volatile unsigned long long*)&a.pfx[j] : DF_FLAG_INCL;
-        const uint32_t fl = (uint32_t)(v >> 62);
-        const uint32_t incl = __ballot_sync(0xffffffffu, fl == 2), none = __ballot_sync(0xffffffffu, fl == 0);
-        const uint32_t upto = incl ? (uint32_t)__ffs((int)incl) - 1 : 31u;
-        const uint32_t need = upto == 31 ? 0xffffffffu : ((2u << upto) - 1);
-        if (none & need) {
-            if (++spins > (1u << 20)) { if (lane == 0) a.st->pad = 1; break; }
-            __nanosleep(100); continue;
-        }
-        unsigned long long part = lane <= upto ? (v & DF_VAL_MASK) : 0ull;
-#pragma unroll
-        for (int d = 16; d; d >>= 1) part += __shfl_xor_sync(0xffffffffu, part, d);
-        excl += part; base -= 32;
-        if (incl) break;
-    }
-    return excl;
 }
 
 __device__ __forceinline__ uint32_t df_block_xor(uint32_t v, uint32_t* red) {
@@ -417,12 +392,12 @@
                 uint8_t* ib = (uint8_t*)img; ib[nbytes - 2] = 0xff; ib[nbytes - 1] = 0xff;
             }
         }
-        if (tid == 0) *(volatile unsigned long long*)&a.pfx[f] = DF_FLAG_AGG | nbytes;
+        if (tid == 0) *(volatile unsigned long long*)&a.pfx[f] = LB_FLAG_AGG | nbytes;
         __syncthreads();
 
         if (warp == 0) {
-            const unsigned long long excl = df_lookback(a, f, lane);
-            if (lane == 0) { *(volatile unsigned long long*)&a.pfx[f] = DF_FLAG_INCL | (excl + nbytes); s_off = excl; }
+            const unsigned long long excl = lookback_excl(a.pfx, f, lane, a.st);
+            if (lane == 0) { *(volatile unsigned long long*)&a.pfx[f] = LB_FLAG_INCL | (excl + nbytes); s_off = excl; }
         }
         __syncthreads();
         uint8_t* G = a.out + (a.zlib ? sizeof(tfdf::ZLIB_HDR) : sizeof(tfdf::GZIP_HDR)) + s_off;
@@ -460,7 +435,7 @@
     }
     if (tid == 0) {
         const uint32_t hdr = a.zlib ? sizeof(tfdf::ZLIB_HDR) : sizeof(tfdf::GZIP_HDR);
-        const uint64_t body = n ? (a.pfx[n - 1] & DF_VAL_MASK) : 0;
+        const uint64_t body = n ? (a.pfx[n - 1] & LB_VAL_MASK) : 0;
         uint8_t* o = a.out;
         if (a.zlib) { o[0] = 0x78; o[1] = 0x9c; }
         else { o[0] = 0x1f; o[1] = 0x8b; o[2] = 0x08; for (int i = 3; i < 9; i++) o[i] = 0; o[9] = 0xff; }
diff --git a/transferia_b200/csrc/kernels_encode.cuh b/transferia_b200/csrc/kernels_encode.cuh
--- a/transferia_b200/csrc/kernels_encode.cuh
+++ b/transferia_b200/csrc/kernels_encode.cuh
@@ -295,6 +295,11 @@
 }
 #endif
 
+struct StrPlace { uint64_t a, b; };
+__host__ __device__ __forceinline__ uint64_t str_data_start(const StrPlace& p, uint64_t n, uint64_t str_bytes_before) {
+    return p.a + (uint64_t)varint_len(n) + p.b * n + str_bytes_before;
+}
+
 struct LayoutArgs {
     DCol* cols; int ncols;
     const int32_t* out_cols;
@@ -306,6 +311,7 @@
     uint8_t* raw; DState* st;
     uint64_t nrows_in; int has_sel; uint32_t frame_bytes;
     uint64_t* col_bytes;
+    const StrPlace* str_place;
 };
 
 #define TF_STR_TILE 256
@@ -334,35 +340,40 @@
 __global__ void __launch_bounds__(256) k_layout_finish(LayoutArgs a) {
     __shared__ uint64_t s_size[3][256];
     __shared__ uint64_t s_pos[256];
-    __shared__ uint64_t s_run;
+    __shared__ uint64_t s_sbefore[256];
+    __shared__ uint64_t s_run, s_srun;
     const uint64_t n = a.st->n_kept;
     if (threadIdx.x == 0) {
         uint8_t* o = a.raw; uint64_t p = 0;
         o[p++] = 1; o[p++] = 0; o[p++] = 2; o[p++] = 0xff; o[p++] = 0xff; o[p++] = 0xff; o[p++] = 0xff; o[p++] = 0;
         uint64_t v = (uint64_t)a.ncols; while (v >= 0x80) { o[p++] = (uint8_t)(v | 0x80); v >>= 7; } o[p++] = (uint8_t)v;
         v = n; while (v >= 0x80) { o[p++] = (uint8_t)(v | 0x80); v >>= 7; } o[p++] = (uint8_t)v;
-        s_run = p;
+        s_run = p; s_srun = 0;
     }
     for (int base = 0; base < a.ncols; base += 256) {
         const int c = base + threadIdx.x;
         __syncthreads();
+        bool str = false;
         if (c < a.ncols) {
             const DCol& d = a.cols[a.out_cols[c]];
+            str = d.out_kind == OK_STR || d.out_kind == OK_TOSTR;
             s_size[0][threadIdx.x] = a.col_header_off[c + 1] - a.col_header_off[c];
             s_size[1][threadIdx.x] = (d.nullable && n) ? n : 0;
-            s_size[2][threadIdx.x] = n ? ((d.out_kind == OK_STR || d.out_kind == OK_TOSTR) ? a.col_bytes[d.str_slot] : (uint64_t)d.out_w * n) : 0;
+            s_size[2][threadIdx.x] = n ? (str ? a.col_bytes[d.str_slot] : (uint64_t)d.out_w * n) : 0;
+            s_sbefore[threadIdx.x] = str ? s_size[2][threadIdx.x] : 0;
         }
         __syncthreads();
         if (threadIdx.x == 0) {
-            uint64_t p = s_run; const int m = a.ncols - base < 256 ? a.ncols - base : 256;
-            for (int k = 0; k < m; k++) { s_pos[k] = p; p += s_size[0][k] + s_size[1][k] + s_size[2][k]; }
-            s_run = p;
+            uint64_t p = s_run, q = s_srun; const int m = a.ncols - base < 256 ? a.ncols - base : 256;
+            for (int k = 0; k < m; k++) { s_pos[k] = p; p += s_size[0][k] + s_size[1][k] + s_size[2][k]; const uint64_t v = s_sbefore[k]; s_sbefore[k] = q; q += v; }
+            s_run = p; s_srun = q;
         }
         __syncthreads();
         if (c < a.ncols) {
             DCol& d = a.cols[a.out_cols[c]];
             const uint64_t p = s_pos[threadIdx.x];
-            d.hdr_off = p; d.null_off = p + s_size[0][threadIdx.x]; d.out_off = d.null_off + s_size[1][threadIdx.x];
+            d.hdr_off = p; d.null_off = p + s_size[0][threadIdx.x];
+            d.out_off = str ? str_data_start(a.str_place[d.str_slot], n, s_sbefore[threadIdx.x]) : d.null_off + s_size[1][threadIdx.x];
             const uint32_t hb = a.col_header_off[c], hn = (uint32_t)s_size[0][threadIdx.x];
             for (uint32_t k = 0; k < hn; k++) a.raw[p + k] = a.col_headers[hb + k];
         }
diff --git a/transferia_b200/csrc/kernels_lz4.cuh b/transferia_b200/csrc/kernels_lz4.cuh
--- a/transferia_b200/csrc/kernels_lz4.cuh
+++ b/transferia_b200/csrc/kernels_lz4.cuh
@@ -1,6 +1,7 @@
 #pragma once
 #include "device_types.cuh"
 #include "kernels_encode.cuh"
+#include "lookback.cuh"
 
 namespace tfk {
 
@@ -16,9 +17,6 @@
 #define LZ_MAX_FRAME (LZ_THREADS * LZ_SEG)
 #define LZ_HDR 25
 #define LZ_NONE 0xffffffffu
-#define LZ_FLAG_AGG (1ull << 62)
-#define LZ_FLAG_INCL (2ull << 62)
-#define LZ_VAL_MASK ((1ull << 62) - 1)
 
 __host__ __device__ inline uint32_t lz4_bound(uint32_t n) { return n + n / 255 + 16; }
 
@@ -87,35 +85,6 @@
         n += 4;
     }
     return n < maxb ? n : maxb;
-}
-
-__device__ __forceinline__ unsigned long long lz_lookback(const Lz4Args& a, uint32_t f, uint32_t lane) {
-    unsigned long long excl = 0;
-    if (!f) return 0;
-    int64_t base = (int64_t)f;
-    for (uint32_t spins = 0;;) {
-        unsigned long long v[4];
-#pragma unroll
-        for (int k = 0; k < 4; k++) { const int64_t j = base - 1 - 32 * k - (int64_t)lane; v[k] = j >= 0 ? *(volatile unsigned long long*)&a.pfx[j] : LZ_FLAG_INCL; }
-        bool done = false, stale = false;
-#pragma unroll
-        for (int k = 0; k < 4; k++) {
-            if (done || stale) continue;
-            const uint32_t fl = (uint32_t)(v[k] >> 62);
-            const uint32_t incl = __ballot_sync(0xffffffffu, fl == 2), none = __ballot_sync(0xffffffffu, fl == 0);
-            const uint32_t upto = incl ? (uint32_t)__ffs((int)incl) - 1 : 31u;
-            const uint32_t need = upto == 31 ? 0xffffffffu : ((2u << upto) - 1);
-            if (none & need) { stale = true; continue; }
-            unsigned long long part = lane <= upto ? (v[k] & LZ_VAL_MASK) : 0ull;
-#pragma unroll
-            for (int d = 16; d; d >>= 1) part += __shfl_xor_sync(0xffffffffu, part, d);
-            excl += part; base -= 32;
-            if (incl) done = true;
-        }
-        if (done) break;
-        if (stale) { if (++spins > (1u << 20)) { if (lane == 0) a.st->pad = 1; break; } __nanosleep(100); }
-    }
-    return excl;
 }
 
 #ifdef TF_KERNELS_LZ4
@@ -181,9 +150,9 @@
     uint32_t pend_f = 0xffffffffu, pend_cs = 0;
     auto resolve_flush = [&](uint32_t pf, uint32_t pcs) {
         if (warp == 0) {
-            const unsigned long long excl = lz_lookback(a, pf, lane);
+            const unsigned long long excl = lookback_excl(a.pfx, pf, lane, a.st);
             if (lane == 0) {
-                *(volatile unsigned long long*)&a.pfx[pf] = LZ_FLAG_INCL | (excl + pcs + LZ_HDR);
+                *(volatile unsigned long long*)&a.pfx[pf] = LB_FLAG_INCL | (excl + pcs + LZ_HDR);
                 s_woff = excl;
                 a.comp_size[pf] = pcs; a.wire_off[pf] = excl;
                 if (pf + 1 == n_frames) { a.st->wire_total = excl + pcs + LZ_HDR; a.tail[0] = n_frames; }
@@ -412,7 +381,7 @@
         const uint32_t ll_final = nseg ? carry_incl[nseg - 1] : 0;
         const int32_t delta_final = (int32_t)(total_seq_bytes + 1 + ext_bytes(ll_final)) - (int32_t)(len - ll_final);
         const uint32_t cs = total_seq_bytes + 1 + ext_bytes(ll_final) + ll_final;
-        if (tid == 0) { *(volatile unsigned long long*)&a.pfx[f] = LZ_FLAG_AGG | (unsigned long long)(cs + LZ_HDR); }
+        if (tid == 0) { *(volatile unsigned long long*)&a.pfx[f] = LB_FLAG_AGG | (unsigned long long)(cs + LZ_HDR); }
         LZ_PHASE(3);
         if (pend_f != 0xffffffffu) resolve_flush(pend_f, pend_cs);
         LZ_PHASE(5);
diff --git a/transferia_b200/csrc/kernels_str.cuh b/transferia_b200/csrc/kernels_str.cuh
--- a/transferia_b200/csrc/kernels_str.cuh
+++ b/transferia_b200/csrc/kernels_str.cuh
@@ -2,18 +2,25 @@
 #include "device_types.cuh"
 #include "kernels_encode.cuh"
 #include "kernels_fmt.cuh"
+#include "lookback.cuh"
 
 namespace tfk {
 
-__device__ __forceinline__ uint32_t str_len(const DCol& c, const uint32_t* sel, uint64_t j, uint64_t n, uint64_t& r) {
+template <bool TOSTR> __device__ __forceinline__ uint32_t str_len_t(const DCol& c, const uint32_t* sel, uint64_t j, uint64_t n, uint64_t& r) {
     if (j >= n) { r = 0; return 0xffffffffu; }
     r = sel ? sel[j] : j;
-    if (c.out_kind == OK_TOSTR) { CountSink cs; cs.n = 0; fmt_value(cs, c, r); return cs.n; }
+    if (TOSTR) { CountSink cs; cs.n = 0; fmt_value(cs, c, r); return cs.n; }
     if (!row_valid(c, r)) return 0;
     return c.offsets[r + 1] - c.offsets[r];
 }
+__device__ __forceinline__ uint32_t str_len(const DCol& c, const uint32_t* sel, uint64_t j, uint64_t n, uint64_t& r) {
+    return c.out_kind == OK_TOSTR ? str_len_t<true>(c, sel, j, n, r) : str_len_t<false>(c, sel, j, n, r);
+}
+
+__device__ __forceinline__ uint32_t leb_len_of_piece(uint32_t pl) { return pl < 129 ? 1 : (pl < 16386 ? 2 : (pl < 2097155 ? 3 : (pl < 268435460 ? 4 : 5))); }
 
 #define TF_STR_GROUP 4
+
 #ifdef TF_KERNELS_STR
 __global__ void __launch_bounds__(TF_STR_THREADS) k_str_sizes(EncodeArgs a) {
     __shared__ uint32_t sm[33];
@@ -26,7 +33,7 @@
     for (int g = 0; g < TF_STR_GROUP; g++) { uint64_t r; Ls[g] = str_len(c, a.sel, jg + (uint64_t)g * TF_STR_TILE + threadIdx.x, n, r); }
 #pragma unroll
     for (int g = 0; g < TF_STR_GROUP; g++) {
-        uint32_t tot; block_excl_scan(Ls[g] != 0xffffffffu ? Ls[g] + (a.columnar ? 0 : varint_len(Ls[g])) : 0u, &tot, sm);
+        uint32_t tot; block_excl_scan(Ls[g] != 0xffffffffu ? Ls[g] : 0u, &tot, sm);
         if (threadIdx.x == 0 && jg + (uint64_t)g * TF_STR_TILE < n) a.tile_sum[(size_t)c.str_slot * a.ntiles_cap + blockIdx.x * TF_STR_GROUP + g] = tot;
         __syncthreads();
     }
@@ -39,6 +46,62 @@
     for (int it = 0; it < 8; it++) { const uint32_t mid = (lo + hi) >> 1; if (ex[mid] <= x) lo = mid; else hi = mid; }
     return lo;
 }
+template <bool VLB>
+__device__ __forceinline__ void str_word_bytes(const DCol& c, const uint32_t* ex_, const uint32_t* src_, uint32_t tot, uint32_t m, uint32_t t, uint32_t r, uint8_t* dst0) {
+    const int32_t sb = (int32_t)(4 * t) - (int32_t)m;
+    uint32_t pe = ex_[r + 1], pl = pe - ex_[r];
+    uint32_t vl = VLB ? leb_len_of_piece(pl) : 0, plen = pl - vl;
+    uint32_t val = 0, mask = 0;
+#pragma unroll
+    for (int b = 0; b < 4; b++) {
+        const int32_t xs = sb + b;
+        if (xs < 0 || (uint32_t)xs >= tot) continue;
+        const uint32_t x = (uint32_t)xs;
+        while (x >= pe) { r++; pe = ex_[r + 1]; pl = pe - ex_[r]; vl = VLB ? leb_len_of_piece(pl) : 0; plen = pl - vl; }
+        const uint32_t k = x - ex_[r];
+        uint32_t byte;
+        if (k < vl) { const uint32_t v = plen >> (7 * k); byte = (v & 0x7f) | ((v >> 7) ? 0x80u : 0u); }
+        else byte = c.heap[src_[r] + (k - vl)];
+        val |= byte << (8 * b); mask |= 1u << b;
+    }
+    uint8_t* dst = dst0 + 4 * (size_t)t;
+    if (mask == 15) *(uint32_t*)dst = val;
+    else { for (int b = 0; b < 4; b++) if ((mask >> b) & 1) dst[b] = (uint8_t)(val >> (8 * b)); }
+}
+template <bool VLB>
+__device__ __forceinline__ void str_write_tile(const DCol& c, const uint32_t* ex_, const uint32_t* src_, uint8_t* gdst) {
+    const uint32_t tot = ex_[TF_STR_TILE];
+    if (!tot) return;
+    const uint32_t hsh = ((uint32_t)(uintptr_t)c.heap & 3);
+    const uint32_t* hw = (const uint32_t*)(c.heap - hsh);
+    const uint32_t m = (uint32_t)((uintptr_t)gdst & 3);
+    const uint32_t T = (m + tot + 3) >> 2;
+    uint8_t* dst0 = gdst - m;
+    auto locate = [&](uint32_t t, uint32_t& r, uint32_t& so) {
+        const int32_t sb = (int32_t)(4 * t) - (int32_t)m;
+        const uint32_t x0 = sb < 0 ? 0u : (uint32_t)sb;
+        r = str_find_row(ex_, x0);
+        const uint32_t pe = ex_[r + 1], vl = VLB ? leb_len_of_piece(pe - ex_[r]) : 0u, k0 = x0 - ex_[r];
+        so = src_[r] + (k0 - vl) + hsh;
+        return sb >= 0 && (uint32_t)sb + 4 <= pe && k0 >= vl;
+    };
+    for (uint32_t t0 = threadIdx.x; t0 < T; t0 += 2 * TF_STR_THREADS) {
+        const uint32_t t1 = t0 + TF_STR_THREADS;
+        const bool h1 = t1 < T;
+        uint32_t r0, so0, r1, so1;
+        const bool f0 = locate(t0, r0, so0);
+        const bool f1 = locate(h1 ? t1 : t0, r1, so1) && h1;
+        const uint32_t sh0 = (so0 & 3) * 8, sh1 = (so1 & 3) * 8;
+        uint32_t a0 = 0, b0 = 0, a1 = 0, b1 = 0;
+        if (f0) { a0 = __ldg(hw + (so0 >> 2)); if (sh0) b0 = __ldg(hw + (so0 >> 2) + 1); }
+        if (f1) { a1 = __ldg(hw + (so1 >> 2)); if (sh1) b1 = __ldg(hw + (so1 >> 2) + 1); }
+        if (f0) *(uint32_t*)(dst0 + 4 * (size_t)t0) = sh0 ? __funnelshift_r(a0, b0, sh0) : a0;
+        else str_word_bytes<VLB>(c, ex_, src_, tot, m, t0, r0, dst0);
+        if (f1) *(uint32_t*)(dst0 + 4 * (size_t)t1) = sh1 ? __funnelshift_r(a1, b1, sh1) : a1;
+        else if (h1) str_word_bytes<VLB>(c, ex_, src_, tot, m, t1, r1, dst0);
+    }
+}
+
 #ifdef TF_KERNELS_STR
 __global__ void __launch_bounds__(TF_STR_THREADS) k_encode_str_plain(EncodeArgs a) {
     __shared__ uint32_t sm[33];
@@ -50,7 +113,6 @@
     const uint64_t n = a.st->n_kept;
     const uint64_t jg = (uint64_t)blockIdx.x * TF_STR_TILE * TF_STR_GROUP;
     if (jg >= n) return;
-    const uint32_t vlb = a.columnar ? 0u : 1u;
     uint32_t Ls[TF_STR_GROUP]; uint64_t Rs[TF_STR_GROUP]; uint32_t src[TF_STR_GROUP];
 #pragma unroll
     for (int g = 0; g < TF_STR_GROUP; g++) Ls[g] = str_len(c, a.sel, jg + (uint64_t)g * TF_STR_TILE + threadIdx.x, n, Rs[g]);
@@ -59,103 +121,26 @@
 #pragma unroll
     for (int g = 0; g < TF_STR_GROUP; g++) {
         const bool have = Ls[g] != 0xffffffffu;
-        uint32_t tot; const uint32_t ex = block_excl_scan(have ? Ls[g] + (vlb ? varint_len(Ls[g]) : 0) : 0u, &tot, sm);
+        uint32_t tot; const uint32_t ex = block_excl_scan(have ? Ls[g] : 0u, &tot, sm);
         const uint64_t j0 = jg + (uint64_t)g * TF_STR_TILE;
         const uint64_t tb = j0 < n ? a.tile_base[(size_t)c.str_slot * a.ntiles_cap + blockIdx.x * TF_STR_GROUP + g] : 0;
-        if (a.columnar && have) ((uint32_t*)(a.raw + c.offs_off))[j0 + threadIdx.x] = (uint32_t)(tb + ex);
+        if (have) ((uint32_t*)(a.raw + c.offs_off))[j0 + threadIdx.x] = (uint32_t)(tb + ex);
         s_ex[g][threadIdx.x] = ex; s_src[g][threadIdx.x] = src[g];
         if (threadIdx.x == 0) { s_ex[g][TF_STR_TILE] = tot; s_tb[g] = tb; }
         __syncthreads();
     }
-    const uint32_t hsh = ((uint32_t)(uintptr_t)c.heap & 3);
-    const uint32_t* hw = (const uint32_t*)(c.heap - hsh);
 #pragma unroll 1
-    for (int g = 0; g < TF_STR_GROUP; g++) {
-        const uint32_t* ex_ = s_ex[g]; const uint32_t* src_ = s_src[g];
-        const uint32_t tot = ex_[TF_STR_TILE];
-        if (!tot) continue;
-        uint8_t* gdst = a.raw + c.out_off + s_tb[g];
-        const uint32_t m = (uint32_t)((uintptr_t)gdst & 3);
-        const uint32_t T = (m + tot + 3) >> 2;
-        uint8_t* dst0 = gdst - m;
-        for (uint32_t t = threadIdx.x; t < T; t += TF_STR_THREADS) {
-            const int32_t sb = (int32_t)(4 * t) - (int32_t)m;
-            const uint32_t x0 = sb < 0 ? 0u : (uint32_t)sb;
-            uint32_t r = str_find_row(ex_, x0);
-            uint32_t pe = ex_[r + 1], pl = pe - ex_[r];
-            uint32_t plen = pl, vl = 0;
-            if (vlb) { vl = pl < 129 ? 1 : (pl < 16386 ? 2 : (pl < 2097155 ? 3 : (pl < 268435460 ? 4 : 5))); plen = pl - vl; }
-            const uint32_t k0 = x0 - ex_[r];
-            if (sb >= 0 && (uint32_t)sb + 4 <= pe && k0 >= vl) {
-                const uint32_t so = src_[r] + (k0 - vl) + hsh; const uint32_t sh = (so & 3) * 8;
-                const uint32_t w0 = __ldg(hw + (so >> 2)); uint32_t val = w0;
-                if (sh) val = __funnelshift_r(w0, __ldg(hw + (so >> 2) + 1), sh);
-                *(uint32_t*)(dst0 + 4 * (size_t)t) = val;
-                continue;
-            }
-            uint32_t val = 0, mask = 0;
-#pragma unroll
-            for (int b = 0; b < 4; b++) {
-                const int32_t xs = sb + b;
-                if (xs < 0 || (uint32_t)xs >= tot) continue;
-                const uint32_t x = (uint32_t)xs;
-                while (x >= pe) { r++; pe = ex_[r + 1]; pl = pe - ex_[r]; if (vlb) { vl = pl < 129 ? 1 : (pl < 16386 ? 2 : (pl < 2097155 ? 3 : (pl < 268435460 ? 4 : 5))); plen = pl - vl; } else plen = pl; }
-                const uint32_t k = x - ex_[r];
-                uint32_t byte;
-                if (k < vl) { const uint32_t v = plen >> (7 * k); byte = (v & 0x7f) | ((v >> 7) ? 0x80u : 0u); }
-                else byte = c.heap[src_[r] + (k - vl)];
-                val |= byte << (8 * b); mask |= 1u << b;
-            }
-            uint8_t* dst = dst0 + 4 * (size_t)t;
-            if (mask == 15) *(uint32_t*)dst = val;
-            else { for (int b = 0; b < 4; b++) if ((mask >> b) & 1) dst[b] = (uint8_t)(val >> (8 * b)); }
-        }
-    }
-}
-#endif
-
-#ifdef TF_KERNELS_STR
-__global__ void __launch_bounds__(TF_STR_THREADS) k_encode_str(EncodeArgs a) {
-    __shared__ uint32_t sm[33];
-    __shared__ __align__(16) uint8_t stage[TF_STR_STAGE + 8];
-    const DCol c = a.cols[a.slots[blockIdx.y]];
-    if (c.out_kind != OK_TOSTR) return;
-    const uint64_t n = a.st->n_kept;
-    const uint64_t j0 = (uint64_t)blockIdx.x * TF_STR_TILE;
-    if (j0 >= n) return;
-    uint64_t R; const uint32_t L = str_len(c, a.sel, j0 + threadIdx.x, n, R);
-    const bool tostr = c.out_kind == OK_TOSTR;
-    const uint8_t* s = (L != 0xffffffffu && L && !tostr) ? c.heap + c.offsets[R] : nullptr;
-    if (tostr && c.nullable && !a.columnar && L != 0xffffffffu) a.raw[c.null_off + j0 + threadIdx.x] = 0;
-    uint32_t tot; const uint32_t ex = block_excl_scan(L != 0xffffffffu ? L + (a.columnar ? 0 : varint_len(L)) : 0u, &tot, sm);
-    const uint64_t tb = a.tile_base[(size_t)c.str_slot * a.ntiles_cap + blockIdx.x];
-    uint8_t* gdst = a.raw + c.out_off + tb;
-    if (a.columnar && L != 0xffffffffu) ((uint32_t*)(a.raw + c.offs_off))[j0 + threadIdx.x] = (uint32_t)(tb + ex);
+    for (int g = 0; g < TF_STR_GROUP; g++) str_write_tile<false>(c, s_ex[g], s_src[g], a.raw + c.out_off + s_tb[g]);
+}
+#endif
+
+template <bool VLB>
+__device__ __forceinline__ void str_text_tile(const DCol& c, bool have, uint64_t R, uint32_t L, uint32_t ex, uint32_t tot, uint8_t* gdst, uint8_t* stage) {
     const bool staged = tot <= TF_STR_STAGE;
-    uint8_t* o = staged ? stage + ex : gdst + ex;
-    if (L != 0xffffffffu) {
-        if (!a.columnar) {
-            uint32_t v = L;
-            while (v >= 0x80) { *o++ = (uint8_t)(v | 0x80); v >>= 7; }
-            *o++ = (uint8_t)v;
-        }
-        if (tostr) { MemSink ms; ms.p = o; fmt_value(ms, c, R); o = ms.p; }
-        uint32_t nb = tostr ? 0 : L;
-        const uint32_t sh = ((uint32_t)(uintptr_t)s & 3) * 8;
-        const uint32_t* sw = (const uint32_t*)((uintptr_t)s & ~(uintptr_t)3);
-        while (nb) {
-            const uint32_t take = nb < 16 ? nb : 16;
-            const uint32_t need = (take + (sh >> 3) + 3) >> 2;
-            uint32_t w0 = __ldg(sw), w1 = need > 1 ? __ldg(sw + 1) : 0, w2 = need > 2 ? __ldg(sw + 2) : 0, w3 = need > 3 ? __ldg(sw + 3) : 0, w4 = need > 4 ? __ldg(sw + 4) : 0;
-            if (sh) { w0 = __funnelshift_r(w0, w1, sh); w1 = __funnelshift_r(w1, w2, sh); w2 = __funnelshift_r(w2, w3, sh); w3 = __funnelshift_r(w3, w4, sh); }
-            const uint32_t ww[4] = {w0, w1, w2, w3};
-#pragma unroll
-            for (int q = 0; q < 4; q++) {
-#pragma unroll
-                for (int b = 0; b < 4; b++) if ((uint32_t)(4 * q + b) < take) o[4 * q + b] = (uint8_t)(ww[q] >> (8 * b));
-            }
-            o += take; sw += 4; nb -= take;
-        }
+    if (have) {
+        uint8_t* o = staged ? stage + ex : gdst + ex;
+        if (VLB) { uint32_t v = L; while (v >= 0x80) { *o++ = (uint8_t)(v | 0x80); v >>= 7; } *o++ = (uint8_t)v; }
+        MemSink ms; ms.p = o; fmt_value(ms, c, R);
     }
     if (!staged) return;
     __syncthreads();
@@ -174,8 +159,102 @@
             for (int b = 0; b < 4; b++) { const int32_t x = sb + b; if (x >= 0 && (uint32_t)x < tot) dst[b] = (uint8_t)(val >> (8 * b)); }
         }
     }
-}
-#endif
-
-
-}
+    __syncthreads();
+}
+
+#ifdef TF_KERNELS_STR
+__global__ void __launch_bounds__(TF_STR_THREADS) k_encode_str(EncodeArgs a) {
+    __shared__ uint32_t sm[33];
+    __shared__ __align__(16) uint8_t stage[TF_STR_STAGE + 8];
+    const DCol c = a.cols[a.slots[blockIdx.y]];
+    if (c.out_kind != OK_TOSTR) return;
+    const uint64_t n = a.st->n_kept;
+    const uint64_t j0 = (uint64_t)blockIdx.x * TF_STR_TILE;
+    if (j0 >= n) return;
+    uint64_t R; const uint32_t L = str_len(c, a.sel, j0 + threadIdx.x, n, R);
+    const bool have = L != 0xffffffffu;
+    uint32_t tot; const uint32_t ex = block_excl_scan(have ? L : 0u, &tot, sm);
+    const uint64_t tb = a.tile_base[(size_t)c.str_slot * a.ntiles_cap + blockIdx.x];
+    if (have) ((uint32_t*)(a.raw + c.offs_off))[j0 + threadIdx.x] = (uint32_t)(tb + ex);
+    str_text_tile<false>(c, have, R, L, ex, tot, a.raw + c.out_off + tb, stage);
+}
+#endif
+
+struct StrNativeArgs {
+    const DCol* cols; const int32_t* str_cols; uint32_t nstr;
+    const StrPlace* place;
+    const uint32_t* sel; DState* st; uint8_t* raw;
+    unsigned long long* cells;
+    uint64_t* col_bytes;
+};
+#ifdef TF_KERNELS_STR
+template <bool TOSTR>
+__global__ void __launch_bounds__(TF_STR_THREADS) k_encode_str_native(StrNativeArgs a) {
+    __shared__ uint32_t sm[33];
+    __shared__ uint32_t s_ex[TF_STR_GROUP][TF_STR_TILE + 1];
+    __shared__ uint32_t s_src[TF_STR_GROUP][TF_STR_TILE];
+    __shared__ __align__(16) uint8_t stage[TOSTR ? TF_STR_STAGE + 8 : 16];
+    __shared__ uint32_t s_ticket;
+    __shared__ unsigned long long s_excl;
+    const uint32_t tid = threadIdx.x, lane = tid & 31;
+    const uint64_t n = a.st->n_kept;
+    const uint32_t groups = (uint32_t)((n + TF_STR_TILE * TF_STR_GROUP - 1) / (TF_STR_TILE * TF_STR_GROUP));
+    const uint32_t ntickets = groups * a.nstr;
+    for (;;) {
+        __syncthreads();
+        if (tid == 0) s_ticket = atomicAdd(&a.st->str_ticket, 1u);
+        __syncthreads();
+        const uint32_t t = s_ticket;
+        if (t >= ntickets) break;
+        const uint32_t s = t / groups;
+        const uint64_t jg = (uint64_t)(t - s * groups) * TF_STR_TILE * TF_STR_GROUP;
+        const DCol c = a.cols[a.str_cols[s]];
+        const bool tostr = TOSTR && c.out_kind == OK_TOSTR;
+        unsigned long long size = 0;
+        if (tostr) {
+#pragma unroll 1
+            for (int g = 0; g < TF_STR_GROUP; g++) {
+                uint64_t R; const uint32_t L = str_len_t<true>(c, a.sel, jg + (uint64_t)g * TF_STR_TILE + tid, n, R);
+                uint32_t tot; const uint32_t ex = block_excl_scan(L != 0xffffffffu ? L + varint_len(L) : 0u, &tot, sm);
+                s_ex[g][tid] = ex; s_src[g][tid] = (uint32_t)R;
+                if (tid == 0) s_ex[g][TF_STR_TILE] = tot;
+                size += tot;
+            }
+        } else {
+            uint32_t Ls[TF_STR_GROUP]; uint64_t Rs[TF_STR_GROUP]; uint32_t src[TF_STR_GROUP];
+#pragma unroll
+            for (int g = 0; g < TF_STR_GROUP; g++) Ls[g] = str_len_t<false>(c, a.sel, jg + (uint64_t)g * TF_STR_TILE + tid, n, Rs[g]);
+#pragma unroll
+            for (int g = 0; g < TF_STR_GROUP; g++) src[g] = (Ls[g] != 0xffffffffu && Ls[g]) ? c.offsets[Rs[g]] : 0u;
+#pragma unroll
+            for (int g = 0; g < TF_STR_GROUP; g++) {
+                uint32_t tot; const uint32_t ex = block_excl_scan(Ls[g] != 0xffffffffu ? Ls[g] + varint_len(Ls[g]) : 0u, &tot, sm);
+                s_ex[g][tid] = ex; s_src[g][tid] = src[g];
+                if (tid == 0) s_ex[g][TF_STR_TILE] = tot;
+                size += tot;
+            }
+        }
+        if (tid == 0) {
+            *(volatile unsigned long long*)&a.cells[t] = (t ? LB_FLAG_AGG : LB_FLAG_INCL) | size;
+            atomicAdd((unsigned long long*)&a.col_bytes[s], size);
+        }
+        if (tid < 32) {
+            const unsigned long long excl = lookback_excl(a.cells, t, lane, a.st);
+            if (lane == 0) { if (t) *(volatile unsigned long long*)&a.cells[t] = LB_FLAG_INCL | (excl + size); s_excl = excl; }
+        }
+        __syncthreads();
+        uint8_t* gdst = a.raw + str_data_start(a.place[s], n, s_excl);
+#pragma unroll 1
+        for (int g = 0; g < TF_STR_GROUP; g++) {
+            const uint32_t tot = s_ex[g][TF_STR_TILE];
+            if (tostr) {
+                const uint32_t pl = s_ex[g][tid + 1] - s_ex[g][tid];
+                str_text_tile<true>(c, jg + (uint64_t)g * TF_STR_TILE + tid < n, s_src[g][tid], pl - leb_len_of_piece(pl), s_ex[g][tid], tot, gdst, stage);
+            } else str_write_tile<true>(c, s_ex[g], s_src[g], gdst);
+            gdst += tot;
+        }
+    }
+}
+#endif
+
+}
diff --git a/transferia_b200/csrc/launch.hpp b/transferia_b200/csrc/launch.hpp
--- a/transferia_b200/csrc/launch.hpp
+++ b/transferia_b200/csrc/launch.hpp
@@ -25,6 +25,8 @@
 void launch_k_str_sizes(dim3 grid, dim3 block, size_t smem, cudaStream_t s, EncodeArgs a);
 void launch_k_encode_str_plain(dim3 grid, dim3 block, size_t smem, cudaStream_t s, EncodeArgs a);
 void launch_k_encode_str(dim3 grid, dim3 block, size_t smem, cudaStream_t s, EncodeArgs a);
+void launch_k_encode_str_native(dim3 grid, dim3 block, size_t smem, cudaStream_t s, StrNativeArgs a, bool tostr);
+cudaError_t str_kernels_init(int* ctas_per_sm_plain, int* ctas_per_sm_tostr);
 void launch_k_mask_encode(dim3 grid, dim3 block, size_t smem, cudaStream_t s, MaskArgs a);
 void launch_k_shard_ids(dim3 grid, dim3 block, size_t smem, cudaStream_t s, ShardArgs a);
 void launch_k_lz4_frames(dim3 grid, dim3 block, size_t smem, cudaStream_t s, Lz4Args a);
diff --git a/transferia_b200/csrc/lookback.cuh b/transferia_b200/csrc/lookback.cuh
--- /dev/null
+++ b/transferia_b200/csrc/lookback.cuh
@@ -0,0 +1,39 @@
+#pragma once
+#include "device_types.cuh"
+
+namespace tfk {
+
+#define LB_FLAG_AGG (1ull << 62)
+#define LB_FLAG_INCL (2ull << 62)
+#define LB_VAL_MASK ((1ull << 62) - 1)
+
+__device__ __forceinline__ unsigned long long lookback_excl(const unsigned long long* cells, uint32_t f, uint32_t lane, DState* st) {
+    unsigned long long excl = 0;
+    if (!f) return 0;
+    int64_t base = (int64_t)f;
+    for (uint32_t spins = 0;;) {
+        unsigned long long v[4];
+#pragma unroll
+        for (int k = 0; k < 4; k++) { const int64_t j = base - 1 - 32 * k - (int64_t)lane; v[k] = j >= 0 ? *(const volatile unsigned long long*)&cells[j] : LB_FLAG_INCL; }
+        bool done = false, stale = false;
+#pragma unroll
+        for (int k = 0; k < 4; k++) {
+            if (done || stale) continue;
+            const uint32_t fl = (uint32_t)(v[k] >> 62);
+            const uint32_t incl = __ballot_sync(0xffffffffu, fl == 2), none = __ballot_sync(0xffffffffu, fl == 0);
+            const uint32_t upto = incl ? (uint32_t)__ffs((int)incl) - 1 : 31u;
+            const uint32_t need = upto == 31 ? 0xffffffffu : ((2u << upto) - 1);
+            if (none & need) { stale = true; continue; }
+            unsigned long long part = lane <= upto ? (v[k] & LB_VAL_MASK) : 0ull;
+#pragma unroll
+            for (int d = 16; d; d >>= 1) part += __shfl_xor_sync(0xffffffffu, part, d);
+            excl += part; base -= 32;
+            if (incl) done = true;
+        }
+        if (done) break;
+        if (stale) { if (++spins > (1u << 20)) { if (lane == 0) st->pad = 1; break; } __nanosleep(100); }
+    }
+    return excl;
+}
+
+}
diff --git a/transferia_b200/csrc/tfgpu.cu b/transferia_b200/csrc/tfgpu.cu
--- a/transferia_b200/csrc/tfgpu.cu
+++ b/transferia_b200/csrc/tfgpu.cu
@@ -54,6 +54,7 @@
     JsonCol* d_sjcols = nullptr; JsonCol* d_scsvcols = nullptr; uint8_t* d_snames = nullptr;
     int32_t* d_fixed_slots = nullptr; int32_t* d_str_slots = nullptr; int32_t* d_mask_slots = nullptr; int32_t* d_out_cols = nullptr;
     MaskKey* d_mask_keys = nullptr;
+    StrPlace* d_str_place = nullptr;
     int n_fsteps = 0, n_fixed_slots = 0, n_str = 0, n_mask_cols = 0, n_tostr = 0;
     std::vector<int32_t> fixed_slots, str_slots, mask_slot_cols, mask_slot_key;
     std::vector<int> col_out_kind, col_out_w, col_str_slot, col_mask_slot, col_nullable;
@@ -74,6 +75,7 @@
     uint64_t launches = 0;
     uint32_t frame_bytes = LZ_MAX_FRAME;
     int sm_count = 132;
+    int str_ctas_per_sm[2] = {1, 1};
     std::vector<std::unique_ptr<PlanDev>> plans;
     DevBuf in_arena, work, raw, wire, strict_stage, lens_arena, lens_arena2, csv_text, csv_stage, json_msgs, n2f_stage, n2f_heap, off_scratch;
     DState* d_state = nullptr; DCol* d_cols = nullptr; size_t d_cols_cap = 0;
@@ -195,10 +197,21 @@
         if (kind == OK_STR || kind == OK_TOSTR) { pd.col_str_slot[c] = (int)pd.str_slots.size(); pd.str_slots.push_back((int32_t)c); }
         else if (kind == OK_MASK) { pd.mask_slot_cols.push_back((int32_t)c); }
         else pd.fixed_slots.push_back((int32_t)c);
-        if (nullable && kind == OK_TODT) pd.fixed_slots.push_back((int32_t)c | TF_SLOT_ZEROMAP);
+        if (nullable && (kind == OK_TODT || kind == OK_TOSTR)) pd.fixed_slots.push_back((int32_t)c | TF_SLOT_ZEROMAP);
         else if (nullable && kind != OK_MASK && kind != OK_TOSTR) pd.fixed_slots.push_back((int32_t)c | TF_SLOT_NULLMAP);
     }
     if (pd.str_slots.size() > 65535) throw tfplan::FatalError(TF_E_FATAL_UNSUPPORTED, "more than 65535 String columns (one grid row per column)");
+    std::vector<StrPlace> place(pd.str_slots.size());
+    if (pl.col_header_off.size() == pl.out_cols.size() + 1) {
+        uint64_t a = 8 + (uint64_t)varint_len(pl.out_cols.size()), b = 0;
+        for (size_t k = 0; k < pl.out_cols.size(); k++) {
+            const size_t c = (size_t)pl.out_cols[k];
+            a += pl.col_header_off[k + 1] - pl.col_header_off[k];
+            b += (uint64_t)pd.col_nullable[c];
+            if (pd.col_str_slot[c] >= 0) place[pd.col_str_slot[c]] = StrPlace{a, b};
+            else b += (uint64_t)pd.col_out_w[c];
+        }
+    }
     std::vector<JsonCol> jcols; std::vector<uint8_t> jnames;
     for (size_t k = 0; k < pl.out_cols.size(); k++) {
         JsonCol jc; std::memset(&jc, 0, sizeof jc); jc.col = pl.out_cols[k]; jc.name_off = (int32_t)jnames.size(); jc.name_len = (int32_t)pl.out_schema[k].name.size();
@@ -246,16 +259,18 @@
                  o_mask = ci.add(pd.mask_slot_cols.data(), pd.mask_slot_cols.size() * 4), o_keys = ci.add(keys.data(), keys.size() * sizeof(MaskKey)),
                  o_out = ci.add(oc.data(), oc.size() * 4), o_jcols = ci.add(jcols.data(), jcols.size() * sizeof(JsonCol)), o_jnames = ci.add(jnames.data(), jnames.size()),
                  o_sjcols = ci.add(sjcols.data(), sjcols.size() * sizeof(JsonCol)), o_scsv = ci.add(scsvcols.data(), scsvcols.size() * sizeof(JsonCol)),
-                 o_snames = ci.add(snames.data(), snames.size()), o_shard = ci.add(shcols.data(), shcols.size() * sizeof(ShardCol));
+                 o_snames = ci.add(snames.data(), snames.size()), o_shard = ci.add(shcols.data(), shcols.size() * sizeof(ShardCol)),
+                 o_place = ci.add(place.data(), place.size() * sizeof(StrPlace));
     uint8_t* P = ci.upload(pd.consts);
     pd.d_terms = (DTerm*)(P + o_terms); pd.d_expr_off = (uint32_t*)(P + o_expr_off); pd.d_fsteps = (DFilterStep*)(P + o_fsteps); pd.d_blob = P + o_blob;
     pd.d_col_headers = P + o_hdr; pd.d_col_header_off = (uint32_t*)(P + o_hdr_off);
     pd.d_fixed_slots = (int32_t*)(P + o_fixed); pd.d_str_slots = (int32_t*)(P + o_str); pd.d_mask_slots = (int32_t*)(P + o_mask); pd.d_mask_keys = (MaskKey*)(P + o_keys);
     pd.d_out_cols = (int32_t*)(P + o_out); pd.d_jcols = (JsonCol*)(P + o_jcols); pd.d_jnames = P + o_jnames;
     pd.d_sjcols = (JsonCol*)(P + o_sjcols); pd.d_scsvcols = (JsonCol*)(P + o_scsv); pd.d_snames = P + o_snames; pd.d_shard_cols = (ShardCol*)(P + o_shard);
-}
-
-struct Sizes { uint64_t raw_bound, n_frames_max, wire_bound; uint32_t ntiles_cap, nblocks; };
+    pd.d_str_place = (StrPlace*)(P + o_place);
+}
+
+struct Sizes { uint64_t raw_bound, n_frames_max, wire_bound; uint32_t ntiles_cap, nblocks, ngroups_cap; };
 
 Sizes compute_sizes(const tfgpu_engine* e, const PlanDev& pd, const tf_batch* in, bool columnar = false, bool json = false) {
     const tfplan::Plan& pl = pd.plan; const uint64_t n = in->nrows;
@@ -276,6 +291,7 @@
     s.wire_bound = s.n_frames_max * (uint64_t)(LZ_HDR + lz4_bound(e->frame_bytes)) + 1024;
     s.ntiles_cap = (uint32_t)((n + TF_STR_TILE - 1) / TF_STR_TILE + 1);
     s.nblocks = (uint32_t)((n + 255) / 256 + 1);
+    s.ngroups_cap = (uint32_t)((n + TF_STR_TILE * TF_STR_GROUP - 1) / (TF_STR_TILE * TF_STR_GROUP));
     return s;
 }
 
@@ -358,7 +374,8 @@
     Layout W;
     const size_t o_keep = W.take(n), o_errcode = W.take(n), o_errstep = W.take(2 * n), o_blockcnt = W.take(sz.nblocks * 4), o_blockoff = W.take(sz.nblocks * 4),
                  o_sel = W.take(n * 4), o_tile_sum = W.take(nslot_alloc * sz.ntiles_cap * 4), o_tile_base = W.take(nslot_alloc * sz.ntiles_cap * 8),
-                 o_comp = W.take(sz.n_frames_max * 4), o_wire_off = W.take(sz.n_frames_max * 8), o_pfx = W.take(sz.n_frames_max * 8), o_col_bytes = W.take(nslot_alloc * 8);
+                 o_comp = W.take(sz.n_frames_max * 4), o_wire_off = W.take(sz.n_frames_max * 8), o_pfx = W.take(sz.n_frames_max * 8),
+                 o_str_cells = W.take(nslot_alloc * sz.ngroups_cap * 8), o_col_bytes = W.take(nslot_alloc * 8);
     e->work.ensure(W.total());
     uint8_t* w = e->work.p;
     e->keep = w + o_keep; e->errcode = w + o_errcode; e->errstep = (uint16_t*)(w + o_errstep);
@@ -460,7 +477,7 @@
         if (ser && !has_filter && n) { CK(cudaMemsetAsync(e->errcode, 0, n, s)); CK(cudaMemsetAsync(e->errstep, 0, 2 * n, s)); }
         if (jt) { e->prof_begin("k_json_sizes", s); launch_k_json_sizes(jt, TF_JSON_TILE, 0, s, ja); e->prof_end(s); }
         LayoutArgs lj{e->d_cols, 0, pd.d_out_cols, pd.d_str_slots, 1, e->tile_sum, e->tile_base, sz.ntiles_cap, pd.d_col_headers, pd.d_col_header_off,
-                      e->raw.p, e->d_state, n, 1, e->frame_bytes, e->col_bytes};
+                      e->raw.p, e->d_state, n, 1, e->frame_bytes, e->col_bytes, nullptr};
         e->prof_begin("k_layout_scan", s); launch_k_layout_scan(1, 1024, 0, s, lj); e->prof_end(s);
         uint64_t json_total = 0;
         {
@@ -472,11 +489,17 @@
         CK(cudaGetLastError());
         return;
     }
-    if (pd.n_str && ntiles) { e->prof_begin("k_str_sizes", s); launch_k_str_sizes(dim3(str_gx, pd.n_str), TF_STR_THREADS, 0, s, ea); e->prof_end(s); }
     LayoutArgs la{e->d_cols, (int)pl.out_cols.size(), pd.d_out_cols, pd.d_str_slots, pd.n_str, e->tile_sum, e->tile_base, sz.ntiles_cap, pd.d_col_headers, pd.d_col_header_off,
-                  e->raw.p, e->d_state, n, 1, e->frame_bytes, e->col_bytes};
-    if (pd.n_str) { e->prof_begin("k_layout_scan", s); launch_k_layout_scan(pd.n_str, 1024, 0, s, la); e->prof_end(s); }
+                  e->raw.p, e->d_state, n, 1, e->frame_bytes, e->col_bytes, pd.d_str_place};
     if (!columnar) {
+        CK(cudaMemsetAsync(w + o_str_cells, 0, o_col_bytes - o_str_cells + nslot_alloc * 8, s));
+        if (pd.n_str && n) {
+            const uint64_t tickets = (uint64_t)pd.n_str * sz.ngroups_cap;
+            if (tickets >= (1ull << 31)) throw tfplan::FatalError(TF_E_FATAL_ARG, "too many String column groups for one batch: split it");
+            StrNativeArgs sa{e->d_cols, pd.d_str_slots, (uint32_t)pd.n_str, pd.d_str_place, sel, e->d_state, e->raw.p, (unsigned long long*)(w + o_str_cells), e->col_bytes};
+            const uint32_t grid = (uint32_t)std::min<uint64_t>(tickets, (uint64_t)e->sm_count * (uint64_t)e->str_ctas_per_sm[pd.n_tostr > 0]);
+            e->prof_begin("k_encode_str_native", s); launch_k_encode_str_native(grid, TF_STR_THREADS, 0, s, sa, pd.n_tostr > 0); e->prof_end(s);
+        }
         e->prof_begin("k_layout_finish", s); launch_k_layout_finish(1, 256, 0, s, la); e->prof_end(s);
         if (n) {
             if (pd.n_fixed_slots) {
@@ -484,8 +507,6 @@
                 EncodeArgs fa = ea; fa.slots = pd.d_fixed_slots;
                 e->prof_begin("k_encode_fixed", s); launch_k_encode_fixed(dim3(gx, pd.n_fixed_slots), 256, 0, s, fa); e->prof_end(s);
             }
-            if (pd.n_str) { e->prof_begin("k_encode_str_plain", s); launch_k_encode_str_plain(dim3(str_gx, pd.n_str), TF_STR_THREADS, 0, s, ea); e->prof_end(s); }
-            if (pd.n_str && pd.n_tostr) { e->prof_begin("k_encode_str", s); launch_k_encode_str(dim3(ntiles, pd.n_str), TF_STR_THREADS, 0, s, ea); e->prof_end(s); }
             if (pd.n_mask_cols) {
                 MaskArgs ma{e->d_cols, pd.d_mask_slots, pd.d_mask_keys, sel, e->d_state, e->raw.p, 0};
                 e->prof_begin("k_mask_encode", s); launch_k_mask_encode(dim3((uint32_t)((n + 127) / 128), pd.n_mask_cols), 128, 0, s, ma); e->prof_end(s);
@@ -507,6 +528,8 @@
         }
         std::vector<int32_t> both(fixed); both.insert(both.end(), valid.begin(), valid.end());
         if (!both.empty()) CK(cudaMemcpyAsync(e->d_call_slots, both.data(), both.size() * 4, cudaMemcpyHostToDevice, s));
+        if (pd.n_str && ntiles) { e->prof_begin("k_str_sizes", s); launch_k_str_sizes(dim3(str_gx, pd.n_str), TF_STR_THREADS, 0, s, ea); e->prof_end(s); }
+        if (pd.n_str) { e->prof_begin("k_layout_scan", s); launch_k_layout_scan(pd.n_str, 1024, 0, s, la); e->prof_end(s); }
         e->prof_begin("k_layout_columnar", s); launch_k_layout_columnar(1, 256, 0, s, la, e->d_regions); e->prof_end(s);
         if (n) {
             if (!fixed.empty()) {
@@ -584,7 +607,7 @@
         CK(cudaMalloc(&e->d_tail, 64)); CK(cudaMemset(e->d_tail, 0, 64));
         CK(cudaEventCreateWithFlags(&e->ev_fork, cudaEventDisableTiming));
         CK(cudaMalloc(&e->d_state, sizeof(DState)));
-        CK(lz4_kernels_init()); CK(dbz_kernels_init()); CK(deflate_kernels_init());
+        CK(lz4_kernels_init()); CK(dbz_kernels_init()); CK(deflate_kernels_init()); CK(str_kernels_init(&e->str_ctas_per_sm[0], &e->str_ctas_per_sm[1]));
     } catch (const CudaError& c) { return c.e == cudaErrorMemoryAllocation ? TF_E_RETRY_OOM : TF_E_RETRY_LAUNCH; }
     catch (const std::exception&) { return TF_E_FATAL_CONFIG; }
     *out = e.release();
diff --git a/transferia_b200/csrc/tu_str.cu b/transferia_b200/csrc/tu_str.cu
--- a/transferia_b200/csrc/tu_str.cu
+++ b/transferia_b200/csrc/tu_str.cu
@@ -5,4 +5,11 @@
 void launch_k_str_sizes(dim3 grid, dim3 block, size_t smem, cudaStream_t s, EncodeArgs a) { k_str_sizes<<<grid, block, smem, s>>>(a); }
 void launch_k_encode_str_plain(dim3 grid, dim3 block, size_t smem, cudaStream_t s, EncodeArgs a) { k_encode_str_plain<<<grid, block, smem, s>>>(a); }
 void launch_k_encode_str(dim3 grid, dim3 block, size_t smem, cudaStream_t s, EncodeArgs a) { k_encode_str<<<grid, block, smem, s>>>(a); }
+void launch_k_encode_str_native(dim3 grid, dim3 block, size_t smem, cudaStream_t s, StrNativeArgs a, bool tostr) {
+    if (tostr) k_encode_str_native<true><<<grid, block, smem, s>>>(a); else k_encode_str_native<false><<<grid, block, smem, s>>>(a);
 }
+cudaError_t str_kernels_init(int* ctas_per_sm_plain, int* ctas_per_sm_tostr) {
+    const cudaError_t r = cudaOccupancyMaxActiveBlocksPerMultiprocessor(ctas_per_sm_plain, k_encode_str_native<false>, TF_STR_THREADS, 0);
+    return r != cudaSuccess ? r : cudaOccupancyMaxActiveBlocksPerMultiprocessor(ctas_per_sm_tostr, k_encode_str_native<true>, TF_STR_THREADS, 0);
+}
+}
```

Result: no change. 1.089 billion (median of 6 runs) (+1.0%).
